# akofke/fountain

Measured on AMD Instinct MI355X. Metric: Mrays/s (primary+secondary) at fixed spp, higher is better.
Workload: dtype f32

## Files before the change

fountain_amd/csrc/ftn_gbuffer.hip:

```cpp
#include "ftn_wavefront.hip"
#include "ftn_gbuffer.h"

namespace ftn {

#define GB_MAX_PASS_THROUGH 4096u
struct GbParams {
    float w2c[16];
    float* out;
    float4 *spillA, *spillB, *spillC;
    float4* rec;
};

__device__ inline Rgb gb_albedo(const ftn_material& m) {
    const Rgb a(m.a[0], m.a[1], m.a[2]), b(m.b[0], m.b[1], m.b[2]);
    switch (m.type) {
        case FTN_MAT_MATTE: return clamp_positive(a);
        case FTN_MAT_MIRROR: return clamp_positive(a);
        case FTN_MAT_METAL: return fresnel_conductor(1.0f, Rgb(1.0f), a, b);
        case FTN_MAT_PLASTIC: return a + b;
        default: return clamp_positive(a) + clamp_positive(b);
    }
}

template <bool TEX>
__global__ void __launch_bounds__(256) k_gb_shade(RenderParams P, WfBuffers W, GbParams G, const uint32_t* __restrict__ q_in, const uint32_t* count_in,
                                                  uint32_t* q_out, uint32_t* count_out) {
    const DScene& S = P.S;
    const uint32_t qi = blockIdx.x * 256u + threadIdx.x;
    bool push = false;
    uint32_t p = 0;
    if (qi < *count_in) {
        p = q_in[qi];
        const float4 ro = W.ray[2 * (size_t)p], rdv = W.ray[2 * (size_t)p + 1];
        DRay ray0; ray0.o = V3(ro.x, ro.y, ro.z); ray0.d = V3(rdv.x, rdv.y, rdv.z); ray0.t_max = rdv.w; ray0.time = 0.0f;
        const DHit h = load_hit(W, p);
        float4 r0 = make_float4(0.0f, 0.0f, 0.0f, 0.0f), r1 = r0, r2 = r0;
        if (h.prim >= 0) {
            DSI si; make_interaction(S, h, ray0, &si);
            if (si.mat < 0) {
                const DRay nr = spawn_ray(si.hit, ray0.d);
                W.ray[2 * (size_t)p] = make_float4(nr.o.x, nr.o.y, nr.o.z, 0.0f); W.ray[2 * (size_t)p + 1] = make_float4(nr.d.x, nr.d.y, nr.d.z, nr.t_max);
                push = true;
            } else {
                ftn_material m = S.materials[si.mat];
                if (TEX && material_is_textured(S, si.mat)) {
                    const uint32_t slot = p / W.samples, sidx = p % W.samples;
                    const DTile tile = P.tiles[slot >> 8];
                    const int px = tile.x0 + (int)(slot & 15u), py = tile.y0 + (int)((slot >> 4) & 15u);
                    Rng crng; crng.seed(indexed_key(P.seed, px, py, W.first_sample + sidx));
                    const V2 j = crng.next2(); const V2 p_film((float)px + j.x, (float)py + j.y); const V2 p_lens = crng.next2(); const float time_u = crng.next();
                    const DRay cam = camera_ray(P.C, p_film, p_lens, time_u);
                    const DRayDiff rd = camera_ray_diff(P.C, p_film, p_lens, cam, 1.0f / sqrtf((float)P.spp));
                    DSIX ex; DSI s2; make_interaction(S, h, ray0, &s2, &ex);
                    const DTexDiffs td = compute_tex_diffs(si.hit.p, si.hit.n, ex.dpdu, ex.dpdv, rd);
                    m = material_resolve(S, si.mat, ex.uv, td);
                }
                const Rgb alb = gb_albedo(m);
                const V3 pc = m4_point(G.w2c, si.hit.p);
                r0 = make_float4(alb.r, alb.g, alb.b, 1.0f);
                r1 = make_float4(si.shading_n.x, si.shading_n.y, si.shading_n.z, pc.z);
                r2 = make_float4(si.hit.p.x, si.hit.p.y, si.hit.p.z, 0.0f);
            }
        }
        if (!push) { float4* R = G.rec + 3 * (size_t)p; R[0] = r0; R[1] = r1; R[2] = r2; }
    }
    const bool pred[1] = {push};
    const uint32_t val[1] = {p};
    uint32_t* const qs[1] = {q_out};
    uint32_t* const cs[1] = {count_out};
    block_push<1>(pred, val, qs, cs);
}

__global__ void k_gb_reset(WfBuffers W, uint32_t out_ctr) {
    if (threadIdx.x != 0 || blockIdx.x != 0) return;
    W.counters[CTR(11)] = 0;
    for (int i = 16; i < 56; i++) W.counters[CTR(i)] = 0;
    W.counters[CTR(out_ctr)] = 0;
}

__device__ inline void gb_film_add(const GbParams& G, const FilmCtxW& F, V2 p_film, float4 r0, float4 r1, float4 r2, int own_x, int own_y, float* acc, uint32_t* spill, uint32_t* bc_writes) {
    const float pdx = p_film.x - 0.5f, pdy = p_film.y - 0.5f;
    int p0x = f2i_sat(ceilf(pdx - F.radius[0])), p0y = f2i_sat(ceilf(pdy - F.radius[1]));
    int p1x = f2i_sat(floorf(pdx + F.radius[0])) + 1, p1y = f2i_sat(floorf(pdy + F.radius[1])) + 1;
    p0x = max(p0x, F.tpb[0]); p0y = max(p0y, F.tpb[1]); p1x = min(p1x, F.tpb[2]); p1y = min(p1y, F.tpb[3]);
    const bool hit = r0.w != 0.0f;
    const float v[10] = {r0.x, r0.y, r0.z, r1.x, r1.y, r1.z, r2.x, r2.y, r2.z, r1.w};
    int touched = 0;
    const size_t width = (size_t)(F.crop[2] - F.crop[0]);
    for (int y = p0y; y < p1y; y++)
        for (int x = p0x; x < p1x; x++) {
            touched++;
            if (x == own_x && y == own_y) {
                if (hit) {
#pragma unroll
                    for (int k = 0; k < 10; k++) acc[k] += v[k] * 1.0f;
                    acc[10] += 1.0f;
                }
                acc[11] += 1.0f;
                continue;
            }
            const size_t i = (size_t)(y - F.crop[1]) * width + (size_t)(x - F.crop[0]);
            float* a = reinterpret_cast<float*>(G.spillA + i);
            float* b = reinterpret_cast<float*>(G.spillB + i);
            float* c = reinterpret_cast<float*>(G.spillC + i);
            if (hit) {
#pragma unroll
                for (int k = 0; k < 3; k++) { atomicAdd(a + k, v[k] * 1.0f); atomicAdd(b + k, v[3 + k] * 1.0f); atomicAdd(c + k, v[6 + k] * 1.0f); }
                atomicAdd(c + 3, v[9] * 1.0f);
                atomicAdd(a + 3, 1.0f);
            }
            atomicAdd(b + 3, 1.0f);
            (*bc_writes)++;
        }
    if (touched != 1) (*spill)++;
}

#define GB_ACC_CHUNK 4u
__global__ void __launch_bounds__(256) k_gb_accumulate(RenderParams P, WfBuffers W, GbParams G) {
    __shared__ float4 s_rec[256 * GB_ACC_CHUNK * 3];
    const uint32_t slot = blockIdx.x * 256u + threadIdx.x;
    uint32_t spill = 0, bc = 0;
    bool valid = false, in_crop = false; int px = 0, py = 0; size_t ai = 0;
    FilmCtxW F; float acc[12];
#pragma unroll
    for (int k = 0; k < 12; k++) acc[k] = 0.0f;
    if (slot < W.n_slots) {
        const DTile tile = P.tiles[slot >> 8];
        px = tile.x0 + (int)(slot & 15u); py = tile.y0 + (int)((slot >> 4) & 15u);
        if (px < tile.x1 && py < tile.y1) {
            valid = true;
            for (int i = 0; i < 4; i++) F.crop[i] = P.crop[i];
            F.sb[0] = tile.x0; F.sb[1] = tile.y0; F.sb[2] = tile.x1; F.sb[3] = tile.y1; F.radius[0] = P.radius[0]; F.radius[1] = P.radius[1];
            const int p0x = f2i_sat(ceilf((float)tile.x0 - 0.5f - P.radius[0])), p0y = f2i_sat(ceilf((float)tile.y0 - 0.5f - P.radius[1]));
            const int p1x = f2i_sat(ceilf((float)tile.x1 - 0.5f + P.radius[0] + 1.0f)), p1y = f2i_sat(ceilf((float)tile.y1 - 0.5f - P.radius[1] + 1.0f));
            F.tpb[0] = max(p0x, P.crop[0]); F.tpb[1] = max(p0y, P.crop[1]); F.tpb[2] = min(p1x, P.crop[2]); F.tpb[3] = min(p1y, P.crop[3]);
            in_crop = px >= P.crop[0] && px < P.crop[2] && py >= P.crop[1] && py < P.crop[3];
            ai = in_crop ? ((size_t)(py - P.crop[1]) * (size_t)(P.crop[2] - P.crop[0]) + (size_t)(px - P.crop[0])) : 0;
            if (in_crop) {
#pragma unroll
                for (int k = 0; k < 12; k++) acc[k] = G.out[12 * ai + k];
            }
        }
    }
    const size_t block_first = (size_t)blockIdx.x * 256u * W.samples;
    for (uint32_t s0 = 0; s0 < W.samples; s0 += GB_ACC_CHUNK) {
        const uint32_t n = W.samples - s0 < GB_ACC_CHUNK ? W.samples - s0 : GB_ACC_CHUNK;
        for (uint32_t e = threadIdx.x; e < 256u * 3u * n; e += 256u) {
            const uint32_t sl = e / (3u * n), k3 = e - sl * 3u * n;
            const size_t p = block_first + (size_t)sl * W.samples + s0 + k3 / 3u;
            if (p < W.n_paths) s_rec[sl * GB_ACC_CHUNK * 3u + k3] = G.rec[3 * p + k3 % 3u];
        }
        __syncthreads();
        if (valid) {
            for (uint32_t k = 0; k < n; k++) {
                const float4* r = &s_rec[(threadIdx.x * GB_ACC_CHUNK + k) * 3u];
                Rng crng; crng.seed(indexed_key(P.seed, px, py, W.first_sample + s0 + k));
                const V2 j = crng.next2();
                gb_film_add(G, F, V2((float)px + j.x, (float)py + j.y), r[0], r[1], r[2], in_crop ? px : (-2147483647), py, acc, &spill, &bc);
            }
        }
        __syncthreads();
    }
    if (valid && in_crop) {
#pragma unroll
        for (int k = 0; k < 12; k++) G.out[12 * ai + k] = acc[k];
    }
    if (spill) atomicAdd(&P.stats->spill_samples, (unsigned long long)spill);
    if (bc) atomicAdd(&P.stats->bc_writes, (unsigned long long)bc);
}

__global__ void __launch_bounds__(256) k_gb_merge(GbParams G, size_t n, const DevStats* __restrict__ stats) {
    if (stats->bc_writes == 0) return;
    for (size_t i = (size_t)blockIdx.x * 256u + threadIdx.x; i < n; i += (size_t)gridDim.x * 256u) {
        const float4 a = G.spillA[i], b = G.spillB[i], c = G.spillC[i];
        if (b.w == 0.0f) continue;
        const float add[12] = {a.x, a.y, a.z, b.x, b.y, b.z, c.x, c.y, c.z, c.w, a.w, b.w};
#pragma unroll
        for (int k = 0; k < 12; k++) G.out[12 * i + k] += add[k];
    }
}

__global__ void __launch_bounds__(256) k_gb_resolve(const float* __restrict__ in, size_t n, float* __restrict__ out12) {
    for (size_t i = (size_t)blockIdx.x * 256u + threadIdx.x; i < n; i += (size_t)gridDim.x * 256u) gbuffer_resolve_pixel(in + 12 * i, out12 + 12 * i);
}
void launch_gbuffer_resolve(const float* in, size_t n, float* out12, hipStream_t stream) {
    if (n == 0) return;
    const unsigned grid = (unsigned)std::min<size_t>((n + 255) / 256, 4096);
    hipLaunchKernelGGL(k_gb_resolve, dim3(grid), dim3(256), 0, stream, in, n, out12);
}

int wavefront_gbuffer(WavefrontState** state, const RenderParams& P, const std::vector<DTile>& tiles, const float w2c[16], float* d_out,
                      float4* spill_a, float4* spill_b, float4* spill_c, hipStream_t stream, double* trace_ms_out) {
    knobs_begin();
    { int rc0 = wf_state_init(state); if (rc0) return rc0; }
    WavefrontState* st = *state;
    const uint32_t n_slots = (uint32_t)tiles.size() * 256u;
    const uint32_t total_samples = P.last_sample - P.first_sample;
    if (n_slots == 0 || total_samples == 0) return FTN_OK;
    if (tiles.size() > ((size_t)1 << 20)) { g_wf_err = "more than 2^20 tiles (2^28 pixel slots) in one call: render the film in several tile ranges"; return FTN_ERR_UNSUPPORTED; }
    uint32_t S = (uint32_t)std::max<size_t>(1, ((size_t)std::min<uint32_t>(knob("FTN_WF_PATHS_M", 256), 256u) << 20) / n_slots);
    S = std::min(S, total_samples);
    int rc = wf_reserve(st, (size_t)S * n_slots);
    while (rc == FTN_ERR_OUT_OF_MEMORY && S > 1) {
        wf_free(st); (void)hipGetLastError();
        S = (S + 1) / 2;
        rc = wf_reserve(st, (size_t)S * n_slots);
    }
    if (rc) { wf_free(st); return rc; }
    if ((rc = trace4_prepare(st, P.S))) return rc;
    WfBuffers W = st->W;
    W.br = nullptr; W.pd = nullptr; W.pd_md = 0; W.pd_occ = 0; W.drain_sig = nullptr; W.drain_seq = 0; W.serial = 0; W.rng_replay = 0; W.mis_any = 0;
    W.gen_blocks = knob("FTN_GEN_BLOCKS", 1);
    uint32_t valid = 0; for (const DTile& t : tiles) valid += (uint32_t)((t.x1 - t.x0) * (t.y1 - t.y0));
    W.valid_per_sample = valid;
    GbParams G;
    memcpy(G.w2c, w2c, sizeof(G.w2c)); G.out = d_out; G.spillA = spill_a; G.spillB = spill_b; G.spillC = spill_c; G.rec = st->pd;
    const bool spheres = P.S.n_spheres != 0, tex = P.S.n_textures != 0;
    const size_t lds = (size_t)P.stack_entries * 256 * sizeof(uint32_t);
    const unsigned blocks_per_cu = (unsigned)std::max<size_t>(1, std::min<size_t>(8, (size_t)(160 * 1024) / std::max<size_t>(lds, 1)));
    const unsigned trace_grid_max = (unsigned)st->n_cu * blocks_per_cu;
    double trace_ms = 0.0;
    for (uint32_t s0 = 0; s0 < total_samples; s0 += S) {
        const uint32_t Sp = std::min(S, total_samples - s0);
        W.n_slots = n_slots; W.samples = Sp; W.n_paths = Sp * n_slots; W.first_sample = P.first_sample + s0; W.seg_cap = (uint32_t)st->cap_paths;
        hipLaunchKernelGGL(k_wf_reset, dim3(1), dim3(64), 0, stream, W, 0, 0, P.stats);
        hipLaunchKernelGGL(k_wf_generate, dim3((W.n_paths + 255) / 256), dim3(256), 0, stream, P, W, 0);
        const unsigned tg = std::min<unsigned>(trace_grid_max, (2 * W.n_paths + 255) / 256);
        uint32_t n_q = Sp * valid;
        for (uint32_t r = 0;; r++) {
            const bool odd = (r & 1u) != 0;
            const uint32_t* q_in = odd ? W.q_shadow : W.q_closest;
            uint32_t* q_out = odd ? W.q_closest : W.q_shadow;
            const uint32_t c_in = odd ? 3u : 2u, c_out = odd ? 2u : 3u;
            if (r > 0) hipLaunchKernelGGL(k_gb_reset, dim3(1), dim3(64), 0, stream, W, c_out);
            WF_TRY(hipEventRecord(st->ev[0], stream));
            launch_trace(st, false, 0, spheres, tg, lds, stream, P, W, q_in, &W.counters[CTR(c_in)], &W.counters[CTR(16)], 2 * W.n_paths,
                         r == 0 && W.samples >= knob("FTN_T4_LOCKSTEP_MIN_SPP", 1) );
            WF_TRY(hipEventRecord(st->ev[1], stream));
            const dim3 sg(std::max<uint32_t>(1u, (n_q + 255) / 256));
            if (tex) hipLaunchKernelGGL(k_gb_shade<true>, sg, dim3(256), 0, stream, P, W, G, q_in, &W.counters[CTR(c_in)], q_out, &W.counters[CTR(c_out)]);
            else hipLaunchKernelGGL(k_gb_shade<false>, sg, dim3(256), 0, stream, P, W, G, q_in, &W.counters[CTR(c_in)], q_out, &W.counters[CTR(c_out)]);
            WF_TRY(hipMemcpyAsync(st->host_counters, W.counters, 16 * 32 * sizeof(uint32_t), hipMemcpyDeviceToHost, stream));
            WF_TRY(hipStreamSynchronize(stream));
            float ms = 0.0f; (void)hipEventElapsedTime(&ms, st->ev[0], st->ev[1]); trace_ms += ms;
            n_q = st->host_counters[CTR(c_out)];
            if (n_q == 0) break;
            if (r == GB_MAX_PASS_THROUGH) {
                g_wf_err = "a camera ray passed through more than 4096 null-material surfaces: the G-buffer would be incomplete";
                return FTN_ERR_INTERNAL;
            }
        }
        hipLaunchKernelGGL(k_gb_accumulate, dim3((n_slots + 255) / 256), dim3(256), 0, stream, P, W, G);
    }
    const size_t npix = (size_t)std::max(0, P.crop[2] - P.crop[0]) * (size_t)std::max(0, P.crop[3] - P.crop[1]);
    if (npix) hipLaunchKernelGGL(k_gb_merge, dim3((unsigned)std::min<size_t>((npix + 255) / 256, 4096)), dim3(256), 0, stream, G, npix, (const DevStats*)P.stats);
    WF_TRY(hipGetLastError());
    if (trace_ms_out) *trace_ms_out = trace_ms;
    return FTN_OK;
}

}
```

fountain_amd/csrc/ftn_trace4.hip:

```cpp
#include "ftn_wf_common.h"

namespace ftn {

enum : uint32_t { T4_IDLE = 0, T4_NODE = 1, T4_LEAF = 2 };
#define T4_NONE 0xffffffffu

typedef float t4_f2 __attribute__((ext_vector_type(2)));
__device__ inline bool slab4(float4 a, float4 b, V3 o, V3 inv, float t_max, float* t0o, float* t1o) {
    const float k = 1.0f + 2.0f * gamma_n(3);
    const t4_f2 px = {a.x, a.y}, py = {a.z, a.w}, pz = {b.x, b.y};
    const t4_f2 tx = (px - (t4_f2){o.x, o.x}) * (t4_f2){inv.x, inv.x};
    const t4_f2 ty = (py - (t4_f2){o.y, o.y}) * (t4_f2){inv.y, inv.y};
    const t4_f2 tz = (pz - (t4_f2){o.z, o.z}) * (t4_f2){inv.z, inv.z};
    const float far_k = fmin_(fmin_(fmax_(tx.x, tx.y), fmax_(ty.x, ty.y)), fmax_(tz.x, tz.y)) * k;
    const float t0 = fmax_(fmax_(fmax_(0.0f, fmin_(tx.x, tx.y)), fmin_(ty.x, ty.y)), fmin_(tz.x, tz.y));
    const float t1 = fmin_(t_max, far_k);
    *t0o = t0; *t1o = t1;
    return !(t0 > t1);
}

struct WaveQueue {
    uint32_t chunk_next, chunk_end, slice, slices_done, chunk; bool exhausted;
};
__device__ inline void wq_init(WaveQueue& q, uint32_t count, uint32_t chunk_max) {
    q.chunk_next = 0; q.chunk_end = 0; q.exhausted = count == 0; q.slice = blockIdx.x & 7u; q.slices_done = 0;
    uint32_t c = count / (gridDim.x * 4u * 16u); c &= ~63u; q.chunk = c < 64u ? 64u : (c > chunk_max ? chunk_max : c);
}
__device__ inline bool wq_refill(WaveQueue& q, uint32_t count, uint32_t* head, uint32_t lane) {
    bool just_dry = false;
    while (q.chunk_next == q.chunk_end && !q.exhausted) {
        const uint32_t s_lo = (uint32_t)(((unsigned long long)count * q.slice) >> 3) & ~63u, s_hi = q.slice == 7u ? count : ((uint32_t)(((unsigned long long)count * (q.slice + 1u)) >> 3) & ~63u);
        uint32_t base = 0;
        if (lane == 0) base = atomicAdd(head + CTR(q.slice), q.chunk);
        base = __shfl(base, 0, 64) + s_lo;
        if (base >= s_hi) { q.slice = (q.slice + 1u) & 7u; if (++q.slices_done == 8u) { q.exhausted = true; just_dry = true; } }
        else { q.chunk_next = base; q.chunk_end = base + q.chunk < s_hi ? base + q.chunk : s_hi; }
    }
    return just_dry;
}

struct RaySetup { V3 o, inv, dorig; float t_max, sx, sy, sz; uint32_t neg24 ; int kz; };
__device__ inline bool ray_is_exceptional(float ox, float oy, float oz, float ix, float iy, float iz) {
    return !(fabsf(ix) < FTN_INF && fabsf(iy) < FTN_INF && fabsf(iz) < FTN_INF && ix != 0.0f && iy != 0.0f && iz != 0.0f &&
             fabsf(ox) < FTN_INF && fabsf(oy) < FTN_INF && fabsf(oz) < FTN_INF &&
             fabsf(ox * ix) < FTN_INF && fabsf(oy * iy) < FTN_INF && fabsf(oz * iz) < FTN_INF);
}
template <bool SPHERES>
__device__ inline void ray_setup(RaySetup& R, float4 a, float4 b) {
    R.o = V3(a.x, a.y, a.z); const V3 d(b.x, b.y, b.z); R.t_max = b.w;
    if (SPHERES) R.dorig = d;
    R.inv = V3(1.0f / d.x, 1.0f / d.y, 1.0f / d.z);
    R.neg24 = ((d.x < 0.0f ? 1u : 0u) | (d.y < 0.0f ? 2u : 0u) | (d.z < 0.0f ? 4u : 0u)) * 0x010101u;
    R.kz = max_dimension(vabs(d));
    const bool k0 = R.kz == 0, k1 = R.kz == 1;
    const V3 dperm(k0 ? d.y : (k1 ? d.z : d.x), k0 ? d.z : (k1 ? d.x : d.y), k0 ? d.x : (k1 ? d.y : d.z));
    R.sx = -dperm.x / dperm.z; R.sy = -dperm.y / dperm.z; R.sz = 1.0f / dperm.z;
}

template <class E> struct T4Stack {
    E* base; E* lim; E* sp; E* spill; size_t n_lanes, gl; uint32_t spill_levels;
    __device__ inline size_t spill_at() const { const uint32_t lv = (uint32_t)((sp - lim) >> 8); return (size_t)(lv < spill_levels ? lv : spill_levels - 1u) * n_lanes + gl; }
    template <bool CHECK> __device__ inline void push(E v) {
        if (!CHECK || sp < lim) *sp = v; else if (spill_levels) spill[spill_at()] = v;
        sp += 256;
    }
    template <bool CHECK> __device__ inline E pop() {
        sp -= 256;
        if (!CHECK || sp < lim) return *sp;
        return spill_levels ? spill[spill_at()] : *base;
    }
    __device__ inline bool empty() const { return sp == base; }
};

enum : uint32_t { T8_IDLE = 0, T8_NODE = 1, T8_LEAF = 2, T8_LEAF_IN = 3  };
#define T8_XBOX 0x40000000u
__device__ inline bool ray_out_of_range8(float ox, float oy, float oz, float ix, float iy, float iz) {
    const float big_i = 1.152921504606846976e18f , big_o = 1.099511627776e12f ;
    return !(fabsf(ix) <= big_i && fabsf(iy) <= big_i && fabsf(iz) <= big_i && fabsf(ox) <= big_o && fabsf(oy) <= big_o && fabsf(oz) <= big_o);
}
struct T8Axis { float a, bn, bf; uint32_t n03, n47, f03, f47; };
__device__ inline T8Axis t8_axis(float org, uint32_t ebyte, float o, float inv, uint32_t lo03, uint32_t lo47, uint32_t hi03, uint32_t hi47) {
    T8Axis A;
    const float step = __uint_as_float(ebyte << 23);
    A.a = step * inv;
    const float b = (org - o) * inv;
    const float m = (fabsf(b) + 255.0f * fabsf(A.a)) * 9.5367431640625e-07f;
    A.bn = b - m; A.bf = b + m;
    const bool neg = inv < 0.0f;
    A.n03 = neg ? hi03 : lo03; A.n47 = neg ? hi47 : lo47; A.f03 = neg ? lo03 : hi03; A.f47 = neg ? lo47 : hi47;
    return A;
}
#define T8_BYTE(w, k) ((float)(((w) >> (8 * (k))) & 0xffu))
#define T8_CHILD(c, t0v, t1v) \
    { const uint32_t kx_ = (c) & 3; \
      const t4_f2 tx_ = __builtin_elementwise_fma((t4_f2){T8_BYTE((c) < 4 ? X.n03 : X.n47, kx_), T8_BYTE((c) < 4 ? X.f03 : X.f47, kx_)}, (t4_f2){X.a, X.a}, (t4_f2){X.bn, X.bf}); \
      const t4_f2 ty_ = __builtin_elementwise_fma((t4_f2){T8_BYTE((c) < 4 ? Y.n03 : Y.n47, kx_), T8_BYTE((c) < 4 ? Y.f03 : Y.f47, kx_)}, (t4_f2){Y.a, Y.a}, (t4_f2){Y.bn, Y.bf}); \
      const t4_f2 tz_ = __builtin_elementwise_fma((t4_f2){T8_BYTE((c) < 4 ? Z.n03 : Z.n47, kx_), T8_BYTE((c) < 4 ? Z.f03 : Z.f47, kx_)}, (t4_f2){Z.a, Z.a}, (t4_f2){Z.bn, Z.bf}); \
      t0v = fmax_(fmax_(fmax_(0.0f, tx_.x), ty_.x), tz_.x); t1v = fmin_(t_max, fmin_(fmin_(tx_.y, ty_.y), tz_.y) * k2); }

struct T4Lane { uint32_t mode, cur, lp; bool finish; };

template <bool CHECK>
__device__ inline void t4_pop_next(T4Stack<uint2>& St, T4Lane& L, float t_max) {
    for (;;) {
        if (St.empty()) { L.finish = true; return; }
        const uint2 v = St.template pop<CHECK>();
        if (!(__uint_as_float(v.y) > t_max)) {
            if (v.x >> 31) { L.lp = v.x & 0x7fffffffu; L.mode = T4_LEAF; } else { L.cur = v.x; L.mode = T4_NODE; }
            return;
        }
    }
}

template <bool CHECK>
__device__ __forceinline__ void t4_visit(T4Stack<uint2>& St, T4Lane& L, float t_max, uint32_t ea, uint32_t eb, uint32_t ec, uint32_t ed, float ta, float tb, float tc, float td, uint32_t ax) {
    const bool sA = (ax & 0xffu) != 0, sR = (ax & 0xff00u) != 0, sB = (ax & 0xff0000u) != 0;
    const uint32_t ex0 = sA ? eb : ea, ex1 = sA ? ea : eb, ey0 = sB ? ed : ec, ey1 = sB ? ec : ed;
    const float tx0 = sA ? tb : ta, tx1 = sA ? ta : tb, ty0 = sB ? td : tc, ty1 = sB ? tc : td;
    const uint32_t e0 = sR ? ey0 : ex0, e1 = sR ? ey1 : ex1, e2 = sR ? ex0 : ey0, e3 = sR ? ex1 : ey1;
    const float t1_ = sR ? ty1 : tx1, t2_ = sR ? tx0 : ty0, t3_ = sR ? tx1 : ty1;
    const bool h0 = e0 != T4_NONE, h1 = e1 != T4_NONE, h2 = e2 != T4_NONE, h3 = e3 != T4_NONE;
    const bool h01 = h0 || h1, h012 = h01 || h2;
    if (h3 && h012) St.template push<CHECK>(make_uint2(e3, __float_as_uint(t3_)));
    if (h2 && h01) St.template push<CHECK>(make_uint2(e2, __float_as_uint(t2_)));
    if (h1 && h0) St.template push<CHECK>(make_uint2(e1, __float_as_uint(t1_)));
    if (h012 || h3) {
        const uint32_t next = h0 ? e0 : (h1 ? e1 : (h2 ? e2 : e3));
        if (next >> 31) { L.lp = next & 0x7fffffffu; L.mode = T4_LEAF; } else L.cur = next;
    } else t4_pop_next<CHECK>(St, L, t_max);
}

template <bool CHECK>
__device__ inline void t4_record_step(const DScene& S, const RaySetup& R, T4Stack<uint2>& St, T4Lane& L) {
    const float4* rec = reinterpret_cast<const float4*>(reinterpret_cast<const char*>(S.quad) + L.cur);
    const float4 q0 = rec[0], q1 = rec[1], q2 = rec[2], q3 = rec[3], q4 = rec[4], q5 = rec[5], q6 = rec[6], q7 = rec[7];
    float ta, tb, tc, td, x1;
    const bool ha = slab4(q0, q1, R.o, R.inv, R.t_max, &ta, &x1), hb = slab4(q2, q3, R.o, R.inv, R.t_max, &tb, &x1);
    const bool hc = slab4(q4, q5, R.o, R.inv, R.t_max, &tc, &x1), hd = slab4(q6, q7, R.o, R.inv, R.t_max, &td, &x1);
    const uint32_t ea = ha ? __float_as_uint(q1.z) : T4_NONE, eb = hb ? __float_as_uint(q3.z) : T4_NONE, ec = hc ? __float_as_uint(q5.z) : T4_NONE, ed = hd ? __float_as_uint(q7.z) : T4_NONE;
    t4_visit<CHECK>(St, L, R.t_max, ea, eb, ec, ed, ta, tb, tc, td, __float_as_uint(q1.w) & R.neg24);
}

template <bool CHECK>
__device__ __forceinline__ void t4q_record_step(const DScene& S, T4Stack<uint2>& St, T4Lane& L, V3 o, V3 inv, float t_max, uint32_t neg24) {
    const uint4* rec = reinterpret_cast<const uint4*>(reinterpret_cast<const char*>(S.quad64) + L.cur);
    const uint4 r0 = rec[0], r1 = rec[1], r2 = rec[2], r3 = rec[3];
    const float k2 = 1.0f + 4.0f * gamma_n(3);
    const T8Axis X = t8_axis(__uint_as_float(r0.x), r0.w & 0xffu, o.x, inv.x, r1.x, r1.x, r1.y, r1.y);
    const T8Axis Y = t8_axis(__uint_as_float(r0.y), (r0.w >> 8) & 0xffu, o.y, inv.y, r1.z, r1.z, r1.w, r1.w);
    const T8Axis Z = t8_axis(__uint_as_float(r0.z), (r0.w >> 16) & 0xffu, o.z, inv.z, r2.x, r2.x, r2.y, r2.y);
    float ta, a1, tb, b1, tc, c1, td, d1;
    T8_CHILD(0, ta, a1) T8_CHILD(1, tb, b1) T8_CHILD(2, tc, c1) T8_CHILD(3, td, d1)
    const uint32_t ea = !(ta > a1) ? r2.z : T4_NONE, eb = !(tb > b1) ? r2.w : T4_NONE, ec = !(tc > c1) ? r3.x : T4_NONE, ed = !(td > d1) ? r3.y : T4_NONE;
    t4_visit<CHECK>(St, L, t_max, ea, eb, ec, ed, ta, tb, tc, td, r3.z & neg24);
}

enum : uint32_t { T4_LEAF_IN = 3 };
template <bool COUNT, bool SPHERES, int BURST, bool Q64 = false>
__global__ void __launch_bounds__(256, (SPHERES ? 1 : (Q64 ? T4Q_WAVES : 5))) k_wf_trace4(DScene S, WfBuffers W, const uint32_t* __restrict__ queue, const uint32_t* count_ptr, uint32_t* head, DevStats* stats,
                                                   uint32_t refill, uint32_t leaf_batch, uint32_t chunk_max, uint32_t lds_entries, uint2* __restrict__ spill, uint32_t spill_levels) {
    T4Stack<uint2> St;
    extern __shared__ uint2 lds_stack2[];
    St.base = lds_stack2 + threadIdx.x;
    St.lim = St.base + 256u * lds_entries; St.sp = St.base; St.spill = spill; St.spill_levels = spill_levels;
    St.n_lanes = (size_t)gridDim.x * 256u; St.gl = (size_t)blockIdx.x * 256u + threadIdx.x;
    const bool st_tiny = lds_entries < 3u;
    uint2* const st_soft = st_tiny ? St.base : St.lim - 3 * 256;
    const uint32_t count = *count_ptr;
    const uint32_t lane = lane_id();
    unsigned long long n_rec = 0, n_prim = 0;
    unsigned long long occ[7] = {0, 0, 0, 0, 0, 0, 0};
    T4Lane L; L.mode = T4_IDLE; L.cur = 0; L.lp = 0; L.finish = false;
    WaveQueue Q; wq_init(Q, count, chunk_max);
    uint32_t rid = 0;
    RaySetup R; R.o = V3(0.0f, 0.0f, 0.0f); R.inv = R.o; R.dorig = R.o; R.t_max = 0.0f; R.neg24 = 0; R.kz = 0; R.sx = R.sy = R.sz = 0.0f;
    int hprim = -1; float hb0 = 0.0f, hb1 = 0.0f, hb2 = 0.0f; bool found = false;
    const float4 rlo = make_float4(S.root_lo[0], S.root_lo[1], S.root_lo[2], 0.0f), rhi = make_float4(S.root_hi[0], S.root_hi[1], S.root_hi[2], 0.0f);
    for (;;) {
        const unsigned long long idle = __ballot(L.mode == T4_IDLE);
        if (!Q.exhausted && (uint32_t)__popcll(idle) >= refill) {
            const uint32_t need = (uint32_t)__popcll(idle);
            if (wq_refill(Q, count, head, lane)) {
                if (W.drain_sig && lane == 0 && atomicAdd(&W.counters[CTR(11)], 1u) + 1u == W.drain_at)
                    __hip_atomic_store(W.drain_sig, W.drain_seq, __ATOMIC_RELAXED, __HIP_MEMORY_SCOPE_SYSTEM);
            }
            const uint32_t avail = Q.chunk_end - Q.chunk_next;
            const uint32_t rank = (uint32_t)__popcll(idle & ((1ull << lane) - 1ull));
            bool hand_back = false; uint32_t q_entry = 0;
            if (COUNT) { occ[5]++; occ[6] += need < avail ? need : avail; }
            if (L.mode == T4_IDLE && rank < avail) {
                float4 a, b;
                q_entry = queue[Q.chunk_next + rank];
                load_queued_ray<false>(W, q_entry, &a, &b, &rid);
                ray_setup<SPHERES>(R, a, b);
                St.sp = St.base; L.cur = 0; found = false; hprim = -1; hb0 = 0.0f; hb1 = 0.0f; hb2 = 0.0f;
                if (ray_is_exceptional(R.o.x, R.o.y, R.o.z, R.inv.x, R.inv.y, R.inv.z) || (Q64 && ray_out_of_range8(R.o.x, R.o.y, R.o.z, R.inv.x, R.inv.y, R.inv.z)))
                    hand_back = true;
                else if (S.n_nodes == 0 || !slab_test(rlo, rhi, R.o, R.inv, R.t_max)) { W.hit[rid] = make_float4(FTN_INF, 0.0f, 0.0f, 0.0f); W.hit_prim[rid] = -1; }
                else if (S.root_is_leaf) { L.lp = 0; L.mode = T4_LEAF; }
                else L.mode = T4_NODE;
            }
            if (__ballot(hand_back) != 0) wave_push(hand_back, q_entry, W.q_exc_closest, &W.counters[CTR(32)]);
            Q.chunk_next += (need < avail ? need : avail);
        }
        const unsigned long long m_node = __ballot(L.mode == T4_NODE), m_leaf = __ballot(L.mode >= T4_LEAF);
        if ((m_node | m_leaf) == 0) { if (Q.exhausted) break; else continue; }
        L.finish = false;
        if (COUNT) occ[0]++;
        if (m_node != 0 && (uint32_t)__popcll(m_leaf) < leaf_batch) {
#pragma unroll
            for (int burst = 0; burst < BURST; burst++) {
                const bool on = L.mode == T4_NODE && !L.finish;
                if (COUNT && on) n_rec++;
                if (COUNT) { const unsigned long long m_on = __ballot(on); if (m_on) { occ[1]++; occ[2] += (unsigned long long)__popcll(m_on); } }
                if (__builtin_expect(__ballot(on && (st_tiny || St.sp > st_soft)) == 0, 1)) {
                    if (on) { if (Q64) t4q_record_step<false>(S, St, L, R.o, R.inv, R.t_max, R.neg24); else t4_record_step<false>(S, R, St, L); }
                } else if (on) { if (Q64) t4q_record_step<true>(S, St, L, R.o, R.inv, R.t_max, R.neg24); else t4_record_step<true>(S, R, St, L); }
            }
        } else {
            if (COUNT) { occ[3]++; occ[4] += (unsigned long long)__popcll(m_leaf); }
            if (L.mode >= T4_LEAF) {
                uint32_t prim = L.lp;
                const bool entering = Q64 && L.mode == T4_LEAF, explicit_box = entering && (L.lp & T8_XBOX);
                float4 x0 = make_float4(0.0f, 0.0f, 0.0f, 0.0f), x1 = x0;
                if (Q64) prim &= 0x3fffffffu;
                if (explicit_box) { x0 = S.quad64_xbox[2 * (size_t)prim]; x1 = S.quad64_xbox[2 * (size_t)prim + 1]; prim = __float_as_uint(x0.w); }
                float4 g0 = S.geom[S.geom_stride * prim], g1 = S.geom[S.geom_stride * prim + 1], g2 = S.geom[S.geom_stride * prim + 2];
                pin4(g0); pin4(g1); pin4(g2);
                bool pass = true;
                if (entering) {
                    if (!explicit_box) {
                        x0 = make_float4(fmin_(fmin_(g0.x, g1.x), g2.x), fmin_(fmin_(g0.y, g1.y), g2.y), fmin_(fmin_(g0.z, g1.z), g2.z), 0.0f);
                        x1 = make_float4(fmax_(fmax_(g0.x, g1.x), g2.x), fmax_(fmax_(g0.y, g1.y), g2.y), fmax_(fmax_(g0.z, g1.z), g2.z), 0.0f);
                    }
                    pass = slab_test(x0, x1, R.o, R.inv, R.t_max);
                }
                if (pass) {
                    if (COUNT) n_prim++;
                    float t = 0.0f, b0 = 0.0f, b1 = 0.0f, b2 = 0.0f;
                    const bool hh = prim_hit<SPHERES>(S, prim, g0, g1, g2, R.o, R.dorig, R.t_max, R.kz, R.sx, R.sy, R.sz, &t, &b0, &b1, &b2);
                    if (hh) { found = true; R.t_max = t; hprim = (int)prim; hb0 = b0; hb1 = b1; hb2 = b2; }
                }
                if (!pass || (__float_as_uint(g0.w) & GF_LEAF_END)) t4_pop_next<true>(St, L, R.t_max);
                else { L.lp = prim + 1u; if (Q64) L.mode = T4_LEAF_IN; }
            }
        }
        if (L.finish) {
            W.hit[rid] = make_float4(found ? R.t_max : FTN_INF, hb0, hb1, hb2); W.hit_prim[rid] = hprim;
            L.mode = T4_IDLE;
        }
    }
    if (COUNT) {
        for (int off = 32; off > 0; off >>= 1) { n_rec += __shfl_down(n_rec, off, 64); n_prim += __shfl_down(n_prim, off, 64); }
        if (lane == 0) { if (n_rec) atomicAdd(&stats->quad_records, n_rec); if (n_prim) atomicAdd(&stats->prims_tested, n_prim); for (int k = 0; k < 7; k++) if (occ[k]) atomicAdd(&stats->t4_occ[k], occ[k]); }
    }
    if (blockIdx.x == 0 && threadIdx.x == 0) atomicAdd(&stats->rays_closest, (unsigned long long)count);
}

extern __shared__ uint32_t lds_stack1[];
template <bool CHECK, int POLICY>
__device__ inline void t4_any_step(const DScene& S, const RaySetup& R, T4Stack<uint32_t>& St, T4Lane& L) {
    const float4* rec = reinterpret_cast<const float4*>(reinterpret_cast<const char*>(S.quad) + L.cur);
    const float4 q0 = rec[0], q1 = rec[1], q2 = rec[2], q3 = rec[3], q4 = rec[4], q5 = rec[5], q6 = rec[6], q7 = rec[7];
    float a0, a1, b0, b1, c0, c1, d0, d1;
    const bool ha = slab4(q0, q1, R.o, R.inv, R.t_max, &a0, &a1), hb = slab4(q2, q3, R.o, R.inv, R.t_max, &b0, &b1);
    const bool hc = slab4(q4, q5, R.o, R.inv, R.t_max, &c0, &c1), hd = slab4(q6, q7, R.o, R.inv, R.t_max, &d0, &d1);
    const uint32_t ea = __float_as_uint(q1.z), eb = __float_as_uint(q3.z), ec = __float_as_uint(q5.z), ed = __float_as_uint(q7.z);
    uint32_t next = 0; bool have = ha || hb || hc || hd;
    if (POLICY == 1) {
        const float sa = ha ? fmaxf(a1 - a0, 0.0f) : -1.0f, sb = hb ? fmaxf(b1 - b0, 0.0f) : -1.0f, sc = hc ? fmaxf(c1 - c0, 0.0f) : -1.0f, sd = hd ? fmaxf(d1 - d0, 0.0f) : -1.0f;
        const float best = fmaxf(fmaxf(sa, sb), fmaxf(sc, sd));
        const bool pa = sa == best, pb = !pa && sb == best, pc = !pa && !pb && sc == best, pd = !pa && !pb && !pc;
        next = pa ? ea : (pb ? eb : (pc ? ec : ed));
        if (ha && !pa) St.template push<CHECK>(ea);
        if (hb && !pb) St.template push<CHECK>(eb);
        if (hc && !pc) St.template push<CHECK>(ec);
        if (hd && !pd) St.template push<CHECK>(ed);
    } else {
        next = ha ? ea : (hb ? eb : (hc ? ec : ed));
        if (hd && (ha || hb || hc)) St.template push<CHECK>(ed);
        if (hc && (ha || hb)) St.template push<CHECK>(ec);
        if (hb && ha) St.template push<CHECK>(eb);
    }
    if (!have) {
        if (St.empty()) { L.finish = true; return; }
        next = St.template pop<CHECK>();
    }
    if (next >> 31) { L.lp = next & 0x7fffffffu; L.mode = T4_LEAF; } else L.cur = next;
}

template <bool COUNT, bool SPHERES, int BURST, int POLICY>
__global__ void __launch_bounds__(256) k_wf_trace4_any(DScene S, WfBuffers W, const uint32_t* __restrict__ queue, const uint32_t* count_ptr, uint32_t* head, DevStats* stats,
                                                       uint32_t refill, uint32_t leaf_batch, uint32_t chunk_max, uint32_t lds_entries, uint32_t* __restrict__ spill, uint32_t spill_levels) {
    T4Stack<uint32_t> St;
    St.base = lds_stack1 + threadIdx.x;
    St.lim = St.base + 256u * lds_entries; St.sp = St.base; St.spill = spill; St.spill_levels = spill_levels;
    St.n_lanes = (size_t)gridDim.x * 256u; St.gl = (size_t)blockIdx.x * 256u + threadIdx.x;
    const bool st_tiny = lds_entries < 3u;
    uint32_t* const st_soft = st_tiny ? St.base : St.lim - 3 * 256;
    const uint32_t count = *count_ptr;
    const uint32_t lane = lane_id();
    unsigned long long n_rec = 0, n_prim = 0;
    unsigned long long occ[7] = {0, 0, 0, 0, 0, 0, 0};
    T4Lane L; L.mode = T4_IDLE; L.cur = 0; L.lp = 0; L.finish = false;
    WaveQueue Q; wq_init(Q, count, chunk_max);
    uint32_t rid = 0;
    RaySetup R; R.o = V3(0.0f, 0.0f, 0.0f); R.inv = R.o; R.dorig = R.o; R.t_max = 0.0f; R.neg24 = 0; R.kz = 0; R.sx = R.sy = R.sz = 0.0f;
    bool found = false;
    const float4 rlo = make_float4(S.root_lo[0], S.root_lo[1], S.root_lo[2], 0.0f), rhi = make_float4(S.root_hi[0], S.root_hi[1], S.root_hi[2], 0.0f);
    for (;;) {
        const unsigned long long idle = __ballot(L.mode == T4_IDLE);
        if (!Q.exhausted && (uint32_t)__popcll(idle) >= refill) {
            const uint32_t need = (uint32_t)__popcll(idle);
            (void)wq_refill(Q, count, head, lane);
            const uint32_t avail = Q.chunk_end - Q.chunk_next;
            const uint32_t rank = (uint32_t)__popcll(idle & ((1ull << lane) - 1ull));
            bool hand_back = false; uint32_t q_entry = 0;
            if (COUNT) { occ[5]++; occ[6] += need < avail ? need : avail; }
            if (L.mode == T4_IDLE && rank < avail) {
                float4 a, b;
                q_entry = queue[Q.chunk_next + rank];
                load_queued_ray<true>(W, q_entry, &a, &b, &rid);
                ray_setup<SPHERES>(R, a, b);
                St.sp = St.base; L.cur = 0; found = false;
                if (ray_is_exceptional(R.o.x, R.o.y, R.o.z, R.inv.x, R.inv.y, R.inv.z)) hand_back = true;
                else if (S.n_nodes == 0 || !slab_test(rlo, rhi, R.o, R.inv, R.t_max)) store_occluded(W, rid, false);
                else if (S.root_is_leaf) { L.lp = 0; L.mode = T4_LEAF; }
                else L.mode = T4_NODE;
            }
            if (__ballot(hand_back) != 0) wave_push(hand_back, q_entry, W.q_exc_any, &W.counters[CTR(33)]);
            Q.chunk_next += (need < avail ? need : avail);
        }
        const unsigned long long m_node = __ballot(L.mode == T4_NODE), m_leaf = __ballot(L.mode == T4_LEAF);
        if ((m_node | m_leaf) == 0) { if (Q.exhausted) break; else continue; }
        L.finish = false;
        if (COUNT) occ[0]++;
        if (m_node != 0 && (uint32_t)__popcll(m_leaf) < leaf_batch) {
#pragma unroll
            for (int burst = 0; burst < BURST; burst++) {
                const bool on = L.mode == T4_NODE && !L.finish;
                if (COUNT && on) n_rec++;
                if (COUNT) { const unsigned long long m_on = __ballot(on); if (m_on) { occ[1]++; occ[2] += (unsigned long long)__popcll(m_on); } }
                if (__builtin_expect(__ballot(on && (st_tiny || St.sp > st_soft)) == 0, 1)) { if (on) t4_any_step<false, POLICY>(S, R, St, L); }
                else if (on) t4_any_step<true, POLICY>(S, R, St, L);
            }
        } else {
            if (COUNT) { occ[3]++; occ[4] += (unsigned long long)__popcll(m_leaf); }
            if (L.mode == T4_LEAF) {
                const uint32_t prim = L.lp;
                float4 g0 = S.geom[S.geom_stride * prim], g1 = S.geom[S.geom_stride * prim + 1], g2 = S.geom[S.geom_stride * prim + 2];
                pin4(g0); pin4(g1); pin4(g2);
                if (COUNT) n_prim++;
                float t = 0.0f, b0 = 0.0f, b1 = 0.0f, b2 = 0.0f;
                const bool hh = prim_hit<SPHERES>(S, prim, g0, g1, g2, R.o, R.dorig, R.t_max, R.kz, R.sx, R.sy, R.sz, &t, &b0, &b1, &b2);
                if (hh) { found = true; L.finish = true; }
                else if (__float_as_uint(g0.w) & GF_LEAF_END) {
                    if (St.empty()) L.finish = true;
                    else { const uint32_t next = St.template pop<true>(); if (next >> 31) L.lp = next & 0x7fffffffu; else { L.cur = next; L.mode = T4_NODE; } }
                } else L.lp++;
            }
        }
        if (L.finish) { store_occluded(W, rid, found); L.mode = T4_IDLE; }
    }
    if (COUNT) {
        for (int off = 32; off > 0; off >>= 1) { n_rec += __shfl_down(n_rec, off, 64); n_prim += __shfl_down(n_prim, off, 64); }
        if (lane == 0) {
            if (n_rec) { atomicAdd(&stats->quad_records, n_rec); atomicAdd(&stats->quad_records_any, n_rec); }
            if (n_prim) { atomicAdd(&stats->prims_tested, n_prim); atomicAdd(&stats->prims_any, n_prim); }
            for (int k = 0; k < 7; k++) if (occ[k]) atomicAdd(&stats->t4_occ[7 + k], occ[k]);
        }
    }
    if (blockIdx.x == 0 && threadIdx.x == 0) atomicAdd(&stats->rays_any, (unsigned long long)count);
}

template <bool CHECK, int POLICY>
__device__ __forceinline__ void t8_any_step(const DScene& S, T4Stack<uint32_t>& St, T4Lane& L, V3 o, V3 inv, float t_max) {
    const uint4* rec = reinterpret_cast<const uint4*>(reinterpret_cast<const char*>(S.oct) + L.cur);
    const uint4 r0 = rec[0], r1 = rec[1], r2 = rec[2], r3 = rec[3], r4 = rec[4], r5 = rec[5];
    const float k2 = 1.0f + 4.0f * gamma_n(3);
    const T8Axis X = t8_axis(__uint_as_float(r0.x), r0.w & 0xffu, o.x, inv.x, r3.x, r3.y, r3.z, r3.w);
    const T8Axis Y = t8_axis(__uint_as_float(r0.y), (r0.w >> 8) & 0xffu, o.y, inv.y, r4.x, r4.y, r4.z, r4.w);
    const T8Axis Z = t8_axis(__uint_as_float(r0.z), (r0.w >> 16) & 0xffu, o.z, inv.z, r5.x, r5.y, r5.z, r5.w);
    float a0, a1, b0, b1, c0, c1, d0, d1, e0, e1, f0, f1, g0, g1, h0, h1;
    T8_CHILD(0, a0, a1) T8_CHILD(1, b0, b1) T8_CHILD(2, c0, c1) T8_CHILD(3, d0, d1) T8_CHILD(4, e0, e1) T8_CHILD(5, f0, f1) T8_CHILD(6, g0, g1) T8_CHILD(7, h0, h1)
    const uint32_t la = r1.x, lb = r1.y, lc = r1.z, ld = r1.w, le = r2.x, lf = r2.y, lg = r2.z, lh = r2.w;
    const bool ha = !(a0 > a1) && la != T4_NONE, hb = !(b0 > b1) && lb != T4_NONE, hc = !(c0 > c1) && lc != T4_NONE, hd = !(d0 > d1) && ld != T4_NONE;
    const bool he = !(e0 > e1) && le != T4_NONE, hf = !(f0 > f1) && lf != T4_NONE, hg = !(g0 > g1) && lg != T4_NONE, hh = !(h0 > h1) && lh != T4_NONE;
    uint32_t next = T4_NONE;
    if (POLICY == 1) {
        const float sa = ha ? a1 - a0 : -1.0f, sb = hb ? b1 - b0 : -1.0f, sc = hc ? c1 - c0 : -1.0f, sd = hd ? d1 - d0 : -1.0f;
        const float se = he ? e1 - e0 : -1.0f, sf = hf ? f1 - f0 : -1.0f, sg = hg ? g1 - g0 : -1.0f, sh = hh ? h1 - h0 : -1.0f;
        const float best = fmaxf(fmaxf(fmaxf(sa, sb), fmaxf(sc, sd)), fmaxf(fmaxf(se, sf), fmaxf(sg, sh)));
        bool taken = !(best >= 0.0f);
#define T8_PICK(hx, sx, lx) { const bool me_ = hx && !taken && sx == best; if (me_) { next = lx; taken = true; } else if (hx) St.template push<CHECK>(lx); }
        T8_PICK(ha, sa, la) T8_PICK(hb, sb, lb) T8_PICK(hc, sc, lc) T8_PICK(hd, sd, ld) T8_PICK(he, se, le) T8_PICK(hf, sf, lf) T8_PICK(hg, sg, lg) T8_PICK(hh, sh, lh)
#undef T8_PICK
    } else {
        bool taken = false;
#define T8_PICK(hx, lx) { if (hx) { if (!taken) { next = lx; taken = true; } else St.template push<CHECK>(lx); } }
        T8_PICK(ha, la) T8_PICK(hb, lb) T8_PICK(hc, lc) T8_PICK(hd, ld) T8_PICK(he, le) T8_PICK(hf, lf) T8_PICK(hg, lg) T8_PICK(hh, lh)
#undef T8_PICK
    }
    if (next == T4_NONE) {
        if (St.empty()) { L.finish = true; return; }
        next = St.template pop<CHECK>();
    }
    if (next >> 31) { L.lp = next & 0x7fffffffu; L.mode = T8_LEAF; } else L.cur = next;
}

template <bool COUNT, int BURST, int POLICY>
__global__ void __launch_bounds__(256) k_wf_trace8_any(DScene S, WfBuffers W, const uint32_t* __restrict__ queue, const uint32_t* count_ptr, uint32_t* head, DevStats* stats,
                                                       uint32_t refill, uint32_t leaf_batch, uint32_t chunk_max, uint32_t lds_entries, uint32_t* __restrict__ spill, uint32_t spill_levels) {
    T4Stack<uint32_t> St;
    St.base = lds_stack1 + threadIdx.x;
    St.lim = St.base + 256u * lds_entries; St.sp = St.base; St.spill = spill; St.spill_levels = spill_levels;
    St.n_lanes = (size_t)gridDim.x * 256u; St.gl = (size_t)blockIdx.x * 256u + threadIdx.x;
    const bool st_tiny = lds_entries < 7u;
    uint32_t* const st_soft = st_tiny ? St.base : St.lim - 7 * 256;
    const uint32_t count = *count_ptr;
    const uint32_t lane = lane_id();
    unsigned long long n_rec = 0, n_prim = 0;
    unsigned long long occ[7] = {0, 0, 0, 0, 0, 0, 0};
    T4Lane L; L.mode = T8_IDLE; L.cur = 0; L.lp = 0; L.finish = false;
    WaveQueue Q; wq_init(Q, count, chunk_max);
    uint32_t rid = 0;
    RaySetup R; R.o = V3(0.0f, 0.0f, 0.0f); R.inv = R.o; R.dorig = R.o; R.t_max = 0.0f; R.neg24 = 0; R.kz = 0; R.sx = R.sy = R.sz = 0.0f;
    bool found = false;
    const float4 rlo = make_float4(S.root_lo[0], S.root_lo[1], S.root_lo[2], 0.0f), rhi = make_float4(S.root_hi[0], S.root_hi[1], S.root_hi[2], 0.0f);
    for (;;) {
        const unsigned long long idle = __ballot(L.mode == T8_IDLE);
        if (!Q.exhausted && (uint32_t)__popcll(idle) >= refill) {
            const uint32_t need = (uint32_t)__popcll(idle);
            (void)wq_refill(Q, count, head, lane);
            const uint32_t avail = Q.chunk_end - Q.chunk_next;
            const uint32_t rank = (uint32_t)__popcll(idle & ((1ull << lane) - 1ull));
            bool hand_back = false; uint32_t q_entry = 0;
            if (COUNT) { occ[5]++; occ[6] += need < avail ? need : avail; }
            if (L.mode == T8_IDLE && rank < avail) {
                float4 a, b;
                q_entry = queue[Q.chunk_next + rank];
                load_queued_ray<true>(W, q_entry, &a, &b, &rid);
                ray_setup<false>(R, a, b);
                St.sp = St.base; L.cur = 0; found = false;
                if (ray_is_exceptional(R.o.x, R.o.y, R.o.z, R.inv.x, R.inv.y, R.inv.z) || ray_out_of_range8(R.o.x, R.o.y, R.o.z, R.inv.x, R.inv.y, R.inv.z)) hand_back = true;
                else if (!slab_test(rlo, rhi, R.o, R.inv, R.t_max)) store_occluded(W, rid, false);
                else L.mode = T8_NODE;
            }
            if (__ballot(hand_back) != 0) wave_push(hand_back, q_entry, W.q_exc_any, &W.counters[CTR(33)]);
            Q.chunk_next += (need < avail ? need : avail);
        }
        const unsigned long long m_node = __ballot(L.mode == T8_NODE), m_leaf = __ballot(L.mode >= T8_LEAF);
        if ((m_node | m_leaf) == 0) { if (Q.exhausted) break; else continue; }
        L.finish = false;
        if (COUNT) occ[0]++;
        if (m_node != 0 && (uint32_t)__popcll(m_leaf) < leaf_batch) {
#pragma unroll
            for (int burst = 0; burst < BURST; burst++) {
                const bool on = L.mode == T8_NODE && !L.finish;
                if (COUNT && on) n_rec++;
                if (COUNT) { const unsigned long long m_on = __ballot(on); if (m_on) { occ[1]++; occ[2] += (unsigned long long)__popcll(m_on); } }
                if (__builtin_expect(__ballot(on && (st_tiny || St.sp > st_soft)) == 0, 1)) { if (on) t8_any_step<false, POLICY>(S, St, L, R.o, R.inv, R.t_max); }
                else if (on) t8_any_step<true, POLICY>(S, St, L, R.o, R.inv, R.t_max);
            }
        } else {
            if (COUNT) { occ[3]++; occ[4] += (unsigned long long)__popcll(m_leaf); }
            if (L.mode >= T8_LEAF) {
                const bool entering = L.mode == T8_LEAF;
                uint32_t prim = L.lp & 0x3fffffffu;
                float4 x0 = make_float4(0.0f, 0.0f, 0.0f, 0.0f), x1 = x0;
                const bool explicit_box = entering && (L.lp & T8_XBOX);
                if (explicit_box) { x0 = S.oct_xbox[2 * (size_t)prim]; x1 = S.oct_xbox[2 * (size_t)prim + 1]; prim = __float_as_uint(x0.w); }
                float4 g0 = S.geom[S.geom_stride * prim], g1 = S.geom[S.geom_stride * prim + 1], g2 = S.geom[S.geom_stride * prim + 2];
                pin4(g0); pin4(g1); pin4(g2);
                bool pass = true;
                if (entering) {
                    if (!explicit_box) {
                        x0 = make_float4(fmin_(fmin_(g0.x, g1.x), g2.x), fmin_(fmin_(g0.y, g1.y), g2.y), fmin_(fmin_(g0.z, g1.z), g2.z), 0.0f);
                        x1 = make_float4(fmax_(fmax_(g0.x, g1.x), g2.x), fmax_(fmax_(g0.y, g1.y), g2.y), fmax_(fmax_(g0.z, g1.z), g2.z), 0.0f);
                    }
                    pass = slab_test(x0, x1, R.o, R.inv, R.t_max);
                }
                bool hh = false;
                if (pass) {
                    if (COUNT) n_prim++;
                    float t = 0.0f, b0 = 0.0f, b1 = 0.0f, b2 = 0.0f;
                    hh = prim_hit<false>(S, prim, g0, g1, g2, R.o, R.dorig, R.t_max, R.kz, R.sx, R.sy, R.sz, &t, &b0, &b1, &b2);
                }
                if (hh) { found = true; L.finish = true; }
                else if (!pass || (__float_as_uint(g0.w) & GF_LEAF_END)) {
                    if (St.empty()) L.finish = true;
                    else { const uint32_t next = St.template pop<true>(); if (next >> 31) { L.lp = next & 0x7fffffffu; L.mode = T8_LEAF; } else { L.cur = next; L.mode = T8_NODE; } }
                } else { L.lp = prim + 1u; L.mode = T8_LEAF_IN; }
            }
        }
        if (L.finish) { store_occluded(W, rid, found); L.mode = T8_IDLE; }
    }
    if (COUNT) {
        for (int off = 32; off > 0; off >>= 1) { n_rec += __shfl_down(n_rec, off, 64); n_prim += __shfl_down(n_prim, off, 64); }
        if (lane == 0) {
            if (n_rec) { atomicAdd(&stats->quad_records, n_rec); atomicAdd(&stats->quad_records_any, n_rec); }
            if (n_prim) { atomicAdd(&stats->prims_tested, n_prim); atomicAdd(&stats->prims_any, n_prim); }
            for (int k = 0; k < 7; k++) if (occ[k]) atomicAdd(&stats->t4_occ[7 + k], occ[k]);
        }
    }
    if (blockIdx.x == 0 && threadIdx.x == 0) atomicAdd(&stats->rays_any, (unsigned long long)count);
}

Trace4Plan trace4_plan(const DScene& S, int n_cu, uint32_t knob_entries_closest, uint32_t knob_entries_any, uint32_t knob_wg_closest, uint32_t knob_wg_any, uint32_t knob_wg_oct, uint32_t knob_entries_oct) {
    Trace4Plan p; memset(&p, 0, sizeof(p));
    const uint32_t bound = S.quad_stack_bound ? S.quad_stack_bound : 1u;
    const uint32_t wg_c = knob_wg_closest ? knob_wg_closest : 5u, wg_a = knob_wg_any ? knob_wg_any : 4u;
    const uint32_t budget_c = ((158u * 1024u) / wg_c) & ~1023u, budget_a = ((158u * 1024u) / wg_a) & ~1023u;
    uint32_t ec = knob_entries_closest ? knob_entries_closest : budget_c / (256u * 8u);
    uint32_t ea = knob_entries_any ? knob_entries_any : budget_a / (256u * 4u);
    p.entries_closest = ec < bound ? ec : bound; p.entries_any = ea < bound ? ea : bound;
    if (p.entries_closest == 0) p.entries_closest = 1;
    if (p.entries_any == 0) p.entries_any = 1;
    p.spill_closest = bound - p.entries_closest; p.spill_any = bound - p.entries_any;
    p.lds_closest = (size_t)p.entries_closest * 256u * 8u; p.lds_any = (size_t)p.entries_any * 256u * 4u;
    auto per_cu = [](size_t lds, uint32_t wg) { return (unsigned)std::max<size_t>(1, std::min<size_t>(wg, (size_t)(158 * 1024) / std::max<size_t>(lds, 1))); };
    p.grid_closest = (unsigned)n_cu * per_cu(p.lds_closest, wg_c); p.grid_any = (unsigned)n_cu * per_cu(p.lds_any, wg_a);
    if (S.quad64 && S.n_quad64) {
        const uint32_t wg_q = knob_wg_closest ? knob_wg_closest : (uint32_t)T4Q_WAVES, budget_q = ((158u * 1024u) / wg_q) & ~1023u;
        const uint32_t bound_q = S.quad64_stack_bound ? S.quad64_stack_bound : 1u;
        uint32_t eq = knob_entries_closest ? knob_entries_closest : budget_q / (256u * 8u);
        p.entries_q64 = eq < bound_q ? eq : bound_q;
        if (p.entries_q64 == 0) p.entries_q64 = 1;
        p.spill_q64 = bound_q - p.entries_q64;
        p.lds_q64 = (size_t)p.entries_q64 * 256u * 8u;
        p.grid_q64 = (unsigned)n_cu * per_cu(p.lds_q64, wg_q);
        p.q64_ok = true;
    }
    if (S.oct && S.n_octs) {
        const uint32_t wg_8 = knob_wg_oct ? knob_wg_oct : 5u, budget_8 = ((158u * 1024u) / wg_8) & ~1023u, bound8 = S.oct_stack_bound ? S.oct_stack_bound : 1u;
        const uint32_t e8 = knob_entries_oct ? knob_entries_oct : budget_8 / (256u * 4u);
        p.entries_oct = e8 < bound8 ? e8 : bound8;
        p.spill_oct = bound8 - p.entries_oct;
        p.lds_oct = (size_t)p.entries_oct * 256u * 4u;
        p.grid_oct = (unsigned)n_cu * per_cu(p.lds_oct, wg_8);
        p.oct_ok = true;
    }
    return p;
}

void launch_trace4(int kind, bool count, bool spheres, unsigned grid, size_t lds, uint32_t lds_entries, void* spill, hipStream_t stream, const DScene& S, const WfBuffers& W,
                   const uint32_t* queue, const uint32_t* count_ptr, uint32_t* head, DevStats* stats, uint32_t refill, uint32_t leaf_batch, uint32_t chunk, uint32_t burst, uint32_t any_policy, uint32_t spill_levels) {
    const bool any = kind == T4K_ANY || kind == T4K_ANY_OCT;
#define FTN_T4(K, SPILL_T, ...) hipLaunchKernelGGL((K<__VA_ARGS__>), dim3(grid), dim3(256), lds, stream, S, W, queue, count_ptr, head, stats, refill, leaf_batch, chunk, lds_entries, (SPILL_T)spill, spill_levels)
    if (kind == T4K_CLOSEST_Q64) {
        if (count) FTN_T4(k_wf_trace4, uint2*, true, false, 2, true);
        else if (burst <= 1) FTN_T4(k_wf_trace4, uint2*, false, false, 1, true); else if (burst == 2) FTN_T4(k_wf_trace4, uint2*, false, false, 2, true);
        else if (burst == 3) FTN_T4(k_wf_trace4, uint2*, false, false, 3, true); else FTN_T4(k_wf_trace4, uint2*, false, false, 4, true);
    } else if (kind == T4K_ANY_OCT) {
#define FTN_T8(C, B) do { if (any_policy == 0) FTN_T4(k_wf_trace8_any, uint32_t*, C, B, 0); else FTN_T4(k_wf_trace8_any, uint32_t*, C, B, 1); } while (0)
        if (count) FTN_T8(true, 2);
        else if (burst <= 1) FTN_T8(false, 1); else if (burst == 2) FTN_T8(false, 2); else FTN_T8(false, 3);
#undef FTN_T8
    } else if (any) {
#define FTN_T4A(C, Sp, B) do { if (any_policy == 0) FTN_T4(k_wf_trace4_any, uint32_t*, C, Sp, B, 0); else FTN_T4(k_wf_trace4_any, uint32_t*, C, Sp, B, 1); } while (0)
        if (count) { if (spheres) FTN_T4A(true, true, 2); else FTN_T4A(true, false, 2); }
        else if (spheres) { if (burst <= 2) FTN_T4A(false, true, 2); else FTN_T4A(false, true, 4); }
        else { if (burst <= 1) FTN_T4A(false, false, 1); else if (burst == 2) FTN_T4A(false, false, 2); else if (burst == 3) FTN_T4A(false, false, 3); else FTN_T4A(false, false, 4); }
#undef FTN_T4A
    } else {
        if (count) { if (spheres) FTN_T4(k_wf_trace4, uint2*, true, true, 2); else FTN_T4(k_wf_trace4, uint2*, true, false, 2); }
        else if (spheres) { if (burst <= 2) FTN_T4(k_wf_trace4, uint2*, false, true, 2); else FTN_T4(k_wf_trace4, uint2*, false, true, 4); }
        else { if (burst <= 1) FTN_T4(k_wf_trace4, uint2*, false, false, 1); else if (burst == 2) FTN_T4(k_wf_trace4, uint2*, false, false, 2); else if (burst == 3) FTN_T4(k_wf_trace4, uint2*, false, false, 3); else FTN_T4(k_wf_trace4, uint2*, false, false, 4); }
    }
#undef FTN_T4
}

}
```

fountain_amd/csrc/ftn_wavefront.hip:

```cpp
#include "ftn_wf_common.h"
#include "ftn_texture.h"
#include <string>
#include <cstdlib>
#include <hipcub/hipcub.hpp>

namespace ftn {

__global__ void __launch_bounds__(256) k_wf_generate(RenderParams P, WfBuffers W, int write_state) {
    const uint32_t i = blockIdx.x * 256u + threadIdx.x;
    if (i >= W.n_paths) return;
    const uint32_t slot = i / W.samples, s = i % W.samples;
    const DTile tile = P.tiles[slot >> 8];
    const int px = tile.x0 + (int)(slot & 15u), py = tile.y0 + (int)((slot >> 4) & 15u);
    if (px < tile.x1 && py < tile.y1) {
        Rng rng; rng.seed(indexed_key(P.seed, px, py, W.first_sample + s));
        V2 j = rng.next2();
        V2 p_film((float)px + j.x, (float)py + j.y);
        V2 p_lens = rng.next2();
        float time_u = rng.next();
        DRay ray = camera_ray(P.C, p_film, p_lens, time_u);
        W.ray[2 * (size_t)(i)] = make_float4(ray.o.x, ray.o.y, ray.o.z, 0.0f);
        W.ray[2 * (size_t)(i) + 1] = make_float4(ray.d.x, ray.d.y, ray.d.z, ray.t_max);
        if (write_state) {
            W.beta[i] = make_float4(1.0f, 1.0f, 1.0f, __uint_as_float(PS_ALIVE));
            W.rad[i] = make_float4(0.0f, 0.0f, 0.0f, 0.0f);
            W.rng01[i] = make_ulonglong2(rng.s0, rng.s1); W.rng23[i] = make_ulonglong2(rng.s2, rng.s3);
        }
        uint32_t local = (uint32_t)(py - tile.y0) * (uint32_t)(tile.x1 - tile.x0) + (uint32_t)(px - tile.x0);
        if (W.gen_blocks && tile.x1 - tile.x0 == 16 && tile.y1 - tile.y0 == 16) {
            const uint32_t x = slot & 15u, y = (slot >> 4) & 15u;
            local = (x & 1u) | ((y & 1u) << 1) | ((x & 2u) << 1) | ((y & 2u) << 2) | ((x & 4u) << 2) | ((y & 4u) << 3) | ((x & 8u) << 3) | ((y & 8u) << 4);
        }
        const uint32_t pix = tile.valid_off + local;
        const uint32_t qi = pix * W.samples + s;
        W.q_active[0][qi] = i | (P.max_depth == 0 ? WF_Q_DEPTH : 0u);
        W.q_closest[qi] = i;
    }
}

enum : uint32_t { TM_IDLE = 0, TM_NODE = 1, TM_LEAF = 2 };

template <bool ANY, bool COUNT, bool SPHERES, int BURST >
__global__ void __launch_bounds__(256) k_wf_trace(DScene S, WfBuffers W, const uint32_t* __restrict__ queue, const uint32_t* count_ptr, uint32_t* head,
                                                  DevStats* stats, uint32_t refill, uint32_t leaf_batch, uint32_t chunk, uint32_t node_burst) {
    extern __shared__ uint32_t lds_stack[];
    uint32_t* const st_base = lds_stack + threadIdx.x;
    uint32_t* sptr = st_base;
    const uint32_t count = *count_ptr;
    const uint32_t lane = lane_id();
    const uint32_t np = W.n_paths;
    TravCount tc{0, 0};
    uint32_t w_idle_lanes = 0, w_leafwait_lanes = 0;
    uint32_t w_node_steps = 0, w_leaf_steps = 0;
    uint32_t mode = TM_IDLE;
    uint32_t chunk_next = 0, chunk_end = 0; bool exhausted = count == 0;
    uint32_t slice = blockIdx.x & 7u, slices_done = 0;
    { uint32_t c = count / (gridDim.x * 4u * 16u); c &= ~63u; chunk = c < 64u ? 64u : (c > chunk ? chunk : c); }
    uint32_t rid = 0, cur = 0 , neg16 = 0, lp = 0, lp_end = 0;
    V3 o, inv, dperm; float t_max = 0.0f, sx = 0.0f, sy = 0.0f, sz = 0.0f; int kz = 0;
    int hprim = -1; float hb0 = 0.0f, hb1 = 0.0f, hb2 = 0.0f; bool found = false;
    V3 dorig;
    for (;;) {
        const unsigned long long idle = __ballot(mode == TM_IDLE);
        if (!exhausted && (uint32_t)__popcll(idle) >= refill) {
            const uint32_t need = (uint32_t)__popcll(idle);
            while (chunk_next == chunk_end && !exhausted) {
                const uint32_t s_lo = (uint32_t)(((unsigned long long)count * slice) >> 3) & ~63u, s_hi = slice == 7u ? count : ((uint32_t)(((unsigned long long)count * (slice + 1u)) >> 3) & ~63u);
                uint32_t base = 0;
                if (lane == 0) base = atomicAdd(head + CTR(slice), chunk);
                base = __shfl(base, 0, 64) + s_lo;
                if (base >= s_hi) {
                    slice = (slice + 1u) & 7u;
                    if (++slices_done == 8u) {
                        exhausted = true;
                        if (!ANY && W.drain_sig && lane == 0 && atomicAdd(&W.counters[CTR(11)], 1u) + 1u == W.drain_at)
                            __hip_atomic_store(W.drain_sig, W.drain_seq, __ATOMIC_RELAXED, __HIP_MEMORY_SCOPE_SYSTEM);
                    }
                }
                else { chunk_next = base; chunk_end = base + chunk < s_hi ? base + chunk : s_hi; }
            }
            const uint32_t avail = chunk_end - chunk_next;
            const uint32_t rank = (uint32_t)__popcll(idle & ((1ull << lane) - 1ull));
            if (mode == TM_IDLE && rank < avail) {
                float4 a, b;
                load_queued_ray<ANY>(W, queue[chunk_next + rank], &a, &b, &rid);
                o = V3(a.x, a.y, a.z); const V3 d(b.x, b.y, b.z); t_max = b.w;
                if (SPHERES) dorig = d;
                inv = V3(1.0f / d.x, 1.0f / d.y, 1.0f / d.z);
                neg16 = (d.x < 0.0f ? 0x10000u : 0u) | (d.y < 0.0f ? 0x20000u : 0u) | (d.z < 0.0f ? 0x40000u : 0u);
                kz = max_dimension(vabs(d));
                { const int kx = kz == 2 ? 0 : kz + 1, ky = kx == 2 ? 0 : kx + 1; dperm = V3(d.get(kx), d.get(ky), d.get(kz)); }
                sx = -dperm.x / dperm.z; sy = -dperm.y / dperm.z; sz = 1.0f / dperm.z;
                sptr = st_base; cur = 0; found = false; hprim = -1; hb0 = 0.0f; hb1 = 0.0f; hb2 = 0.0f;
                mode = TM_NODE;
                if (S.n_nodes == 0) {
                    if (ANY) store_occluded(W, rid, false); else { W.hit[rid] = make_float4(FTN_INF, 0.0f, 0.0f, 0.0f); W.hit_prim[rid] = -1; }
                    mode = TM_IDLE;
                }
            }
            chunk_next += (need < avail ? need : avail);
        }
        const unsigned long long m_node = __ballot(mode == TM_NODE), m_leaf = __ballot(mode == TM_LEAF);
        if ((m_node | m_leaf) == 0) { if (exhausted) break; else continue; }
        bool finish = false;
        if (m_node != 0 && (uint32_t)__popcll(m_leaf) < leaf_batch) {
#pragma unroll
            for (uint32_t burst = 0; burst < (BURST ? (uint32_t)BURST : node_burst); burst++) {
                if (COUNT && __ballot(mode == TM_NODE && !finish) != 0) { w_node_steps++; w_idle_lanes += (uint32_t)__popcll(__ballot(mode == TM_IDLE || finish)); w_leafwait_lanes += (uint32_t)__popcll(__ballot(mode == TM_LEAF)); }
                if (mode == TM_NODE && !finish) {
                    const float4* rec = reinterpret_cast<const float4*>(reinterpret_cast<const char*>(S.nodes) + cur);
                    float4 na = rec[0], nb = rec[1];
                    pin4(na); pin4(nb);
                    if (COUNT) tc.nodes++;
                    bool pop = true;
                    if (slab_test_node(na, nb, o, inv, t_max)) {
                        const uint32_t idx = __float_as_uint(nb.z), meta = __float_as_uint(nb.w);
                        if (meta >> 24) { lp = idx; lp_end = idx + (meta & 0xffffu); mode = TM_LEAF; pop = false; }
                        else {
                            if (meta & neg16) { *sptr = cur + 32u; cur = idx; }
                            else { *sptr = idx; cur = cur + 32u; }
                            sptr += 256;
                            pop = false;
                        }
                    }
                    if (pop) { if (sptr == st_base) finish = true; else { sptr -= 256; cur = *sptr; } }
                }
            }
        } else {
            if (COUNT) w_leaf_steps++;
            if (mode == TM_LEAF) {
                const uint32_t prim = lp;
                float4 g0 = S.geom[S.geom_stride * prim], g1 = S.geom[S.geom_stride * prim + 1], g2 = S.geom[S.geom_stride * prim + 2];
                pin4(g0); pin4(g1); pin4(g2);
                if (COUNT) tc.prims++;
                float t = 0.0f, b0 = 0.0f, b1 = 0.0f, b2 = 0.0f;
                const bool hh = prim_hit<SPHERES>(S, prim, g0, g1, g2, o, dorig, t_max, kz, sx, sy, sz, &t, &b0, &b1, &b2);
                if (hh) { found = true; t_max = t; hprim = (int)prim; hb0 = b0; hb1 = b1; hb2 = b2; }
                lp++;
                if (ANY && hh) finish = true;
                else if (lp == lp_end) { if (sptr == st_base) finish = true; else { sptr -= 256; cur = *sptr; mode = TM_NODE; } }
            }
        }
        if (finish) {
            if (ANY) store_occluded(W, rid, found);
            else { W.hit[rid] = make_float4(found ? t_max : FTN_INF, hb0, hb1, hb2); W.hit_prim[rid] = hprim; }
            mode = TM_IDLE;
        }
    }
    if (COUNT) {
        unsigned long long n = tc.nodes, p = tc.prims;
        for (int off = 32; off > 0; off >>= 1) { n += __shfl_down(n, off, 64); p += __shfl_down(p, off, 64); }
        if (lane == 0) {
            if (n) atomicAdd(&stats->nodes_visited, n); if (p) atomicAdd(&stats->prims_tested, p);
            if (ANY) { if (n) atomicAdd(&stats->nodes_any, n); if (p) atomicAdd(&stats->prims_any, p); }
            atomicAdd(&W.counters[CTR(6)], w_node_steps); atomicAdd(&W.counters[CTR(7)], w_leaf_steps);
            atomicAdd(&W.counters[CTR(8)], w_idle_lanes >> 6); atomicAdd(&W.counters[CTR(9)], w_leafwait_lanes >> 6);
        }
    }
    if (stats && blockIdx.x == 0 && threadIdx.x == 0) { if (ANY) atomicAdd(&stats->rays_any, (unsigned long long)count); else atomicAdd(&stats->rays_closest, (unsigned long long)count); }
}

template <bool SPHERES>
__global__ void __launch_bounds__(256) k_wf_trace_any2(DScene S, WfBuffers W, const uint32_t* __restrict__ queue, const uint32_t* count_ptr, uint32_t* head,
                                                       DevStats* stats, uint32_t refill, uint32_t leaf_batch, uint32_t chunk, uint32_t policy) {
    extern __shared__ uint32_t lds_stack[];
    uint32_t* const st_base = lds_stack + threadIdx.x;
    uint32_t* sptr = st_base;
    const uint32_t count = *count_ptr;
    const uint32_t lane = lane_id();
    uint32_t mode = TM_IDLE;
    uint32_t chunk_next = 0, chunk_end = 0; bool exhausted = count == 0;
    uint32_t slice = blockIdx.x & 7u, slices_done = 0;
#ifdef FTN_DRAIN_PROBE
    const uint32_t t_start = (uint32_t)wall_clock64(); uint32_t t_dry = t_start; bool seen_dry = false;
#endif
    { uint32_t c = count / (gridDim.x * 4u * 16u); c &= ~63u; chunk = c < 64u ? 64u : (c > chunk ? chunk : c); }
    uint32_t rid = 0, cur = 0, neg16 = 0, lp = 0;
    V3 o, inv, dperm; float t_max = 0.0f, sx = 0.0f, sy = 0.0f, sz = 0.0f; int kz = 0;
    bool found = false;
    V3 dorig;
    const float4 rlo = make_float4(S.root_lo[0], S.root_lo[1], S.root_lo[2], 0.0f), rhi = make_float4(S.root_hi[0], S.root_hi[1], S.root_hi[2], 0.0f);
    for (;;) {
        const unsigned long long idle = __ballot(mode == TM_IDLE);
        if (!exhausted && (uint32_t)__popcll(idle) >= refill) {
            const uint32_t need = (uint32_t)__popcll(idle);
            while (chunk_next == chunk_end && !exhausted) {
                const uint32_t s_lo = (uint32_t)(((unsigned long long)count * slice) >> 3) & ~63u, s_hi = slice == 7u ? count : ((uint32_t)(((unsigned long long)count * (slice + 1u)) >> 3) & ~63u);
                uint32_t base = 0;
                if (lane == 0) base = atomicAdd(head + CTR(slice), chunk);
                base = __shfl(base, 0, 64) + s_lo;
                if (base >= s_hi) { slice = (slice + 1u) & 7u; if (++slices_done == 8u) exhausted = true; }
                else { chunk_next = base; chunk_end = base + chunk < s_hi ? base + chunk : s_hi; }
            }
            const uint32_t avail = chunk_end - chunk_next;
            const uint32_t rank = (uint32_t)__popcll(idle & ((1ull << lane) - 1ull));
            if (mode == TM_IDLE && rank < avail) {
                float4 a, b;
                load_queued_ray<true>(W, queue[chunk_next + rank], &a, &b, &rid);
                o = V3(a.x, a.y, a.z); const V3 d(b.x, b.y, b.z); t_max = b.w;
                if (SPHERES) dorig = d;
                inv = V3(1.0f / d.x, 1.0f / d.y, 1.0f / d.z);
                neg16 = (d.x < 0.0f ? 0x10000u : 0u) | (d.y < 0.0f ? 0x20000u : 0u) | (d.z < 0.0f ? 0x40000u : 0u);
                kz = max_dimension(vabs(d));
                { const int kx = kz == 2 ? 0 : kz + 1, ky = kx == 2 ? 0 : kx + 1; dperm = V3(d.get(kx), d.get(ky), d.get(kz)); }
                sx = -dperm.x / dperm.z; sy = -dperm.y / dperm.z; sz = 1.0f / dperm.z;
                sptr = st_base; cur = 0; found = false;
                if (S.n_nodes == 0 || !slab_test(rlo, rhi, o, inv, t_max)) { store_occluded(W, rid, false); mode = TM_IDLE; }
                else if (S.root_is_leaf) { lp = 0; mode = TM_LEAF; }
                else mode = TM_NODE;
            }
            chunk_next += (need < avail ? need : avail);
        }
        const unsigned long long m_node = __ballot(mode == TM_NODE), m_leaf = __ballot(mode == TM_LEAF);
#ifdef FTN_DRAIN_PROBE
        if (exhausted && !seen_dry) { seen_dry = true; t_dry = (uint32_t)wall_clock64(); }
#endif
        if ((m_node | m_leaf) == 0) { if (exhausted) break; else continue; }
        bool finish = false;
        if (m_node != 0 && (uint32_t)__popcll(m_leaf) < leaf_batch) {
#pragma unroll
            for (uint32_t burst = 0; burst < 8u; burst++) {
                if (mode == TM_NODE && !finish) {
                    const float4* rec = reinterpret_cast<const float4*>(reinterpret_cast<const char*>(S.fat) + cur);
                    float4 a0 = rec[0], b0 = rec[1], a1 = rec[2], b1 = rec[3];
                    pin4(a0); pin4(b0); pin4(a1); pin4(b1);
                    float i00, i01, i10, i11;
                    const bool h0 = slab_test_node_iv(a0, b0, o, inv, t_max, &i00, &i01), h1 = slab_test_node_iv(a1, b1, o, inv, t_max, &i10, &i11);
                    const uint32_t m0 = __float_as_uint(b0.w), m1 = __float_as_uint(b1.w);
                    const uint32_t e0 = __float_as_uint(b0.z) | ((m0 >> 24) ? 0x80000000u : 0u), e1 = __float_as_uint(b1.z) | ((m1 >> 24) ? 0x80000000u : 0u);
                    const bool second_first = (policy & 0xffu) == 2u ? (i11 - i10) > (i01 - i00) : (((m0 & neg16) != 0) != ((policy & 0xffu) == 1u));
                    const uint32_t en = second_first ? e1 : e0, ef = second_first ? e0 : e1;
                    const bool hn = second_first ? h1 : h0, hf = second_first ? h0 : h1;
                    uint32_t next = 0; bool have = true;
                    if (hn) { next = en; if (hf) { *sptr = ef; sptr += 256; } }
                    else if (hf) next = ef;
                    else if (sptr == st_base) { finish = true; have = false; }
                    else { sptr -= 256; next = *sptr; }
                    if (have) { if (next >> 31) { lp = next & 0x7fffffffu; mode = TM_LEAF; } else cur = next; }
                }
            }
        } else {
            if (mode == TM_LEAF) {
                const uint32_t prim = lp;
                float4 g0 = S.geom[S.geom_stride * prim], g1 = S.geom[S.geom_stride * prim + 1], g2 = S.geom[S.geom_stride * prim + 2];
                pin4(g0); pin4(g1); pin4(g2);
                float t = 0.0f, b0 = 0.0f, b1 = 0.0f, b2 = 0.0f;
                const bool hh = prim_hit<SPHERES>(S, prim, g0, g1, g2, o, dorig, t_max, kz, sx, sy, sz, &t, &b0, &b1, &b2);
                if (hh) { found = true; finish = true; }
                else if (__float_as_uint(g0.w) & GF_LEAF_END) {
                    if (sptr == st_base) finish = true;
                    else { sptr -= 256; const uint32_t next = *sptr; if (next >> 31) lp = next & 0x7fffffffu; else { cur = next; mode = TM_NODE; } }
                } else lp++;
            }
        }
        if (finish) { store_occluded(W, rid, found); mode = TM_IDLE; }
    }
#ifdef FTN_DRAIN_PROBE
    if (lane == 0) {
        uint32_t* T = &W.counters[CTR(13) + 4 * ((policy >> 8) & 7u)];
        atomicMax(&T[0], ~t_start); atomicMax(&T[1], ~t_dry); atomicMax(&T[2], t_dry); atomicMax(&T[3], (uint32_t)wall_clock64());
    }
#endif
    if (blockIdx.x == 0 && threadIdx.x == 0) atomicAdd(&stats->rays_any, (unsigned long long)count);
}

#define WF_NCLASS 8
__device__ inline uint32_t wf_class_of(const RenderParams& P, const WfBuffers& W, uint32_t entry) {
    if (entry & WF_Q_FIN) return 0u;
    const int prim = W.hit_prim[entry & WF_Q_ID_MASK];
    if (prim < 0 || (entry & WF_Q_DEPTH)) return 1u;
    return P.S.prim_class[prim];
}
#define WF_CLS_ROUNDS 32
__global__ void __launch_bounds__(256) k_wf_classify(RenderParams P, WfBuffers W, int in_q) {
    __shared__ unsigned char s_cls[WF_CLS_ROUNDS][256];
    __shared__ uint32_t s_cnt[WF_CLS_ROUNDS][WF_NCLASS][4];
    __shared__ uint32_t s_pre[WF_CLS_ROUNDS][WF_NCLASS];
    __shared__ uint32_t s_base[WF_NCLASS];
    const uint32_t count = W.counters[CTR(in_q == 0 ? 0 : 1)];
    const uint32_t stride = gridDim.x * 256u, rounds = (count + stride - 1) / stride;
    const uint32_t wave = threadIdx.x >> 6, lane = lane_id();
    for (uint32_t r0 = 0; r0 < rounds; r0 += WF_CLS_ROUNDS) {
        const uint32_t nr = rounds - r0 < WF_CLS_ROUNDS ? rounds - r0 : WF_CLS_ROUNDS;
        for (uint32_t r = 0; r < nr; r++) {
            const uint32_t qi = (r0 + r) * stride + blockIdx.x * 256u + threadIdx.x;
            uint32_t c = WF_NCLASS;
            if (qi < count) c = wf_class_of(P, W, W.q_active[in_q][qi]);
            s_cls[r][threadIdx.x] = (unsigned char)c;
#pragma unroll
            for (int k = 0; k < WF_NCLASS; k++) {
                const unsigned long long m = __ballot(c == (uint32_t)k);
                if (lane == 0) s_cnt[r][k][wave] = (uint32_t)__popcll(m);
            }
        }
        __syncthreads();
        if (threadIdx.x < WF_NCLASS) {
            const uint32_t k = threadIdx.x; uint32_t tot = 0;
            for (uint32_t r = 0; r < nr; r++) { s_pre[r][k] = tot; tot += s_cnt[r][k][0] + s_cnt[r][k][1] + s_cnt[r][k][2] + s_cnt[r][k][3]; }
            s_base[k] = tot ? atomicAdd(&W.cls[CTR(k)], tot) : 0u;
        }
        __syncthreads();
        for (uint32_t r = 0; r < nr; r++) {
            const uint32_t qi = (r0 + r) * stride + blockIdx.x * 256u + threadIdx.x;
            const uint32_t c = s_cls[r][threadIdx.x];
            unsigned long long mine = 0;
#pragma unroll
            for (int k = 0; k < WF_NCLASS; k++) { const unsigned long long m = __ballot(c == (uint32_t)k); if (c == (uint32_t)k) mine = m; }
            if (c < WF_NCLASS) {
                uint32_t off = s_base[c] + s_pre[r][c];
                for (uint32_t w2 = 0; w2 < wave; w2++) off += s_cnt[r][c][w2];
                W.q_sorted[(size_t)c * W.seg_cap + off + (uint32_t)__popcll(mine & ((1ull << lane) - 1ull))] = W.q_active[in_q][qi] & WF_Q_ID_MASK;
            }
        }
        __syncthreads();
    }
}

__device__ inline DHit load_hit(const WfBuffers& W, uint32_t r) {
    const float4 h = W.hit[r]; DHit o; o.t = h.x; o.b0 = h.y; o.b1 = h.z; o.b2 = h.w; o.prim = W.hit_prim[r]; return o;
}

#ifndef FTN_SHADE_MIN_WAVES
#define FTN_SHADE_MIN_WAVES 1
#endif
#ifndef FTN_SHADE_WAVES_NOBSDF
#define FTN_SHADE_WAVES_NOBSDF 4
#endif
#ifndef FTN_SHADE_WAVES_MATTE
#define FTN_SHADE_WAVES_MATTE 3
#endif
#ifndef FTN_SHADE_WAVES_OTHER
#define FTN_SHADE_WAVES_OTHER 3
#endif
template <bool TEX, int MT, bool ENV>
__global__ void __launch_bounds__(256, (MT == -1 ? FTN_SHADE_MIN_WAVES : (MT == -2 ? FTN_SHADE_WAVES_NOBSDF : (MT == 0 ? FTN_SHADE_WAVES_MATTE : FTN_SHADE_WAVES_OTHER)))) k_wf_shade(RenderParams P, WfBuffers W, int in_q, uint32_t class_mask, uint32_t first ) {
    const DScene& S = P.S;
    uint32_t cbase[WF_NCLASS + 1], ccnt[WF_NCLASS];
    cbase[0] = 0;
#pragma unroll
    for (int k = 0; k < WF_NCLASS; k++) { ccnt[k] = ((class_mask >> k) & 1u) ? W.cls[CTR(k)] : 0u; cbase[k + 1] = cbase[k] + ((ccnt[k] + 255u) & ~255u); }
    const uint32_t count = cbase[WF_NCLASS];
    uint32_t* out_q = W.q_active[in_q ^ 1];
    uint32_t* out_count = &W.counters[CTR(in_q == 0 ? 1 : 0)];
    int err = 0;
    const uint32_t stride = gridDim.x * 256u;
    const uint32_t rounds = (count + stride - 1) / stride;
    for (uint32_t round = 0; round < rounds; round++) {
        const uint32_t qi = round * stride + blockIdx.x * 256u + threadIdx.x;
        bool have = false;
        uint32_t sorted_idx = 0;
        if (qi < count) {
            uint32_t c = 0, cb = 0, cc = ccnt[0];
#pragma unroll
            for (int k = 1; k < WF_NCLASS; k++) if (qi >= cbase[k]) { c = (uint32_t)k; cb = cbase[k]; cc = ccnt[k]; }
            have = qi - cb < cc;
            sorted_idx = c * W.seg_cap + (qi - cb);
        }
        bool push_active = false, push_closest = false, push_mis = false, push_shadow = false, push_mis_any = false;
        uint32_t p = 0, active_entry = 0;
        if (have) {
            p = W.q_sorted[sorted_idx];
            float4 bq = make_float4(1.0f, 1.0f, 1.0f, __uint_as_float(PS_ALIVE)), lq = make_float4(0.0f, 0.0f, 0.0f, 0.0f);
            if (!first) { if (W.br) { bq = W.br[2 * (size_t)p]; lq = W.br[2 * (size_t)p + 1]; } else { bq = W.beta[p]; lq = W.rad[p]; } }
            Rgb beta(bq.x, bq.y, bq.z), L(lq.x, lq.y, lq.z);
            uint32_t ps = __float_as_uint(bq.w);
            if (ps & PS_DIRECT) {
                float4 q0, q1, q2, q3 = make_float4(0.0f, 0.0f, 0.0f, 0.0f);
                if (W.pd) { const float4* Q = W.pd + 4 * (size_t)p; q0 = Q[0]; q1 = Q[1]; q2 = Q[2]; if (W.pd_md) q3 = Q[3]; } else { q0 = W.pend0[p]; q1 = W.pend1[p]; q2 = W.pend2[p]; }
                const uint32_t occ_word = __float_as_uint(q3.w);
                Rgb radiance(0.0f);
                if ((ps & PS_SHADOW) && !(W.pd_occ ? (occ_word & 0xffu) != 0u : W.occluded[p] != 0)) radiance = radiance + Rgb(q0.x, q0.y, q0.z);
                if (ps & PS_MIS_ANY) {
                    const int light_index = (int)__float_as_uint(lq.w);
                    const DLight& Lt = ENV ? S.env0 : S.lights[light_index];
                    const float4 md = W.pd_md ? q3 : W.ray[2 * (size_t)(p + W.n_paths) + 1];
                    Rgb inc(0.0f);
                    if (!(W.pd_occ ? (occ_word & 0xff00u) != 0u : W.occluded[p + W.n_paths] != 0)) inc = light_Le_env(Lt, V3(md.x, md.y, md.z));
                    if (!inc.is_black()) radiance = radiance + Rgb(q1.x, q1.y, q1.z) * inc * q0.w / q1.w;
                } else if (ps & PS_MIS) {
                    const int light_index = (int)__float_as_uint(lq.w);
                    const DLight& Lt = ENV ? S.env0 : S.lights[light_index];
                    const DHit mh = load_hit(W, p + W.n_paths);
                    const float4 mo = W.ray[2 * (size_t)(p + W.n_paths)], md = W.ray[2 * (size_t)(p + W.n_paths) + 1];
                    Rgb inc(0.0f);
                    if (mh.prim >= 0) {
                      if (!ENV) {
                        int h_mat, h_light; prim_mat_light(S, mh.prim, &h_mat, &h_light);
                        if (h_light >= 0 && h_light == light_index) {
                            DRay r0; r0.o = V3(mo.x, mo.y, mo.z); r0.d = V3(md.x, md.y, md.z); r0.t_max = FTN_INF; r0.time = 0.0f;
                            DSI s2; make_interaction(S, mh, r0, &s2);
                            inc = area_Le(Lt, s2.hit.n, -r0.d);
                        }
                      }
                    } else if (ENV || Lt.kind == LK_INFINITE) inc = light_Le_env(Lt, V3(md.x, md.y, md.z));
                    if (!inc.is_black()) radiance = radiance + Rgb(q1.x, q1.y, q1.z) * inc * q0.w / q1.w;
                }
                Rgb direct = Rgb(q2.x, q2.y, q2.z) * ((float)S.n_lights * radiance);
                L = L + direct;
                ps &= ~(PS_DIRECT | PS_SHADOW | PS_MIS | PS_MIS_ANY);
            }
            if (!(ps & PS_ALIVE)) {
                W.rad[p] = make_float4(L.r, L.g, L.b, 0.0f);
            } else {
                DRay ray0; ray0.o = V3(0.0f, 0.0f, 0.0f); ray0.d = V3(0.0f, 0.0f, 1.0f); ray0.t_max = FTN_INF; ray0.time = 0.0f;
                DHit h; h.t = FTN_INF; h.b0 = 0.0f; h.b1 = 0.0f; h.b2 = 0.0f; h.prim = -1;
                bool need_ray = true;
                if (MT == -2 && !first) { h.prim = W.hit_prim[p]; need_ray = h.prim >= 0 || (ps & PS_BOUNCE_MASK) == 0u || (ps & PS_SPECULAR) != 0u; }
                if (need_ray) {
                    const float4 ro = W.ray[2 * (size_t)(p)], rdv = W.ray[2 * (size_t)(p) + 1];
                    ray0.o = V3(ro.x, ro.y, ro.z); ray0.d = V3(rdv.x, rdv.y, rdv.z); ray0.t_max = rdv.w;
                    h = load_hit(W, p);
                }
                const bool hit = h.prim >= 0;
                uint32_t bounces = ps & PS_BOUNCE_MASK;
                const bool specular_bounce = (ps & PS_SPECULAR) != 0;
                DSI si;
                if (hit) make_interaction(S, h, ray0, &si);
                if (bounces == 0 || specular_bounce) {
                    if (hit) {
                        Rgb e(0.0f);
                        if (!ENV && si.light >= 0) e = area_Le(S.lights[si.light], si.hit.n, -ray0.d);
                        L = L + beta * e;
                    } else L = L + beta * (ENV ? Rgb(0.0f) + light_Le_env(S.env0, ray0.d) : scene_env_Le(S, ray0.d));
                }
                bool alive = true;
                uint32_t light_word = 0;
                if (!hit || bounces >= P.max_depth) alive = false;
                else {
                    Rng rng;
                    if (first) {
                        const uint32_t slot = p / W.samples, sidx = p % W.samples;
                        const DTile tile = P.tiles[slot >> 8];
                        rng.seed(indexed_key(P.seed, tile.x0 + (int)(slot & 15u), tile.y0 + (int)((slot >> 4) & 15u), W.first_sample + sidx));
                        (void)rng.next2(); (void)rng.next2(); (void)rng.next();
                    } else if (W.rng_replay) {
                        const uint32_t slot = p / W.samples, sidx = p % W.samples;
                        const DTile tile = P.tiles[slot >> 8];
                        rng.seed(indexed_key(P.seed, tile.x0 + (int)(slot & 15u), tile.y0 + (int)((slot >> 4) & 15u), W.first_sample + sidx));
                        rng.skip(ps >> PS_DRAWS_SHIFT);
                    } else { ulonglong2 a = W.rng01[p], b = W.rng23[p]; rng.s0 = a.x; rng.s1 = a.y; rng.s2 = b.x; rng.s3 = b.y; }
                    uint32_t n_draws = first ? 5u : (ps >> PS_DRAWS_SHIFT);
                    const int mat = si.mat;
                    if (MT == -2 || mat < 0) {
                        DRay nr = spawn_ray(si.hit, ray0.d);
                        W.ray[2 * (size_t)(p)] = make_float4(nr.o.x, nr.o.y, nr.o.z, 0.0f); W.ray[2 * (size_t)(p) + 1] = make_float4(nr.d.x, nr.d.y, nr.d.z, nr.t_max);
                        push_closest = true;
                    } else {
                        DBsdf B;
                        ftn_material mloc; const ftn_material* mp = &S.materials[mat];
                        if (TEX && material_is_textured(S, mat)) {
                            DRayDiff rd;
                            if (W.serial) {
                                const float4 d0 = W.dfd[p], d1 = W.dfd[(size_t)W.n_paths + p], d2 = W.dfd[2 * (size_t)W.n_paths + p];
                                rd.has = true; rd.rxo = V3(d0.x, d0.y, d0.z); rd.ryo = V3(d1.x, d1.y, d1.z); rd.ryd = V3(d2.x, d2.y, d2.z); rd.rxd = V3(d0.w, d1.w, d2.w);
                            } else {
                                const uint32_t slot = p / W.samples, sidx = p % W.samples;
                                const DTile tile = P.tiles[slot >> 8];
                                const int px = tile.x0 + (int)(slot & 15u), py = tile.y0 + (int)((slot >> 4) & 15u);
                                Rng crng; crng.seed(indexed_key(P.seed, px, py, W.first_sample + sidx));
                                const V2 j = crng.next2(); const V2 p_film((float)px + j.x, (float)py + j.y); const V2 p_lens = crng.next2(); const float time_u = crng.next();
                                const DRay cam = camera_ray(P.C, p_film, p_lens, time_u);
                                rd = camera_ray_diff(P.C, p_film, p_lens, cam, 1.0f / sqrtf((float)P.spp));
                            }
                            DSIX ex; DSI s2; make_interaction(S, h, ray0, &s2, &ex);
                            const DTexDiffs td = compute_tex_diffs(si.hit.p, si.hit.n, ex.dpdu, ex.dpdv, rd);
                            mloc = material_resolve(S, mat, ex.uv, td); mp = &mloc;
                        }
                        if (!make_bsdf<(MT >= 0 ? MT : -1)>(*mp, si, true, &B)) { err = FTN_ERR_UNSUPPORTED; alive = false; }
                        else {
                            if (bsdf_num(B, T_ALL & ~T_SPECULAR) > 0 && S.n_lights > 0) {
                                const uint32_t nl = S.n_lights;
                                const uint32_t ln = (uint32_t)f2usize(fmin_(rng.next() * (float)nl, (float)(nl - 1)));
                                const V2 ul = rng.next2(), us = rng.next2();
                                n_draws += 5u;
                                const DLight& Lt = ENV ? S.env0 : S.lights[ln];
                                const uint32_t flags = T_ALL & ~T_SPECULAR;
                                const bool delta = !ENV && (Lt.kind == LK_POINT || Lt.kind == LK_DISTANT);
                                ps |= PS_DIRECT; light_word = ln;
                                Rgb ld(0.0f); float mis_w = 0.0f, mis_pdf = 1.0f; Rgb mis_f(0.0f); V3 mis_d(0.0f, 0.0f, 0.0f);
                                DLiSample ls = ENV ? light_sample_env(Lt, si.hit, ul) : light_sample(S, Lt, si.hit, ul);
                                if (ls.pdf > 0.0f && !ls.radiance.is_black()) {
                                    Rgb f = bsdf_f(B, si.wo, ls.wi, flags) * abs_dot(ls.wi, si.shading_n);
                                    float sp = bsdf_pdf(B, si.wo, ls.wi, flags);
                                    if (!f.is_black()) {
                                        DRay sr = spawn_ray_to_hit(si.hit, ls.p1);
                                        W.sh[2 * (size_t)(p)] = make_float4(sr.o.x, sr.o.y, sr.o.z, 0.0f); W.sh[2 * (size_t)(p) + 1] = make_float4(sr.d.x, sr.d.y, sr.d.z, sr.t_max);
                                        ld = delta ? (f * ls.radiance / ls.pdf) : (f * ls.radiance * power_heuristic(ls.pdf, sp) / ls.pdf);
                                        ps |= PS_SHADOW; push_shadow = true;
                                    }
                                }
                                if (!delta) {
                                    DScatter sc;
                                    if (bsdf_sample(B, si.wo, us, flags, &sc)) {
                                        Rgb f = sc.f * abs_dot(sc.wi, si.shading_n);
                                        if (!f.is_black()) {
                                            bool go = true;
                                            if (sc.type & T_SPECULAR) mis_w = 1.0f;
                                            else {
                                                float lp = ENV ? light_pdf_env(Lt, sc.wi) : light_pdf(S, Lt, si.hit, sc.wi);
                                                if (lp == 0.0f) go = false; else mis_w = power_heuristic(sc.pdf, lp);
                                            }
                                            if (go) {
                                                DRay mr = spawn_ray(si.hit, sc.wi);
                                                W.ray[2 * (size_t)(p + W.n_paths)] = make_float4(mr.o.x, mr.o.y, mr.o.z, 0.0f);
                                                W.ray[2 * (size_t)(p + W.n_paths) + 1] = make_float4(mr.d.x, mr.d.y, mr.d.z, mr.t_max);
                                                mis_f = f; mis_pdf = sc.pdf; mis_d = mr.d;
                                                if (W.mis_any && (ENV || Lt.kind == LK_INFINITE)) { ps |= PS_MIS_ANY; push_mis_any = true; } else { ps |= PS_MIS; push_mis = true; }
                                            }
                                        }
                                    }
                                }
                                if (W.pd) {
                                    float4* Q = W.pd + 4 * (size_t)p;
                                    Q[0] = make_float4(ld.r, ld.g, ld.b, mis_w); Q[1] = make_float4(mis_f.r, mis_f.g, mis_f.b, mis_pdf); Q[2] = make_float4(beta.r, beta.g, beta.b, 0.0f);
                                    if (W.pd_md) Q[3] = make_float4(mis_d.x, mis_d.y, mis_d.z, 0.0f);
                                } else {
                                    W.pend0[p] = make_float4(ld.r, ld.g, ld.b, mis_w);
                                    W.pend1[p] = make_float4(mis_f.r, mis_f.g, mis_f.b, mis_pdf);
                                    W.pend2[p] = make_float4(beta.r, beta.g, beta.b, 0.0f);
                                }
                            }
                            DScatter bs;
                            const V2 u = rng.next2();
                            n_draws += 2u;
                            const bool ok = bsdf_sample(B, -ray0.d, u, T_ALL, &bs);
                            if (ok && !bs.f.is_black()) {
                                beta = beta * (bs.f * abs_dot(bs.wi, si.shading_n) / bs.pdf);
                                ps = (bs.type & T_SPECULAR) ? (ps | PS_SPECULAR) : (ps & ~PS_SPECULAR);
                                DRay nr = spawn_ray(si.hit, bs.wi);
                                if (beta.max_component() < P.rr_threshold && bounces > 3) {
                                    float q = fmax_(0.05f, 1.0f - beta.max_component());
                                    n_draws += 1u;
                                    if (rng.next() < q) alive = false; else beta = beta / (1.0f - q);
                                }
                                if (alive) {
                                    W.ray[2 * (size_t)(p)] = make_float4(nr.o.x, nr.o.y, nr.o.z, 0.0f); W.ray[2 * (size_t)(p) + 1] = make_float4(nr.d.x, nr.d.y, nr.d.z, nr.t_max);
                                    bounces += 1; push_closest = true;
                                }
                            } else alive = false;
                        }
                    }
                    if (W.rng_replay) ps = (ps & ((1u << PS_DRAWS_SHIFT) - 1u)) | (n_draws << PS_DRAWS_SHIFT);
                    else if (alive || W.serial) { W.rng01[p] = make_ulonglong2(rng.s0, rng.s1); W.rng23[p] = make_ulonglong2(rng.s2, rng.s3); }
                }
                ps = (ps & ~(PS_BOUNCE_MASK | PS_ALIVE)) | (bounces & PS_BOUNCE_MASK) | (alive ? PS_ALIVE : 0u);
                push_active = alive || (ps & PS_DIRECT);
                if (W.br) {
                    if (push_active) { W.br[2 * (size_t)p] = make_float4(beta.r, beta.g, beta.b, __uint_as_float(ps)); W.br[2 * (size_t)p + 1] = make_float4(L.r, L.g, L.b, __uint_as_float(light_word)); }
                    else W.rad[p] = make_float4(L.r, L.g, L.b, 0.0f);
                } else {
                    if (push_active) W.beta[p] = make_float4(beta.r, beta.g, beta.b, __uint_as_float(ps));
                    W.rad[p] = make_float4(L.r, L.g, L.b, __uint_as_float(light_word));
                }
                active_entry = p | (alive ? (bounces >= P.max_depth ? WF_Q_DEPTH : 0u) : WF_Q_FIN);
            }
            if (W.serial && !push_active) W.ser_retired[p] = 1;
        }
        {
            const bool pred[6] = {push_active, push_closest, push_mis, push_shadow, push_mis_any, push_mis_any};
            const uint32_t val[6] = {active_entry, p, p | WF_MIS_BIT, p, p | WF_MIS_BIT, 0u};
            uint32_t* const qs[6] = {out_q, W.q_closest, W.q_closest, W.q_shadow, W.q_shadow, nullptr};
            uint32_t* const cs[6] = {out_count, &W.counters[CTR(2)], &W.counters[CTR(2)], &W.counters[CTR(3)], &W.counters[CTR(3)], &W.counters[CTR(10)]};
            block_push<6>(pred, val, qs, cs);
        }
    }
    if (err) atomicCAS(&P.stats->error, 0, err);
}

template <bool TEX, int MT, bool ENV> static unsigned shade_wgs_per_cu() {
    static const unsigned nb = [] { int v = 0; return (hipOccupancyMaxActiveBlocksPerMultiprocessor(&v, k_wf_shade<TEX, MT, ENV>, 256, 0) == hipSuccess && v >= 1) ? (unsigned)(v > 8 ? 8 : v) : 3u; }();
    return nb;
}

#define WF_DL_MAX 8u
#define WF_WH_MAX_LIGHTS 32u
__device__ inline void dl_unwind(const RenderParams& P, const WfBuffers& W, uint32_t p, uint32_t depth, bool have_tail, Rgb tail) {
    Rgb li = have_tail ? tail : Rgb(0.0f);
    bool child = have_tail;
    for (int d = (int)depth - 1; d >= 0; d--) {
        const float4 a = W.dlA[(size_t)d * W.n_paths + p];
        Rgb r(a.x, a.y, a.z);
        if (child) { const float4 b = W.dlB[(size_t)d * W.n_paths + p]; r = r + Rgb(b.x, b.y, b.z) * li * b.w / a.w; }
        else if ((uint32_t)d + 1 < P.max_depth) r = r + Rgb(0.0f);
        if ((uint32_t)d + 1 < P.max_depth) r = r + Rgb(0.0f);
        li = r; child = true;
    }
    W.rad[p] = make_float4(li.r, li.g, li.b, 0.0f);
}

template <bool WHITTED, bool TEX>
__global__ void __launch_bounds__(256) k_wf_shade_dl(RenderParams P, WfBuffers W, int in_q) {
    const DScene& S = P.S;
    uint32_t cbase[WF_NCLASS + 1], ccnt[WF_NCLASS];
    cbase[0] = 0;
#pragma unroll
    for (int k = 0; k < WF_NCLASS; k++) { ccnt[k] = W.cls[CTR(k)]; cbase[k + 1] = cbase[k] + ((ccnt[k] + 255u) & ~255u); }
    const uint32_t count = cbase[WF_NCLASS];
    uint32_t* out_q = W.q_active[in_q ^ 1];
    uint32_t* out_count = &W.counters[CTR(in_q == 0 ? 1 : 0)];
    int err = 0;
    const uint32_t stride = gridDim.x * 256u;
    const uint32_t rounds = (count + stride - 1) / stride;
    const uint32_t nl = S.n_lights;
    for (uint32_t round = 0; round < rounds; round++) {
        const uint32_t qi = round * stride + blockIdx.x * 256u + threadIdx.x;
        bool have = false; uint32_t sorted_idx = 0;
        if (qi < count) {
            uint32_t c = 0, cb = 0, cc = ccnt[0];
#pragma unroll
            for (int k = 1; k < WF_NCLASS; k++) if (qi >= cbase[k]) { c = (uint32_t)k; cb = cbase[k]; cc = ccnt[k]; }
            have = qi - cb < cc;
            sorted_idx = c * W.seg_cap + (qi - cb);
        }
        bool push_active = false, push_closest = false, push_mis = false, push_mis_any = false;
        uint32_t sh_mask = 0;
        uint32_t p = 0, active_entry = 0;
        if (have) {
            p = W.q_sorted[sorted_idx];
            const float4 bq = W.beta[p], lq = W.rad[p];
            uint32_t ps = __float_as_uint(bq.w);
            uint32_t depth = ps & PS_BOUNCE_MASK;
            if (ps & PS_DIRECT) {
                const uint32_t lv = depth - 1u;
                float4 a = W.dlA[(size_t)lv * W.n_paths + p];
                Rgb rad(a.x, a.y, a.z);
                if (WHITTED) {
                    const uint32_t mask = __float_as_uint(lq.w);
                    for (uint32_t l = 0; l < nl; l++) if ((mask >> l) & 1u) {
                        const float4 t = W.whT[(size_t)l * W.n_paths + p];
                        if (!W.occluded[p + (size_t)l * W.n_paths]) rad = rad + Rgb(t.x, t.y, t.z);
                    }
                } else {
                    const float4 q0 = W.pend0[p], q1 = W.pend1[p];
                    Rgb radiance(0.0f);
                    if ((ps & PS_SHADOW) && !W.occluded[p]) radiance = radiance + Rgb(q0.x, q0.y, q0.z);
                    const int light_index = (int)__float_as_uint(lq.w);
                    const DLight& Lt = S.lights[light_index];
                    if (ps & PS_MIS_ANY) {
                        const float4 md = W.ray[2 * (size_t)(p + W.n_paths) + 1];
                        Rgb inc(0.0f);
                        if (!W.occluded[p + W.n_paths]) inc = light_Le_env(Lt, V3(md.x, md.y, md.z));
                        if (!inc.is_black()) radiance = radiance + Rgb(q1.x, q1.y, q1.z) * inc * q0.w / q1.w;
                    } else if (ps & PS_MIS) {
                        const DHit mh = load_hit(W, p + W.n_paths);
                        const float4 mo = W.ray[2 * (size_t)(p + W.n_paths)], md = W.ray[2 * (size_t)(p + W.n_paths) + 1];
                        Rgb inc(0.0f);
                        if (mh.prim >= 0) {
                            int h_mat, h_light; prim_mat_light(S, mh.prim, &h_mat, &h_light);
                            if (h_light >= 0 && h_light == light_index) {
                                DRay r0; r0.o = V3(mo.x, mo.y, mo.z); r0.d = V3(md.x, md.y, md.z); r0.t_max = FTN_INF; r0.time = 0.0f;
                                DSI s2; make_interaction(S, mh, r0, &s2);
                                inc = area_Le(Lt, s2.hit.n, -r0.d);
                            }
                        } else if (Lt.kind == LK_INFINITE) inc = light_Le_env(Lt, V3(md.x, md.y, md.z));
                        if (!inc.is_black()) radiance = radiance + Rgb(q1.x, q1.y, q1.z) * inc * q0.w / q1.w;
                    }
                    rad = rad + (float)nl * radiance;
                }
                a.x = rad.r; a.y = rad.g; a.z = rad.b;
                W.dlA[(size_t)lv * W.n_paths + p] = a;
                ps &= ~(PS_DIRECT | PS_SHADOW | PS_MIS | PS_MIS_ANY);
            }
            if (!(ps & PS_ALIVE)) {
                dl_unwind(P, W, p, depth, false, Rgb(0.0f));
                W.beta[p] = make_float4(0.0f, 0.0f, 0.0f, __uint_as_float(ps));
            } else {
                const float4 ro = W.ray[2 * (size_t)(p)], rdv = W.ray[2 * (size_t)(p) + 1];
                DRay ray0; ray0.o = V3(ro.x, ro.y, ro.z); ray0.d = V3(rdv.x, rdv.y, rdv.z); ray0.t_max = rdv.w; ray0.time = 0.0f;
                const DHit h = load_hit(W, p);
                bool alive = false; uint32_t light_word = 0; bool ended = false;
                if (h.prim < 0) { dl_unwind(P, W, p, depth, true, scene_env_Le(S, ray0.d)); ended = true; }
                else if (depth >= WF_DL_MAX) { err = FTN_ERR_UNSUPPORTED; ended = true; }
                else {
                    DSI si; make_interaction(S, h, ray0, &si);
                    DBsdf B;
                    ftn_material mloc; const ftn_material* mp = si.mat >= 0 ? &S.materials[si.mat] : nullptr;
                    DSIX ex; DTexDiffs td; float bsdf_eta = 1.0f; DRayDiff rd; rd.has = false;
                    if (TEX && mp) {
                        if (depth == 0u) {
                            const uint32_t slot = p / W.samples, sidx = p % W.samples;
                            const DTile tile = P.tiles[slot >> 8];
                            const int px = tile.x0 + (int)(slot & 15u), py = tile.y0 + (int)((slot >> 4) & 15u);
                            Rng crng; crng.seed(indexed_key(P.seed, px, py, W.first_sample + sidx));
                            const V2 j = crng.next2(); const V2 p_film((float)px + j.x, (float)py + j.y); const V2 p_lens = crng.next2(); const float time_u = crng.next();
                            const DRay cam = camera_ray(P.C, p_film, p_lens, time_u);
                            rd = camera_ray_diff(P.C, p_film, p_lens, cam, 1.0f / sqrtf((float)P.spp));
                        } else {
                            const float4 d0 = W.dfd[p], d1 = W.dfd[(size_t)W.n_paths + p], d2 = W.dfd[2 * (size_t)W.n_paths + p];
                            rd.has = true; rd.rxo = V3(d0.x, d0.y, d0.z); rd.ryo = V3(d1.x, d1.y, d1.z); rd.ryd = V3(d2.x, d2.y, d2.z); rd.rxd = V3(d0.w, d1.w, d2.w);
                        }
                        DSI s2; make_interaction(S, h, ray0, &s2, &ex);
                        td = compute_tex_diffs(si.hit.p, si.hit.n, ex.dpdu, ex.dpdv, rd);
                        if (material_is_textured(S, si.mat)) { mloc = material_resolve(S, si.mat, ex.uv, td); mp = &mloc; }
                        if (mp->type == FTN_MAT_GLASS) bsdf_eta = mp->s0;
                    }
                    if (!mp || !make_bsdf<-1>(*mp, si, false, &B)) { err = FTN_ERR_UNSUPPORTED; ended = true; }
                    else {
                        Rng rng; { ulonglong2 a = W.rng01[p], b = W.rng23[p]; rng.s0 = a.x; rng.s1 = a.y; rng.s2 = b.x; rng.s3 = b.y; }
                        Rgb rad(0.0f);
                        if (WHITTED) {
                            uint32_t mask = 0;
                            if (nl > WF_WH_MAX_LIGHTS) err = FTN_ERR_UNSUPPORTED;
                            else for (uint32_t l = 0; l < nl; l++) {
                                const DLight& Lt = S.lights[l];
                                DLiSample ls = light_sample(S, Lt, si.hit, rng.next2());
                                if (ls.radiance.is_black() || ls.pdf == 0.0f) continue;
                                Rgb f = bsdf_f(B, si.wo, ls.wi, T_ALL);
                                if (!f.is_black()) {
                                    DRay sr = spawn_ray_to_hit(si.hit, ls.p1);
                                    const size_t slot = p + (size_t)l * W.n_paths;
                                    W.sh[2 * slot] = make_float4(sr.o.x, sr.o.y, sr.o.z, 0.0f); W.sh[2 * slot + 1] = make_float4(sr.d.x, sr.d.y, sr.d.z, sr.t_max);
                                    const Rgb term = f * ls.radiance * abs_dot(ls.wi, si.shading_n) / ls.pdf;
                                    W.whT[slot] = make_float4(term.r, term.g, term.b, 0.0f);
                                    mask |= 1u << l;
                                }
                            }
                            if (mask) { ps |= PS_DIRECT; light_word = mask; sh_mask = mask; }
                        } else {
                            if (si.light >= 0) rad = rad + area_Le(S.lights[si.light], si.hit.n, si.wo);
                            else rad = rad + Rgb(0.0f);
                            if (nl > 0) {
                                const uint32_t ln = (uint32_t)f2usize(fmin_(rng.next() * (float)nl, (float)(nl - 1)));
                                const V2 ul = rng.next2(), us = rng.next2();
                                const DLight& Lt = S.lights[ln];
                                const uint32_t flags = T_ALL & ~T_SPECULAR;
                                const bool delta = Lt.kind == LK_POINT || Lt.kind == LK_DISTANT;
                                ps |= PS_DIRECT; light_word = ln;
                                Rgb ld(0.0f); float mis_w = 0.0f, mis_pdf = 1.0f; Rgb mis_f(0.0f);
                                DLiSample ls = light_sample(S, Lt, si.hit, ul);
                                if (ls.pdf > 0.0f && !ls.radiance.is_black()) {
                                    Rgb f = bsdf_f(B, si.wo, ls.wi, flags) * abs_dot(ls.wi, si.shading_n);
                                    float sp = bsdf_pdf(B, si.wo, ls.wi, flags);
                                    if (!f.is_black()) {
                                        DRay sr = spawn_ray_to_hit(si.hit, ls.p1);
                                        W.sh[2 * (size_t)(p)] = make_float4(sr.o.x, sr.o.y, sr.o.z, 0.0f); W.sh[2 * (size_t)(p) + 1] = make_float4(sr.d.x, sr.d.y, sr.d.z, sr.t_max);
                                        ld = delta ? (f * ls.radiance / ls.pdf) : (f * ls.radiance * power_heuristic(ls.pdf, sp) / ls.pdf);
                                        ps |= PS_SHADOW; sh_mask = 1u;
                                    }
                                }
                                if (!delta) {
                                    DScatter sc;
                                    if (bsdf_sample(B, si.wo, us, flags, &sc)) {
                                        Rgb f = sc.f * abs_dot(sc.wi, si.shading_n);
                                        if (!f.is_black()) {
                                            bool go = true;
                                            if (sc.type & T_SPECULAR) mis_w = 1.0f;
                                            else { float lp = light_pdf(S, Lt, si.hit, sc.wi); if (lp == 0.0f) go = false; else mis_w = power_heuristic(sc.pdf, lp); }
                                            if (go) {
                                                DRay mr = spawn_ray(si.hit, sc.wi);
                                                W.ray[2 * (size_t)(p + W.n_paths)] = make_float4(mr.o.x, mr.o.y, mr.o.z, 0.0f);
                                                W.ray[2 * (size_t)(p + W.n_paths) + 1] = make_float4(mr.d.x, mr.d.y, mr.d.z, mr.t_max);
                                                mis_f = f; mis_pdf = sc.pdf;
                                                if (W.mis_any && Lt.kind == LK_INFINITE) { ps |= PS_MIS_ANY; push_mis_any = true; } else { ps |= PS_MIS; push_mis = true; }
                                            }
                                        }
                                    }
                                }
                                W.pend0[p] = make_float4(ld.r, ld.g, ld.b, mis_w);
                                W.pend1[p] = make_float4(mis_f.r, mis_f.g, mis_f.b, mis_pdf);
                            }
                        }
                        float4 lvA = make_float4(rad.r, rad.g, rad.b, 1.0f), lvB = make_float4(0.0f, 0.0f, 0.0f, 0.0f);
                        if (depth + 1u < P.max_depth) {
                            const V2 ur = rng.next2();
                            DScatter sr;
                            const bool has_r = bsdf_sample(B, si.wo, ur, T_REFL | T_SPECULAR, &sr) && !(abs_dot(sr.wi, si.shading_n) == 0.0f);
                            const bool has_t = bsdf_num(B, T_TRANS | T_SPECULAR) > 0;
                            if (has_t) err = FTN_ERR_UNSUPPORTED;
                            else if (has_r) {
                                lvA.w = sr.pdf; lvB = make_float4(sr.f.r, sr.f.g, sr.f.b, fabsf(dot(sr.wi, si.shading_n)));
                                if (TEX) {
                                    rd = specular_diff(true, rd, si.hit.p, si.wo, sr.wi, si.shading_n, ex.dndu, ex.dndv, td, bsdf_eta);
                                    W.dfd[p] = make_float4(rd.rxo.x, rd.rxo.y, rd.rxo.z, rd.rxd.x); W.dfd[(size_t)W.n_paths + p] = make_float4(rd.ryo.x, rd.ryo.y, rd.ryo.z, rd.rxd.y);
                                    W.dfd[2 * (size_t)W.n_paths + p] = make_float4(rd.ryd.x, rd.ryd.y, rd.ryd.z, rd.rxd.z);
                                }
                                DRay nr = spawn_ray(si.hit, sr.wi);
                                W.ray[2 * (size_t)(p)] = make_float4(nr.o.x, nr.o.y, nr.o.z, 0.0f); W.ray[2 * (size_t)(p) + 1] = make_float4(nr.d.x, nr.d.y, nr.d.z, nr.t_max);
                                alive = true; push_closest = true;
                            }
                        }
                        W.dlA[(size_t)depth * W.n_paths + p] = lvA; W.dlB[(size_t)depth * W.n_paths + p] = lvB;
                        depth += 1u;
                        W.rng01[p] = make_ulonglong2(rng.s0, rng.s1); W.rng23[p] = make_ulonglong2(rng.s2, rng.s3);
                        if (!alive && !(ps & PS_DIRECT)) { dl_unwind(P, W, p, depth, false, Rgb(0.0f)); ended = true; }
                    }
                }
                if (err && !ended) ended = true;
                if (ended) { alive = false; ps &= ~(PS_DIRECT | PS_SHADOW | PS_MIS | PS_MIS_ANY); sh_mask = 0; push_closest = push_mis = push_mis_any = false; if (err) W.rad[p] = make_float4(0.0f, 0.0f, 0.0f, 0.0f); }
                ps = (ps & ~(PS_BOUNCE_MASK | PS_ALIVE)) | (depth & PS_BOUNCE_MASK) | (alive ? PS_ALIVE : 0u);
                W.beta[p] = make_float4(0.0f, 0.0f, 0.0f, __uint_as_float(ps));
                if (!ended) W.rad[p] = make_float4(0.0f, 0.0f, 0.0f, __uint_as_float(light_word));
                push_active = alive || (ps & PS_DIRECT);
                active_entry = p | (alive ? 0u : WF_Q_FIN);
            }
        }
        {
            const bool pred[5] = {push_active, push_closest, push_mis, push_mis_any, push_mis_any};
            const uint32_t val[5] = {active_entry, p, p | WF_MIS_BIT, p | WF_MIS_BIT, 0u};
            uint32_t* const qs[5] = {out_q, W.q_closest, W.q_closest, W.q_shadow, nullptr};
            uint32_t* const cs[5] = {out_count, &W.counters[CTR(2)], &W.counters[CTR(2)], &W.counters[CTR(3)], &W.counters[CTR(10)]};
            block_push<5>(pred, val, qs, cs);
        }
        for (uint32_t l = 0; l < (WHITTED ? nl : 1u); l++) {
            const bool on = ((sh_mask >> l) & 1u) != 0;
            const bool pred[1] = {on};
            const uint32_t val[1] = {p + l * W.n_paths};
            uint32_t* const qs[1] = {W.q_shadow};
            uint32_t* const cs[1] = {&W.counters[CTR(3)]};
            if (__syncthreads_or(on ? 1 : 0)) block_push<1>(pred, val, qs, cs);
        }
    }
    if (err) atomicCAS(&P.stats->error, 0, err);
}

__global__ void k_wf_reset(WfBuffers W, int mode, int in_q, DevStats* stats) {
    if (threadIdx.x != 0 || blockIdx.x != 0) return;
    if (mode == 0) {
        for (int i = 0; i < 64; i++) W.counters[CTR(i)] = 0;
#ifdef FTN_DRAIN_PROBE
        for (int k = 0; k < 32; k++) W.counters[CTR(13) + k] = 0;
#endif
        W.counters[CTR(0)] = W.samples * W.valid_per_sample; W.counters[CTR(2)] = W.samples * W.valid_per_sample;
        stats->camera_samples += (unsigned long long)W.samples * W.valid_per_sample;
    } else if (mode == 1) {
        W.counters[CTR(2)] = 0; W.counters[CTR(3)] = 0; W.counters[CTR(in_q == 0 ? 1 : 0)] = 0; W.counters[CTR(11)] = 0;
        for (int i = 16; i < 32; i++) W.counters[CTR(i)] = 0;
        for (int i = 32; i < 56; i++) W.counters[CTR(i)] = 0;
    } else if (mode == 2) {
        for (int i = 0; i < WF_NCLASS; i++) W.cls[CTR(i)] = 0;
    } else if (mode == 3) {
        for (int i = 0; i < 64; i++) W.counters[CTR(i)] = 0;
    }
}

struct FilmCtxW { int crop[4]; int tpb[4]; int sb[4]; float radius[2]; };
#define WF_OWN_SERIAL (-2147483647 - 1)
__device__ inline void wf_film_add(const RenderParams& P, const FilmCtxW& F, V2 p_film, Rgb L, int own_x, int own_y, float4* acc, uint32_t* spill, uint32_t* bc_writes) {
    float pdx = p_film.x - 0.5f, pdy = p_film.y - 0.5f;
    int p0x = f2i_sat(ceilf(pdx - F.radius[0])), p0y = f2i_sat(ceilf(pdy - F.radius[1]));
    int p1x = f2i_sat(floorf(pdx + F.radius[0])) + 1, p1y = f2i_sat(floorf(pdy + F.radius[1])) + 1;
    p0x = max(p0x, F.tpb[0]); p0y = max(p0y, F.tpb[1]); p1x = min(p1x, F.tpb[2]); p1y = min(p1y, F.tpb[3]);
    const Rgb contrib = L * 1.0f * 1.0f;
    int touched = 0;
    const size_t width = (size_t)(F.crop[2] - F.crop[0]);
    for (int y = p0y; y < p1y; y++)
        for (int x = p0x; x < p1x; x++) {
            touched++;
            if (x == own_x && y == own_y) { acc->x += contrib.r; acc->y += contrib.g; acc->z += contrib.b; acc->w += 1.0f; continue; }
            const bool in_tile = x >= F.sb[0] && x < F.sb[2] && y >= F.sb[1] && y < F.sb[3];
            if (in_tile && own_x == WF_OWN_SERIAL) {
                float4* a = P.accA + ((size_t)(y - F.crop[1]) * width + (size_t)(x - F.crop[0]));
                float4 v = *a; v.x += contrib.r; v.y += contrib.g; v.z += contrib.b; v.w += 1.0f; *a = v;
                continue;
            }
            float* f = reinterpret_cast<float*>((in_tile ? P.accB : P.accC) + ((size_t)(y - F.crop[1]) * width + (size_t)(x - F.crop[0])));
            atomicAdd(f + 0, contrib.r); atomicAdd(f + 1, contrib.g); atomicAdd(f + 2, contrib.b); atomicAdd(f + 3, 1.0f);
            (*bc_writes)++;
        }
    if (touched != 1) (*spill)++;
}
#define WF_ACC_CHUNK 8u
__global__ void __launch_bounds__(256) k_wf_accumulate(RenderParams P, WfBuffers W) {
    __shared__ float4 s_rad[256 * WF_ACC_CHUNK];
    const uint32_t slot = blockIdx.x * 256u + threadIdx.x;
    uint32_t spill = 0, bc = 0, cam = 0; int err = 0;
    bool valid = false, in_crop = false; int px = 0, py = 0; size_t ai = 0;
    FilmCtxW F; float4 acc = make_float4(0.0f, 0.0f, 0.0f, 0.0f);
    if (slot < W.n_slots) {
        const DTile tile = P.tiles[slot >> 8];
        px = tile.x0 + (int)(slot & 15u); py = tile.y0 + (int)((slot >> 4) & 15u);
        if (px < tile.x1 && py < tile.y1) {
            valid = true;
            for (int i = 0; i < 4; i++) F.crop[i] = P.crop[i];
            F.sb[0] = tile.x0; F.sb[1] = tile.y0; F.sb[2] = tile.x1; F.sb[3] = tile.y1; F.radius[0] = P.radius[0]; F.radius[1] = P.radius[1];
            int p0x = f2i_sat(ceilf((float)tile.x0 - 0.5f - P.radius[0])), p0y = f2i_sat(ceilf((float)tile.y0 - 0.5f - P.radius[1]));
            int p1x = f2i_sat(ceilf((float)tile.x1 - 0.5f + P.radius[0] + 1.0f)), p1y = f2i_sat(ceilf((float)tile.y1 - 0.5f - P.radius[1] + 1.0f));
            F.tpb[0] = max(p0x, P.crop[0]); F.tpb[1] = max(p0y, P.crop[1]); F.tpb[2] = min(p1x, P.crop[2]); F.tpb[3] = min(p1y, P.crop[3]);
            in_crop = px >= P.crop[0] && px < P.crop[2] && py >= P.crop[1] && py < P.crop[3];
            ai = in_crop ? ((size_t)(py - P.crop[1]) * (size_t)(P.crop[2] - P.crop[0]) + (size_t)(px - P.crop[0])) : 0;
            if (in_crop) acc = P.accA[ai];
        }
    }
    const size_t block_first = (size_t)blockIdx.x * 256u * W.samples;
    for (uint32_t s0 = 0; s0 < W.samples; s0 += WF_ACC_CHUNK) {
        const uint32_t n = W.samples - s0 < WF_ACC_CHUNK ? W.samples - s0 : WF_ACC_CHUNK;
        for (uint32_t e = threadIdx.x; e < 256u * n; e += 256u) {
            const uint32_t sl = e / n, k = e - sl * n;
            const size_t p = block_first + (size_t)sl * W.samples + s0 + k;
            if (p < W.n_paths) s_rad[sl * WF_ACC_CHUNK + k] = W.rad[p];
        }
        __syncthreads();
        if (valid) {
            for (uint32_t k = 0; k < n; k++) {
                const float4 l = s_rad[threadIdx.x * WF_ACC_CHUNK + k];
                Rgb L(l.x, l.y, l.z);
                if (L.has_nans()) err = FTN_ERR_NAN_RADIANCE;
                Rng crng; crng.seed(indexed_key(P.seed, px, py, W.first_sample + s0 + k));
                const V2 j = crng.next2();
                wf_film_add(P, F, V2((float)px + j.x, (float)py + j.y), L, in_crop ? px : (-2147483647), py, &acc, &spill, &bc);
                cam++;
            }
        }
        __syncthreads();
    }
    if (valid && in_crop) P.accA[ai] = acc;
    (void)cam;
    if (spill) atomicAdd(&P.stats->spill_samples, (unsigned long long)spill);
    if (bc) atomicAdd(&P.stats->bc_writes, (unsigned long long)bc);
    if (err) atomicCAS(&P.stats->error, 0, err);
}

template <bool TEX>
__global__ void __launch_bounds__(256) k_wf_serial_advance(RenderParams P, WfBuffers W, int out_q, int init) {
    const uint32_t t = blockIdx.x * 256u + threadIdx.x;
    bool push = false;
    uint32_t spill = 0, bc = 0, cam = 0; int err = 0;
    if (t < W.n_paths) {
        const DTile tile = P.tiles[t];
        const uint32_t tw = (uint32_t)(tile.x1 - tile.x0), npix = tw * (uint32_t)(tile.y1 - tile.y0);
        Rng rng; uint2 cur = make_uint2(0u, 0u); bool start = false;
        if (init) { rng.seed(tile.tile_id); start = npix > 0u && P.spp > 0u; W.ser_retired[t] = 0; }
        else if (W.ser_retired[t]) {
            W.ser_retired[t] = 0;
            { const ulonglong2 a = W.rng01[t], b = W.rng23[t]; rng.s0 = a.x; rng.s1 = a.y; rng.s2 = b.x; rng.s3 = b.y; }
            cur = W.ser_cursor[t];
            const float4 l = W.rad[t]; const float2 pf = W.ser_pfilm[t];
            Rgb L(l.x, l.y, l.z);
            if (L.has_nans()) err = FTN_ERR_NAN_RADIANCE;
            FilmCtxW F;
            for (int i = 0; i < 4; i++) F.crop[i] = P.crop[i];
            F.sb[0] = tile.x0; F.sb[1] = tile.y0; F.sb[2] = tile.x1; F.sb[3] = tile.y1; F.radius[0] = P.radius[0]; F.radius[1] = P.radius[1];
            const int p0x = f2i_sat(ceilf((float)tile.x0 - 0.5f - P.radius[0])), p0y = f2i_sat(ceilf((float)tile.y0 - 0.5f - P.radius[1]));
            const int p1x = f2i_sat(ceilf((float)tile.x1 - 0.5f + P.radius[0] + 1.0f)), p1y = f2i_sat(ceilf((float)tile.y1 - 0.5f - P.radius[1] + 1.0f));
            F.tpb[0] = max(p0x, P.crop[0]); F.tpb[1] = max(p0y, P.crop[1]); F.tpb[2] = min(p1x, P.crop[2]); F.tpb[3] = min(p1y, P.crop[3]);
            float4 none = make_float4(0.0f, 0.0f, 0.0f, 0.0f);
            wf_film_add(P, F, V2(pf.x, pf.y), L, WF_OWN_SERIAL, 0, &none, &spill, &bc);
            cam = 1;
            if (++cur.y == P.spp) { cur.y = 0; cur.x++; }
            start = cur.x < npix;
        }
        if (start) {
            const int px = tile.x0 + (int)(cur.x % tw), py = tile.y0 + (int)(cur.x / tw);
            const V2 j = rng.next2();
            const V2 p_film((float)px + j.x, (float)py + j.y);
            const V2 p_lens = rng.next2();
            const float time_u = rng.next();
            const DRay ray = camera_ray(P.C, p_film, p_lens, time_u);
            W.ray[2 * (size_t)t] = make_float4(ray.o.x, ray.o.y, ray.o.z, 0.0f);
            W.ray[2 * (size_t)t + 1] = make_float4(ray.d.x, ray.d.y, ray.d.z, ray.t_max);
            W.beta[t] = make_float4(1.0f, 1.0f, 1.0f, __uint_as_float(PS_ALIVE));
            W.rad[t] = make_float4(0.0f, 0.0f, 0.0f, 0.0f);
            W.rng01[t] = make_ulonglong2(rng.s0, rng.s1); W.rng23[t] = make_ulonglong2(rng.s2, rng.s3);
            W.ser_cursor[t] = cur; W.ser_pfilm[t] = make_float2(p_film.x, p_film.y);
            if (TEX) {
                const DRayDiff rd = camera_ray_diff(P.C, p_film, p_lens, ray, 1.0f / sqrtf((float)P.spp));
                W.dfd[t] = make_float4(rd.rxo.x, rd.rxo.y, rd.rxo.z, rd.rxd.x); W.dfd[(size_t)W.n_paths + t] = make_float4(rd.ryo.x, rd.ryo.y, rd.ryo.z, rd.rxd.y);
                W.dfd[2 * (size_t)W.n_paths + t] = make_float4(rd.ryd.x, rd.ryd.y, rd.ryd.z, rd.rxd.z);
            }
            push = true;
        }
    }
    {
        const bool pred[2] = {push, push};
        const uint32_t val[2] = {t | (P.max_depth == 0 ? WF_Q_DEPTH : 0u), t};
        uint32_t* const qs[2] = {W.q_active[out_q], W.q_closest};
        uint32_t* const cs[2] = {&W.counters[CTR(out_q == 0 ? 0 : 1)], &W.counters[CTR(2)]};
        block_push<2>(pred, val, qs, cs);
    }
    if (cam) atomicAdd(&P.stats->camera_samples, (unsigned long long)cam);
    if (spill) atomicAdd(&P.stats->spill_samples, (unsigned long long)spill);
    if (bc) atomicAdd(&P.stats->bc_writes, (unsigned long long)bc);
    if (err) atomicCAS(&P.stats->error, 0, err);
}

static thread_local std::string g_wf_err;
const char* wavefront_error() { return g_wf_err.c_str(); }

__device__ inline uint32_t spread3(uint32_t v) {
    v &= 0x3ffu; v = (v | (v << 16)) & 0x030000ffu; v = (v | (v << 8)) & 0x0300f00fu; v = (v | (v << 4)) & 0x030c30c3u; v = (v | (v << 2)) & 0x09249249u; return v;
}
template <bool ANY>
__global__ void __launch_bounds__(256) k_wf_ray_keys(DScene S, WfBuffers W, const uint32_t* __restrict__ queue, uint32_t count, uint32_t* __restrict__ keys, uint32_t bits) {
    const uint32_t i = blockIdx.x * 256u + threadIdx.x;
    if (i >= count) return;
    float4 a, b; uint32_t slot;
    load_queued_ray<ANY>(W, queue[i], &a, &b, &slot);
    const float ex = S.root_hi[0] - S.root_lo[0], ey = S.root_hi[1] - S.root_lo[1], ez = S.root_hi[2] - S.root_lo[2];
    const float sc = (float)(1u << bits);
    const float fx = fminf(fmaxf((a.x - S.root_lo[0]) / ex, 0.0f), 0.999f) * sc, fy = fminf(fmaxf((a.y - S.root_lo[1]) / ey, 0.0f), 0.999f) * sc, fz = fminf(fmaxf((a.z - S.root_lo[2]) / ez, 0.0f), 0.999f) * sc;
    const uint32_t m = spread3((uint32_t)fx) | (spread3((uint32_t)fy) << 1) | (spread3((uint32_t)fz) << 2);
    const uint32_t oct = (b.x < 0.0f ? 1u : 0u) | (b.y < 0.0f ? 2u : 0u) | (b.z < 0.0f ? 4u : 0u);
    keys[i] = (m << 3) | oct;
}

struct WavefrontState {
    void* sort_tmp = nullptr; size_t sort_tmp_bytes = 0;
    size_t cap_paths = 0;
    void* mem[40]; int n_mem = 0;
    WfBuffers W;
    float4* br = nullptr; float4* pd = nullptr;
    hipEvent_t ev[64]; int n_ev = 0;
    hipStream_t side = nullptr; hipEvent_t ev_ready = nullptr, ev_side = nullptr;
    uint32_t* drain_sig = nullptr; uint32_t drain_seq = 0;
    uint32_t* host_counters = nullptr;
    int n_cu = 256;
    void* dl_mem[8] = {nullptr, nullptr, nullptr, nullptr, nullptr, nullptr, nullptr, nullptr}; size_t dl_paths = 0; uint32_t dl_levels = 0, dl_slots = 0; bool dl_tex = false;
    Trace4Plan t4; bool t4_on = false, t8_on = false, q64_on = false;
    void* ser_mem[4] = {nullptr, nullptr, nullptr, nullptr}; size_t ser_paths = 0; bool ser_tex = false; uint32_t* ser_host = nullptr;
    void* t4_spill_c = nullptr; void* t4_spill_a = nullptr; size_t t4_spill_c_bytes = 0, t4_spill_a_bytes = 0;
};
#define WF_TRY(expr) do { hipError_t e_ = (expr); if (e_ != hipSuccess) { g_wf_err = std::string(#expr ": ") + hipGetErrorString(e_); return e_ == hipErrorOutOfMemory ? FTN_ERR_OUT_OF_MEMORY : FTN_ERR_NO_DEVICE; } } while (0)

static void wf_free(WavefrontState* st) { for (int i = 0; i < st->n_mem; i++) (void)hipFree(st->mem[i]); st->n_mem = 0; st->cap_paths = 0; }
void wavefront_destroy(WavefrontState* st) {
    if (!st) return;
    wf_free(st);
    if (st->sort_tmp) (void)hipFree(st->sort_tmp);
    for (int i = 0; i < st->n_ev; i++) (void)hipEventDestroy(st->ev[i]);
    if (st->ev_ready) (void)hipEventDestroy(st->ev_ready);
    if (st->ev_side) (void)hipEventDestroy(st->ev_side);
    if (st->side) (void)hipStreamDestroy(st->side);
    if (st->drain_sig) (void)hipFree(st->drain_sig);
    for (void* m : st->dl_mem) if (m) (void)hipFree(m);
    for (void* m : st->ser_mem) if (m) (void)hipFree(m);
    if (st->t4_spill_c) (void)hipFree(st->t4_spill_c);
    if (st->t4_spill_a) (void)hipFree(st->t4_spill_a);
    if (st->host_counters) (void)hipHostFree(st->host_counters);
    if (st->ser_host) (void)hipHostFree(st->ser_host);
    delete st;
}
template <class T> static int wf_alloc(WavefrontState* st, T** p, size_t n) {
    WF_TRY(hipMalloc((void**)p, n * sizeof(T)));
    st->mem[st->n_mem++] = (void*)*p;
    return FTN_OK;
}
static int wf_reserve(WavefrontState* st, size_t n) {
    if (n <= st->cap_paths) return FTN_OK;
    wf_free(st);
    WfBuffers& W = st->W; int rc;
    if ((rc = wf_alloc(st, &W.ray, 4 * n)) || (rc = wf_alloc(st, &W.hit, 2 * n)) || (rc = wf_alloc(st, &W.hit_prim, 2 * n)) ||
        (rc = wf_alloc(st, &W.sh, 2 * n)) || (rc = wf_alloc(st, &W.occluded, 2 * n)) || (rc = wf_alloc(st, &W.beta, n)) || (rc = wf_alloc(st, &W.rad, n)) ||
        (rc = wf_alloc(st, &W.rng01, n)) || (rc = wf_alloc(st, &W.rng23, n)) || (rc = wf_alloc(st, &W.pend0, n)) || (rc = wf_alloc(st, &W.pend1, n)) || (rc = wf_alloc(st, &W.pend2, n)) ||
        (rc = wf_alloc(st, &W.q_active[0], n)) || (rc = wf_alloc(st, &W.q_active[1], n)) || (rc = wf_alloc(st, &W.q_closest, 2 * n)) || (rc = wf_alloc(st, &W.q_shadow, 2 * n)) || (rc = wf_alloc(st, &W.q_sorted, 8 * n)) || (rc = wf_alloc(st, &W.cls, 8 * 32)) ||
        (rc = wf_alloc(st, &W.q_exc_closest, 2 * n)) || (rc = wf_alloc(st, &W.q_exc_any, 2 * n)) || (rc = wf_alloc(st, &W.counters, 64 * 32)) || (rc = wf_alloc(st, &st->br, 2 * n)) || (rc = wf_alloc(st, &st->pd, 4 * n))) return rc;
    st->cap_paths = n;
    return FTN_OK;
}

#include <unordered_map>
static thread_local std::unordered_map<std::string, std::pair<bool, uint32_t>> g_knobs;
static void knobs_begin() { g_knobs.clear(); }
static uint32_t knob(const char* name, uint32_t def) {
    auto it = g_knobs.find(name);
    if (it == g_knobs.end()) { const char* v = getenv(name); it = g_knobs.emplace(name, std::make_pair(v != nullptr, v ? (uint32_t)atoi(v) : 0u)).first; }
    return it->second.first ? it->second.second : def;
}

static int sort_ray_queue(WavefrontState* st, const RenderParams& P, const WfBuffers& W, bool any, uint32_t* queue, uint32_t cnt, uint32_t* out,
                          uint32_t* k_in, uint32_t* k_out, uint32_t bits, hipStream_t stream, const uint32_t** sorted_q) {
    *sorted_q = queue;
    if (cnt < knob("FTN_WF_SORT_MIN", 16384u)) return FTN_OK;
    if (any) hipLaunchKernelGGL(k_wf_ray_keys<true>, dim3((cnt + 255) / 256), dim3(256), 0, stream, P.S, W, queue, cnt, k_in, bits);
    else hipLaunchKernelGGL(k_wf_ray_keys<false>, dim3((cnt + 255) / 256), dim3(256), 0, stream, P.S, W, queue, cnt, k_in, bits);
    const int end_bit = (int)(3 * bits + 3);
    size_t need = 0;
    hipcub::DoubleBuffer<uint32_t> keys(k_in, k_out), vals(queue, out);
    WF_TRY(hipcub::DeviceRadixSort::SortPairs(nullptr, need, keys, vals, (int)cnt, 0, end_bit, stream));
    if (need > st->sort_tmp_bytes) { if (st->sort_tmp) (void)hipFree(st->sort_tmp); st->sort_tmp = nullptr; st->sort_tmp_bytes = 0; WF_TRY(hipMalloc(&st->sort_tmp, need)); st->sort_tmp_bytes = need; }
    WF_TRY(hipcub::DeviceRadixSort::SortPairs(st->sort_tmp, need, keys, vals, (int)cnt, 0, end_bit, stream));
    *sorted_q = vals.Current();
    return FTN_OK;
}


#ifdef FTN_DRAIN_PROBE
static uint32_t g_probe_bounce = 0;
#endif
static int trace4_prepare(WavefrontState* st, const DScene& S) {
    st->t4_on = S.quad != nullptr && knob("FTN_TRACE4", 1) != 0;
    if (!st->t4_on) return FTN_OK;
    st->t4 = trace4_plan(S, st->n_cu, knob("FTN_T4_ENTRIES", 0), knob("FTN_T4_ENTRIES_ANY", 0), knob("FTN_T4_WG", 0), knob("FTN_T4_WG_ANY", 0), knob("FTN_T8_WG", 0), knob("FTN_T8_ENTRIES", 0));
    st->q64_on = st->t4.q64_ok && S.n_spheres == 0 && knob("FTN_QUAD64", 1) != 0;
    const size_t need_c = std::max<size_t>((size_t)st->t4.grid_closest * 256u * st->t4.spill_closest * sizeof(uint2),
                                           st->q64_on ? (size_t)st->t4.grid_q64 * 256u * st->t4.spill_q64 * sizeof(uint2) : 0);
    st->t8_on = st->t4.oct_ok && S.n_spheres == 0 && knob("FTN_T8", 1) != 0;
    const size_t need_a8 = st->t8_on ? (size_t)st->t4.grid_oct * 256u * st->t4.spill_oct * sizeof(uint32_t) : 0;
    const size_t need_a = std::max<size_t>(need_a8, (size_t)st->t4.grid_any * 256u * st->t4.spill_any * sizeof(uint32_t));
    if (need_c > st->t4_spill_c_bytes) { if (st->t4_spill_c) (void)hipFree(st->t4_spill_c); st->t4_spill_c = nullptr; st->t4_spill_c_bytes = 0; WF_TRY(hipMalloc(&st->t4_spill_c, need_c)); st->t4_spill_c_bytes = need_c; }
    if (need_a > st->t4_spill_a_bytes) { if (st->t4_spill_a) (void)hipFree(st->t4_spill_a); st->t4_spill_a = nullptr; st->t4_spill_a_bytes = 0; WF_TRY(hipMalloc(&st->t4_spill_a, need_a)); st->t4_spill_a_bytes = need_a; }
    return FTN_OK;
}

static void launch_trace(WavefrontState* st, bool any, int count, bool spheres, unsigned grid, size_t lds, hipStream_t stream, const RenderParams& P, const WfBuffers& W,
                         const uint32_t* queue, const uint32_t* count_ptr, uint32_t* head, uint32_t max_rays, bool camera_rays = false) {
    if (st->t4_on && count != 1) {
        const Trace4Plan& T = st->t4;
        const bool oct = any && st->t8_on, q64 = !any && st->q64_on;
        const unsigned g = std::min<unsigned>(oct ? T.grid_oct : (any ? T.grid_any : (q64 ? T.grid_q64 : T.grid_closest)), std::max<unsigned>(1u, (max_rays + 255u) / 256u));
        uint32_t chunk4 = knob("FTN_TRACE_CHUNK", 128);
        while (chunk4 > 64u && (uint64_t)chunk4 * g * 4u * 4u > (uint64_t)max_rays) chunk4 >>= 1;
        if (oct) launch_trace4(T4K_ANY_OCT, count == 2, false, g, T.lds_oct, T.entries_oct, st->t4_spill_a, stream, P.S, W, queue, count_ptr, head, P.stats,
                               camera_rays ? knob("FTN_T8_REFILL1", 16) : knob("FTN_T8_REFILL", 24), camera_rays ? knob("FTN_T8_LEAF_BATCH1", 16) : knob("FTN_T8_LEAF_BATCH", 16), chunk4, knob("FTN_T8_BURST", 2), knob("FTN_T8_POLICY", 1), T.spill_oct);
        else launch_trace4(any ? T4K_ANY : (q64 ? T4K_CLOSEST_Q64 : T4K_CLOSEST), count == 2, spheres, g, any ? T.lds_any : (q64 ? T.lds_q64 : T.lds_closest),
                      any ? T.entries_any : (q64 ? T.entries_q64 : T.entries_closest), any ? st->t4_spill_a : st->t4_spill_c, stream, P.S, W,
                      queue, count_ptr, head, P.stats,
                      any ? knob("FTN_T4_ANY_REFILL", 32) : (camera_rays ? knob("FTN_T4_REFILL0", 64) : knob("FTN_T4_REFILL", 32)),
                      any ? knob("FTN_T4_ANY_LEAF_BATCH", 16) : (camera_rays ? knob("FTN_T4_LEAF_BATCH0", 2) : knob("FTN_T4_LEAF_BATCH", 16)), chunk4,
                      any ? knob("FTN_T4_ANY_BURST", 4) : (camera_rays ? knob("FTN_T4_BURST0", 3) : knob("FTN_T4_BURST", 2)), knob("FTN_T4_ANY_POLICY", 1), any ? T.spill_any : (q64 ? T.spill_q64 : T.spill_closest));
        const unsigned ge = std::min<unsigned>(grid, (unsigned)st->n_cu);
        uint32_t* ecount = &W.counters[CTR(any ? 33 : 32)]; uint32_t* ehead = &W.counters[CTR(any ? 48 : 40)];
        DevStats* none = nullptr;
#define FTN_TRE(A, Sp) hipLaunchKernelGGL((k_wf_trace<A, false, Sp, 8>), dim3(ge), dim3(256), lds, stream, P.S, W, any ? W.q_exc_any : W.q_exc_closest, ecount, ehead, none, 24u, 2u, 64u, 8u)
        if (any) { if (spheres) FTN_TRE(true, true); else FTN_TRE(true, false); } else { if (spheres) FTN_TRE(false, true); else FTN_TRE(false, false); }
#undef FTN_TRE
        return;
    }
    const bool count_b = count != 0;
    const uint32_t refill = knob("FTN_TRACE_REFILL", 24), leaf_batch = knob("FTN_TRACE_LEAF_BATCH", 2), chunk_knob = knob("FTN_TRACE_CHUNK", 128), node_burst = knob("FTN_TRACE_BURST", 8);
    uint32_t chunk = chunk_knob;
    const uint32_t waves = grid * 4u;
    while (chunk > 64u && (uint64_t)chunk * waves * 4u > (uint64_t)max_rays) chunk >>= 1;
    if (any && !count_b && knob("FTN_TRACE_ANY2", 1) && P.S.fat) {
        const uint32_t refill2 = knob("FTN_ANY2_REFILL", 16), leaf_batch2 = knob("FTN_ANY2_LEAF_BATCH", leaf_batch);
        uint32_t policy2 = knob("FTN_ANY2_POLICY", 2);
#ifdef FTN_DRAIN_PROBE
        policy2 |= g_probe_bounce << 8;
#endif
        if (spheres) hipLaunchKernelGGL((k_wf_trace_any2<true>), dim3(grid), dim3(256), lds, stream, P.S, W, queue, count_ptr, head, P.stats, refill2, leaf_batch2, chunk, policy2);
        else hipLaunchKernelGGL((k_wf_trace_any2<false>), dim3(grid), dim3(256), lds, stream, P.S, W, queue, count_ptr, head, P.stats, refill2, leaf_batch2, chunk, policy2);
        return;
    }
    lds += knob("FTN_TRACE_LDS_PAD", 0);
#define FTN_TR(A, C, Sp, B) hipLaunchKernelGGL((k_wf_trace<A, C, Sp, B>), dim3(grid), dim3(256), lds, stream, P.S, W, queue, count_ptr, head, P.stats, refill, leaf_batch, chunk, node_burst)
    const bool fixed = node_burst == 8 && !count_b && !knob("FTN_TRACE_NO_UNROLL", 0);
    if (fixed) { if (any) { if (spheres) FTN_TR(true, false, true, 8); else FTN_TR(true, false, false, 8); } else { if (spheres) FTN_TR(false, false, true, 8); else FTN_TR(false, false, false, 8); } }
    else if (any) { if (count_b) { if (spheres) FTN_TR(true, true, true, 0); else FTN_TR(true, true, false, 0); } else { if (spheres) FTN_TR(true, false, true, 0); else FTN_TR(true, false, false, 0); } }
    else { if (count_b) { if (spheres) FTN_TR(false, true, true, 0); else FTN_TR(false, true, false, 0); } else { if (spheres) FTN_TR(false, false, true, 0); else FTN_TR(false, false, false, 0); } }
#undef FTN_TR
}

static void wf_free_dl(WavefrontState* st) { for (void*& m : st->dl_mem) { if (m) (void)hipFree(m); m = nullptr; } st->dl_paths = 0; st->dl_levels = 0; st->dl_slots = 0; st->dl_tex = false; }
static int wf_reserve_dl(WavefrontState* st, size_t n, uint32_t levels, uint32_t slots, bool tex) {
    if (n <= st->dl_paths && levels <= st->dl_levels && slots <= st->dl_slots && (!tex || st->dl_tex)) return FTN_OK;
    wf_free_dl(st);
    const size_t sl = std::max<uint32_t>(slots, 2u);
    WF_TRY(hipMalloc(&st->dl_mem[0], (size_t)levels * n * sizeof(float4)));
    WF_TRY(hipMalloc(&st->dl_mem[1], (size_t)levels * n * sizeof(float4)));
    WF_TRY(hipMalloc(&st->dl_mem[2], (size_t)slots * n * sizeof(float4)));
    WF_TRY(hipMalloc(&st->dl_mem[3], 2 * (size_t)slots * n * sizeof(float4)));
    WF_TRY(hipMalloc(&st->dl_mem[4], sl * n));
    WF_TRY(hipMalloc(&st->dl_mem[5], sl * n * sizeof(uint32_t)));
    WF_TRY(hipMalloc(&st->dl_mem[6], sl * n * sizeof(uint32_t)));
    if (tex) WF_TRY(hipMalloc(&st->dl_mem[7], 3 * n * sizeof(float4)));
    st->dl_paths = n; st->dl_levels = levels; st->dl_slots = slots; st->dl_tex = tex;
    return FTN_OK;
}

static int wf_state_init(WavefrontState** state) {
    if (*state) return FTN_OK;
    *state = new WavefrontState();
    for (int i = 0; i < 64; i++) { WF_TRY(hipEventCreate(&(*state)->ev[i])); (*state)->n_ev = i + 1; }
    {
        int least = 0, greatest = 0;
        WF_TRY(hipDeviceGetStreamPriorityRange(&least, &greatest));
        WF_TRY(hipStreamCreateWithPriority(&(*state)->side, hipStreamNonBlocking, knob("FTN_WF_SIDE_PRIO", 1) ? least : 0));
    }
    WF_TRY(hipEventCreateWithFlags(&(*state)->ev_ready, hipEventDisableTiming));
    WF_TRY(hipEventCreateWithFlags(&(*state)->ev_side, hipEventDisableTiming));
    {
        int dev = 0, can = 0;
        WF_TRY(hipGetDevice(&dev));
        if (hipDeviceGetAttribute(&can, hipDeviceAttributeCanUseStreamWaitValue, dev) == hipSuccess && can) {
            if (hipExtMallocWithFlags((void**)&(*state)->drain_sig, 8, hipMallocSignalMemory) != hipSuccess) { (void)hipGetLastError(); (*state)->drain_sig = nullptr; }
            else WF_TRY(hipMemset((*state)->drain_sig, 0, 8));
        }
    }
    WF_TRY(hipHostMalloc((void**)&(*state)->host_counters, 16 * 32 * sizeof(uint32_t)));
    hipDeviceProp_t prop; int dev = 0; WF_TRY(hipGetDevice(&dev)); WF_TRY(hipGetDeviceProperties(&prop, dev));
    (*state)->n_cu = prop.multiProcessorCount > 0 ? prop.multiProcessorCount : 256;
    return FTN_OK;
}

__global__ void __launch_bounds__(256) k_batch_setup(const float* __restrict__ rays8, uint32_t n, float4* __restrict__ ray, uint32_t* __restrict__ queue) {
    const uint32_t i = blockIdx.x * 256u + threadIdx.x;
    if (i >= n) return;
    const float* r = rays8 + 8 * (size_t)i;
    ray[2 * (size_t)i] = make_float4(r[0], r[1], r[2], r[7]);
    ray[2 * (size_t)i + 1] = make_float4(r[3], r[4], r[5], r[6]);
    queue[i] = i;
}
__global__ void __launch_bounds__(256) k_batch_finish(DScene S, const float* __restrict__ rays8, uint32_t n, const float4* __restrict__ hit, const int* __restrict__ hit_prim,
                                                      float* t_hit, int* prim, float* bary, float* out24) {
    const uint32_t i = blockIdx.x * 256u + threadIdx.x;
    if (i >= n) return;
    const float4 h4 = hit[i]; const int hp = hit_prim[i];
    if (t_hit) t_hit[i] = hp >= 0 ? h4.x : FTN_INF;
    if (prim) prim[i] = hp;
    if (bary) { bary[3 * (size_t)i] = hp >= 0 ? h4.y : 0.0f; bary[3 * (size_t)i + 1] = hp >= 0 ? h4.z : 0.0f; bary[3 * (size_t)i + 2] = hp >= 0 ? h4.w : 0.0f; }
    if (out24) {
        float* o = out24 + 24 * (size_t)i;
        if (hp < 0) { for (int k = 0; k < 24; k++) o[k] = 0.0f; o[23] = -1.0f; }
        else {
            const float* r = rays8 + 8 * (size_t)i;
            DRay ray0; ray0.o = V3(r[0], r[1], r[2]); ray0.d = V3(r[3], r[4], r[5]); ray0.t_max = r[6]; ray0.time = r[7];
            DHit h; h.t = h4.x; h.b0 = h4.y; h.b1 = h4.z; h.b2 = h4.w; h.prim = hp;
            DSI si; make_interaction(S, h, ray0, &si);
            o[0] = si.hit.p.x; o[1] = si.hit.p.y; o[2] = si.hit.p.z; o[3] = si.hit.p_err.x; o[4] = si.hit.p_err.y; o[5] = si.hit.p_err.z;
            o[6] = si.hit.n.x; o[7] = si.hit.n.y; o[8] = si.hit.n.z; o[9] = 0.0f; o[10] = 0.0f;
            o[11] = si.wo.x; o[12] = si.wo.y; o[13] = si.wo.z; o[14] = si.s_dpdu.x; o[15] = si.s_dpdu.y; o[16] = si.s_dpdu.z;
            o[17] = 0.0f; o[18] = 0.0f; o[19] = 0.0f; o[20] = si.shading_n.x; o[21] = si.shading_n.y; o[22] = si.shading_n.z; o[23] = h.t;
        }
    }
}
int wavefront_trace_batch(WavefrontState** state, const DScene& S, uint32_t stack_entries, const float* d_rays8, size_t n_rays, int mode, bool count,
                          float* t_hit, int* prim, float* bary, unsigned char* occluded, float* out24, DevStats* stats, hipStream_t stream) {
    if (n_rays == 0) return FTN_OK;
    if (n_rays >= (1ull << 31)) { g_wf_err = "too many rays in one batch"; return FTN_ERR_INVALID_ARGUMENT; }
    knobs_begin();
    int rc = wf_state_init(state); if (rc) return rc;
    WavefrontState* st = *state;
    if ((rc = trace4_prepare(st, S))) return rc;
    const uint32_t n = (uint32_t)n_rays;
    const bool any = mode == 1;
    float4 *ray = nullptr, *hit = nullptr; int* hit_prim = nullptr; uint32_t *queue = nullptr, *scratch = nullptr, *counters = nullptr, *q_exc = nullptr;
    auto cleanup = [&]() { (void)hipFree(ray); (void)hipFree(hit); (void)hipFree(hit_prim); (void)hipFree(queue); (void)hipFree(scratch); (void)hipFree(counters); (void)hipFree(q_exc); };
#define WFB_TRY(expr) do { hipError_t e_ = (expr); if (e_ != hipSuccess) { g_wf_err = std::string(#expr ": ") + hipGetErrorString(e_); cleanup(); return e_ == hipErrorOutOfMemory ? FTN_ERR_OUT_OF_MEMORY : FTN_ERR_NO_DEVICE; } } while (0)
    WFB_TRY(hipMalloc((void**)&ray, (size_t)n * 32)); WFB_TRY(hipMalloc((void**)&queue, (size_t)n * 4)); WFB_TRY(hipMalloc((void**)&scratch, (size_t)n * 12));
    WFB_TRY(hipMalloc((void**)&counters, 64 * 32 * 4)); WFB_TRY(hipMemsetAsync(counters, 0, 64 * 32 * 4, stream));
    WFB_TRY(hipMalloc((void**)&q_exc, (size_t)n * 4));
    if (!any) { WFB_TRY(hipMalloc((void**)&hit, (size_t)n * 16)); WFB_TRY(hipMalloc((void**)&hit_prim, (size_t)n * 4)); }
    hipLaunchKernelGGL(k_batch_setup, dim3((n + 255) / 256), dim3(256), 0, stream, d_rays8, n, ray, queue);
    WFB_TRY(hipMemcpyAsync(&counters[CTR(any ? 3 : 2)], &n, 4, hipMemcpyHostToDevice, stream));
    WfBuffers W; memset(&W, 0, sizeof(W));
    W.n_paths = n; W.ray = ray; W.sh = ray; W.hit = hit; W.hit_prim = hit_prim; W.occluded = occluded; W.counters = counters; W.q_exc_closest = q_exc; W.q_exc_any = q_exc;
    RenderParams P; memset(&P, 0, sizeof(P)); P.S = S; P.stats = stats;
    const uint32_t* q = queue;
    if (knob("FTN_WF_SORT", 0)) { rc = sort_ray_queue(st, P, W, any, queue, n, scratch, scratch + n, scratch + 2 * (size_t)n, 7, stream, &q); if (rc) { cleanup(); return rc; } }
    const size_t lds = (size_t)stack_entries * 256 * sizeof(uint32_t);
    const unsigned per_cu = (unsigned)std::max<size_t>(1, std::min<size_t>(8, (size_t)(160 * 1024) / std::max<size_t>(lds, 1)));
    const unsigned grid = std::min<unsigned>((unsigned)st->n_cu * per_cu, (n + 255) / 256);
    launch_trace(st, any, count ? 1 : 0, S.n_spheres != 0, grid, lds, stream, P, W, q, &counters[CTR(any ? 3 : 2)], &counters[CTR(any ? 24 : 16)], n);
    if (!any) hipLaunchKernelGGL(k_batch_finish, dim3((n + 255) / 256), dim3(256), 0, stream, S, d_rays8, n, hit, hit_prim, t_hit, prim, bary, out24);
    WFB_TRY(hipStreamSynchronize(stream));
    WFB_TRY(hipGetLastError());
#undef WFB_TRY
    cleanup();
    return FTN_OK;
}

static int wavefront_render_serial(WavefrontState* st, const RenderParams& P, uint32_t n_tiles, bool count, bool count_production, hipStream_t stream, WavefrontTimes* times) {
    int rc = wf_reserve(st, (size_t)std::max<uint32_t>(n_tiles, 256u));
    if (rc) { wf_free(st); return rc; }
    const bool tex = P.S.n_textures != 0;
    if (n_tiles > st->ser_paths || (tex && !st->ser_tex)) {
        for (void*& m : st->ser_mem) { if (m) (void)hipFree(m); m = nullptr; }
        st->ser_paths = 0;
        WF_TRY(hipMalloc(&st->ser_mem[0], (size_t)n_tiles * sizeof(uint2)));
        WF_TRY(hipMalloc(&st->ser_mem[1], (size_t)n_tiles * sizeof(float2)));
        WF_TRY(hipMalloc(&st->ser_mem[2], (size_t)n_tiles));
        if (tex) WF_TRY(hipMalloc(&st->ser_mem[3], 3 * (size_t)n_tiles * sizeof(float4)));
        st->ser_paths = n_tiles; st->ser_tex = tex;
    }
    if ((rc = trace4_prepare(st, P.S))) return rc;
    WfBuffers W = st->W;
    W.serial = 1; W.ser_cursor = (uint2*)st->ser_mem[0]; W.ser_pfilm = (float2*)st->ser_mem[1]; W.ser_retired = (unsigned char*)st->ser_mem[2]; W.dfd = (float4*)st->ser_mem[3];
    W.n_slots = 0; W.samples = 1; W.n_paths = n_tiles; W.first_sample = 0; W.seg_cap = (uint32_t)st->cap_paths; W.valid_per_sample = 0;
    W.gen_blocks = 0; W.rng_replay = 0; W.br = nullptr; W.pd = nullptr; W.pd_md = 0; W.pd_occ = 0;
    const int count_mode = count ? (count_production ? 2 : 1) : 0;
    W.mis_any = ((!count || count_production) && knob("FTN_MIS_ANY", 1)) ? 1u : 0u;
    const bool spheres = P.S.n_spheres != 0;
    const size_t lds = (size_t)P.stack_entries * 256 * sizeof(uint32_t);
    const unsigned blocks_per_cu = (unsigned)std::max<size_t>(1, std::min<size_t>(8, (size_t)(160 * 1024) / std::max<size_t>(lds, 1)));
    const unsigned tg = std::min<unsigned>((unsigned)st->n_cu * blocks_per_cu, (2 * n_tiles + 255) / 256);
    const dim3 pgrid((n_tiles + 255) / 256), sgrid(std::min<unsigned>((unsigned)st->n_cu * 8u, (n_tiles + 255) / 256));
    const bool env = P.S.env_only && knob("FTN_SHADE_ENV", 1);
    hipEvent_t e0 = st->ev[0], e1 = st->ev[1];
    (void)hipEventRecord(e0, stream);
    hipLaunchKernelGGL(k_wf_reset, dim3(1), dim3(64), 0, stream, W, 3, 0, P.stats);
    if (tex) hipLaunchKernelGGL((k_wf_serial_advance<true>), pgrid, dim3(256), 0, stream, P, W, 0, 1); else hipLaunchKernelGGL((k_wf_serial_advance<false>), pgrid, dim3(256), 0, stream, P, W, 0, 1);
    int in_q = 0; unsigned long long rounds = 0, trace_launches = 0;
    if (!st->ser_host) WF_TRY(hipHostMalloc((void**)&st->ser_host, 2 * 16 * 32 * sizeof(uint32_t)));
    int polled_q[2] = {0, 0}; uint32_t* last = st->ser_host;
    const bool side_ok = st->side != nullptr && knob("FTN_WF_OVERLAP", 2) != 0 && getenv("ROCPROF_COUNTER_COLLECTION") == nullptr;
    const uint64_t max_rounds = 256u * (uint64_t)std::max<uint32_t>(P.spp, 1u) * ((uint64_t)P.max_depth + 4u + (1u << 12));
    for (uint64_t it = 0; it < max_rounds; it++) {
        const bool beside = it > 0 && side_ok;
        if (beside) { WF_TRY(hipEventRecord(st->ev_ready, stream)); WF_TRY(hipStreamWaitEvent(st->side, st->ev_ready, 0));
                      launch_trace(st, true, count_mode, spheres, tg, lds, st->side, P, W, W.q_shadow, &W.counters[CTR(3)], &W.counters[CTR(24)], 2 * n_tiles);
                      WF_TRY(hipEventRecord(st->ev_side, st->side)); }
        launch_trace(st, false, count_mode, spheres, tg, lds, stream, P, W, W.q_closest, &W.counters[CTR(2)], &W.counters[CTR(16)], 2 * n_tiles);
        trace_launches++;
        if (it > 0 && !beside) launch_trace(st, true, count_mode, spheres, tg, lds, stream, P, W, W.q_shadow, &W.counters[CTR(3)], &W.counters[CTR(24)], 2 * n_tiles);
        if (beside) WF_TRY(hipStreamWaitEvent(stream, st->ev_side, 0));
        hipLaunchKernelGGL(k_wf_reset, dim3(1), dim3(64), 0, stream, W, 2, in_q, P.stats);
        hipLaunchKernelGGL(k_wf_classify, sgrid, dim3(256), 0, stream, P, W, in_q);
        hipLaunchKernelGGL(k_wf_reset, dim3(1), dim3(64), 0, stream, W, 1, in_q, P.stats);
#define FTN_SH2(T, M, E, mask) hipLaunchKernelGGL((k_wf_shade<T, M, E>), sgrid, dim3(256), 0, stream, P, W, in_q, mask, 0u)
#define FTN_SH(M, mask) do { if (tex) { if (env) FTN_SH2(true, M, true, mask); else FTN_SH2(true, M, false, mask); } \
                             else { if (env) FTN_SH2(false, M, true, mask); else FTN_SH2(false, M, false, mask); } } while (0)
        if (!knob("FTN_SHADE_SPECIALISE", 1)) FTN_SH(-1, 0xffu);
        else {
            FTN_SH(-2, 0x83u);
            if (P.S.material_types & 1u) FTN_SH(0, 1u << 2);
            if (P.S.material_types & 2u) FTN_SH(1, 1u << 3);
            if (P.S.material_types & 4u) FTN_SH(2, 1u << 4);
            if (P.S.material_types & 8u) FTN_SH(3, 1u << 5);
            if (P.S.material_types & 16u) FTN_SH(4, 1u << 6);
        }
#undef FTN_SH2
#undef FTN_SH
        if (tex) hipLaunchKernelGGL((k_wf_serial_advance<true>), pgrid, dim3(256), 0, stream, P, W, in_q ^ 1, 0); else hipLaunchKernelGGL((k_wf_serial_advance<false>), pgrid, dim3(256), 0, stream, P, W, in_q ^ 1, 0);
        in_q ^= 1; rounds++;
        uint32_t* hb = st->ser_host + (it & 1u) * 16u * 32u;
        WF_TRY(hipMemcpyAsync(hb, W.counters, 16 * 32 * sizeof(uint32_t), hipMemcpyDeviceToHost, stream));
        WF_TRY(hipEventRecord(st->ev[2 + (it & 1u)], stream));
        polled_q[it & 1u] = in_q;
        if (it >= 1) {
            const uint32_t k = (uint32_t)((it - 1) & 1u);
            WF_TRY(hipEventSynchronize(st->ev[2 + k]));
            if (st->ser_host[k * 16u * 32u + CTR(polled_q[k] == 0 ? 0 : 1)] == 0) { last = hb; break; }
        }
        last = hb;
    }
    WF_TRY(hipStreamSynchronize(stream));
    memcpy(st->host_counters, last, 16 * 32 * sizeof(uint32_t));
    (void)hipEventRecord(e1, stream);
    WF_TRY(hipEventSynchronize(e1));
    WF_TRY(hipGetLastError());
    if (times) {
        float ms = 0.0f; (void)hipEventElapsedTime(&ms, e0, e1);
        memset(times, 0, sizeof(*times));
        times->trace_launches = trace_launches; times->mis_any_rays = W.mis_any ? st->host_counters[CTR(10)] : 0;
        times->shade_launches = rounds;
        (void)ms;
    }
    return FTN_OK;
}

int wavefront_render(WavefrontState** state, const RenderParams& P0, const std::vector<DTile>& tiles, bool count, hipStream_t stream, WavefrontTimes* times,
                     bool count_production) {
    knobs_begin();
    { int rc0 = wf_state_init(state); if (rc0) return rc0; }
    WavefrontState* st = *state;
    RenderParams P = P0;
    const uint32_t n_slots = (uint32_t)tiles.size() * 256u;
    if (n_slots == 0) return FTN_OK;
    const uint32_t total_samples = P.last_sample - P.first_sample;
    if (total_samples == 0) return FTN_OK;
    if (tiles.size() > ((size_t)1 << 20)) { g_wf_err = "more than 2^20 tiles (2^28 pixel slots) in one call: render the film in several tile ranges"; return FTN_ERR_UNSUPPORTED; }
    if (P.sampler_kind != FTN_SAMPLER_INDEXED) {
        if (P.integrator_kind != FTN_INTEGRATOR_PATH) { g_wf_err = "the tile-serial sampler runs on the queues for PathIntegrator"; return FTN_ERR_UNSUPPORTED; }
        return wavefront_render_serial(st, P, (uint32_t)tiles.size(), count, count_production, stream, times);
    }
    uint32_t S = (uint32_t)std::max<size_t>(1, ((size_t)std::min<uint32_t>(knob("FTN_WF_PATHS_M", 256), 256u) << 20) / n_slots);
    S = std::min(S, total_samples);
    const int count_mode = count ? (count_production ? 2 : 1) : 0;
    const bool dl_mode = P.integrator_kind != FTN_INTEGRATOR_PATH;
    const bool whitted = P.integrator_kind == FTN_INTEGRATOR_WHITTED;
    const bool dl_tex = dl_mode && P.S.n_textures != 0;
    uint32_t dl_levels = 0, dl_slots = 0;
    if (dl_mode) {
        if (whitted && P.S.n_lights > WF_WH_MAX_LIGHTS) { g_wf_err = "the wavefront pipeline runs WhittedIntegrator for up to 32 lights (one bit per light in a path's pending-light word)"; return FTN_ERR_UNSUPPORTED; }
        dl_levels = std::max<uint32_t>(1u, std::min<uint32_t>(P.max_depth, WF_DL_MAX)); dl_slots = whitted ? std::max<uint32_t>(P.S.n_lights, 1u) : 1u;
        const size_t cap = ((size_t)1 << 31) / std::max<uint32_t>(dl_slots, 2u) - 1u;
        S = (uint32_t)std::max<size_t>(1, std::min<size_t>(S, cap / n_slots));
        if ((size_t)n_slots > cap) { g_wf_err = "too many pixel slots for this many lights in one call: render the film in several tile ranges"; return FTN_ERR_UNSUPPORTED; }
    }
    auto reserve = [&](uint32_t samples) -> int {
        int r = wf_reserve(st, (size_t)samples * n_slots);
        if (!r && dl_mode) r = wf_reserve_dl(st, st->cap_paths, dl_levels, dl_slots, dl_tex);
        return r;
    };
    int rc = reserve(S);
    while (rc == FTN_ERR_OUT_OF_MEMORY && S > 1) {
        wf_free(st); wf_free_dl(st); (void)hipGetLastError();
        S = (S + 1) / 2;
        rc = reserve(S);
    }
    if (rc) { wf_free(st); wf_free_dl(st); return rc; }
    if ((rc = trace4_prepare(st, P.S))) return rc;
    if (dl_mode) { st->W.dlA = (float4*)st->dl_mem[0]; st->W.dlB = (float4*)st->dl_mem[1]; st->W.whT = (float4*)st->dl_mem[2]; st->W.dfd = (float4*)st->dl_mem[7]; }
    WfBuffers W = st->W;
    if (dl_mode) { W.sh = (float4*)st->dl_mem[3]; W.occluded = (unsigned char*)st->dl_mem[4]; W.q_shadow = (uint32_t*)st->dl_mem[5]; W.q_exc_any = (uint32_t*)st->dl_mem[6]; }
    if (!knob("FTN_ENV_CELLS_USE", 1)) P.S.env0.cells = nullptr;
    const bool spheres = P.S.n_spheres != 0;
    uint32_t valid = 0; for (const DTile& t : tiles) valid += (uint32_t)((t.x1 - t.x0) * (t.y1 - t.y0));
    W.valid_per_sample = valid;
    W.mis_any = ((!count || count_production) && knob("FTN_MIS_ANY", 1)) ? 1u : 0u;
    W.rng_replay = (!dl_mode && 5u + 8u * ((uint32_t)P.max_depth + 1u) <= 511u && knob("FTN_RNG_REPLAY", 1)) ? 1u : 0u;
    W.br = (!dl_mode && knob("FTN_WF_BR", 1)) ? st->br : nullptr;
    W.pd = (!dl_mode && knob("FTN_WF_PD", 3)) ? st->pd : nullptr;
    W.pd_md = (W.pd && knob("FTN_WF_PD", 3) >= 2) ? 1u : 0u;
    W.pd_occ = (W.pd && knob("FTN_WF_PD", 3) >= 3) ? 1u : 0u;
    W.gen_blocks = knob("FTN_GEN_BLOCKS", 1);
    const size_t lds = (size_t)P.stack_entries * 256 * sizeof(uint32_t);
    const unsigned blocks_per_cu = (unsigned)std::max<size_t>(1, std::min<size_t>(8, (size_t)(160 * 1024) / std::max<size_t>(lds, 1)));
    const unsigned trace_grid_max = (unsigned)st->n_cu * blocks_per_cu;
    const unsigned shade_grid_max = (unsigned)st->n_cu * 8u;
    double trace_ms = 0.0; unsigned long long trace_launches = 0, mis_any_rays = 0;
    double group_ms[4] = {0.0, 0.0, 0.0, 0.0}; unsigned long long group_n[4] = {0, 0, 0, 0};
    const uint32_t overlap_mode = knob("FTN_WF_OVERLAP", 2);
    const bool drain_gate = knob("FTN_WF_DRAIN_GATE", 1) != 0 && getenv("ROCPROF_COUNTER_COLLECTION") == nullptr;
    const uint32_t sort_bits = knob("FTN_WF_SORT", 0) ? std::min<uint32_t>(std::max<uint32_t>(knob("FTN_WF_SORT_BITS", 7), 1u), 9u) : 0u;
    uint32_t n_active = 0;
    int ev_used = 0;
    struct Span { int a, b, kind; };
    std::vector<Span> spans;
    static const char* const kGroup[4] = {"closest-hit trace", "any-hit trace", "classify + shade", "queue sort"};
    auto flush_events = [&]() -> int {
        if (spans.empty()) return FTN_OK;
        for (const Span& s : spans) WF_TRY(hipEventSynchronize(st->ev[s.b]));
        for (const Span& s : spans) {
            float ms = 0.0f; (void)hipEventElapsedTime(&ms, st->ev[s.a], st->ev[s.b]);
            group_ms[s.kind] += ms; group_n[s.kind]++;
            if (s.kind == 0) trace_ms += ms;
            if (knob("FTN_WF_DEBUG", 0)) fprintf(stderr, "[wf] %s: %.3f ms\n", kGroup[s.kind], ms);
        }
        spans.clear(); ev_used = 0;
        return FTN_OK;
    };
    auto span_begin = [&](hipStream_t sm) -> int { const int a = ev_used++; (void)hipEventRecord(st->ev[a], sm); return a; };
    auto span_end = [&](int a, int kind, hipStream_t sm) { const int b = ev_used++; (void)hipEventRecord(st->ev[b], sm); spans.push_back(Span{a, b, kind}); };
    auto render_passes = [&]() -> int {
    for (uint32_t s0 = 0; s0 < total_samples; s0 += S) {
        const uint32_t Sp = std::min(S, total_samples - s0);
        W.n_slots = n_slots; W.samples = Sp; W.n_paths = Sp * n_slots; W.first_sample = P.first_sample + s0; W.seg_cap = (uint32_t)st->cap_paths;
        hipLaunchKernelGGL(k_wf_reset, dim3(1), dim3(64), 0, stream, W, 0, 0, P.stats);
        hipLaunchKernelGGL(k_wf_generate, dim3((W.n_paths + 255) / 256), dim3(256), 0, stream, P, W, dl_mode ? 1 : 0);
        int in_q = 0;
        const uint32_t* q_cl = W.q_closest; const uint32_t* q_sh = W.q_shadow;
        const uint32_t max_iter = P.max_depth + 2 + (1u << 20);
        for (uint32_t it = 0; it < max_iter; it++) {
            bool polled = false;
            const unsigned tg = std::min<unsigned>(trace_grid_max, (2 * W.n_paths + 255) / 256);
            if (ev_used + 10 > 64) { rc = flush_events(); if (rc) return rc; }
#ifdef FTN_DRAIN_PROBE
            g_probe_bounce = it;
#endif
            const bool overlap = overlap_mode == 1u || (overlap_mode == 2u && W.n_paths <= (32u << 20));
            const bool beside = overlap && it > 0 && q_sh == W.q_shadow;
            W.drain_sig = nullptr; W.drain_seq = 0;
            const bool gated = beside && st->drain_sig && drain_gate;
            if (beside) WF_TRY(hipEventRecord(st->ev_ready, stream));
            if (gated) {
                if (st->drain_seq >= 0xfffffff0u) { WF_TRY(hipStreamSynchronize(stream)); WF_TRY(hipStreamSynchronize(st->side)); WF_TRY(hipMemset(st->drain_sig, 0, 8)); st->drain_seq = 0; }
                W.drain_sig = st->drain_sig; W.drain_seq = ++st->drain_seq;
                W.drain_at = 1;
            }
            { const int e = span_begin(stream);
              launch_trace(st, false, count_mode, spheres, tg, lds, stream, P, W, q_cl, &W.counters[CTR(2)], &W.counters[CTR(16)], 2 * W.n_paths,
                           it == 0 && W.samples >= knob("FTN_T4_LOCKSTEP_MIN_SPP", 1) );
              span_end(e, 0, stream); }
            if (gated) WF_TRY(hipStreamWriteValue32(stream, st->drain_sig, W.drain_seq, 0));
            trace_launches++;
            if (beside) WF_TRY(hipStreamWaitEvent(st->side, st->ev_ready, 0));
            if (gated) WF_TRY(hipStreamWaitValue32(st->side, st->drain_sig, W.drain_seq, hipStreamWaitValueGte, 0xffffffffu));
            if (it > 0) {
                const unsigned sg = std::min<unsigned>(trace_grid_max, (2 * W.n_paths + 255) / 256);
                hipStream_t as = beside ? st->side : stream;
                const int e = span_begin(as);
                launch_trace(st, true, count_mode, spheres, sg, lds, as, P, W, q_sh, &W.counters[CTR(3)], &W.counters[CTR(24)], 2 * W.n_paths, it == 1 && W.samples >= 4u);
                span_end(e, 1, as);
                if (beside) WF_TRY(hipEventRecord(st->ev_side, st->side));
            }
            {
                const int e_cls = span_begin(stream);
                const unsigned cg = std::min<unsigned>(shade_grid_max, (W.n_paths + 255) / 256);
                hipLaunchKernelGGL(k_wf_reset, dim3(1), dim3(64), 0, stream, W, 2, in_q, P.stats);
                hipLaunchKernelGGL(k_wf_classify, dim3(cg), dim3(256), 0, stream, P, W, in_q);
                span_end(e_cls, 2, stream);
            }
            if (beside) WF_TRY(hipStreamWaitEvent(stream, st->ev_side, 0));
            const int e_shade = span_begin(stream);
            hipLaunchKernelGGL(k_wf_reset, dim3(1), dim3(64), 0, stream, W, 1, in_q, P.stats);
            {
                const dim3 sgrid(std::min<unsigned>(shade_grid_max, (W.n_paths + 255) / 256));
                const bool tex = P.S.n_textures != 0;
                const uint32_t first = it == 0 ? 1u : 0u;
                if (dl_mode) {
                    if (whitted) { if (tex) hipLaunchKernelGGL((k_wf_shade_dl<true, true>), sgrid, dim3(256), 0, stream, P, W, in_q); else hipLaunchKernelGGL((k_wf_shade_dl<true, false>), sgrid, dim3(256), 0, stream, P, W, in_q); }
                    else { if (tex) hipLaunchKernelGGL((k_wf_shade_dl<false, true>), sgrid, dim3(256), 0, stream, P, W, in_q); else hipLaunchKernelGGL((k_wf_shade_dl<false, false>), sgrid, dim3(256), 0, stream, P, W, in_q); }
                } else if (!knob("FTN_SHADE_SPECIALISE", 1)) {
                    if (tex) hipLaunchKernelGGL((k_wf_shade<true, -1, false>), sgrid, dim3(256), 0, stream, P, W, in_q, 0xffu, first);
                    else hipLaunchKernelGGL((k_wf_shade<false, -1, false>), sgrid, dim3(256), 0, stream, P, W, in_q, 0xffu, first);
                } else {
                    const bool env = P.S.env_only && knob("FTN_SHADE_ENV", 1);
                    const unsigned grid_k = knob("FTN_SHADE_GRID", 0), grid_k_nb = knob("FTN_SHADE_GRID_NOBSDF", 0);
#define FTN_SH2(T, M, E, mask) do { const unsigned per_cu = (M) == -2 ? (grid_k_nb ? grid_k_nb : 2u * shade_wgs_per_cu<T, M, E>()) : (grid_k ? grid_k : shade_wgs_per_cu<T, M, E>()); \
                                    hipLaunchKernelGGL((k_wf_shade<T, M, E>), dim3(std::min<unsigned>((unsigned)st->n_cu * per_cu, (W.n_paths + 255) / 256)), dim3(256), 0, stream, P, W, in_q, mask, first); } while (0)
#define FTN_SH(M, mask) do { if (tex) { if (env) FTN_SH2(true, M, true, mask); else FTN_SH2(true, M, false, mask); } \
                             else { if (env) FTN_SH2(false, M, true, mask); else FTN_SH2(false, M, false, mask); } } while (0)
                    FTN_SH(-2, 0x83u);
                    if (P.S.material_types & 1u) FTN_SH(0, 1u << 2);
                    if (P.S.material_types & 2u) FTN_SH(1, 1u << 3);
                    if (P.S.material_types & 4u) FTN_SH(2, 1u << 4);
                    if (P.S.material_types & 8u) FTN_SH(3, 1u << 5);
                    if (P.S.material_types & 16u) FTN_SH(4, 1u << 6);
#undef FTN_SH2
#undef FTN_SH
                }
            }
            span_end(e_shade, 2, stream);
            in_q ^= 1;
            if (sort_bits) {
                WF_TRY(hipMemcpyAsync(st->host_counters, W.counters, 16 * 32 * sizeof(uint32_t), hipMemcpyDeviceToHost, stream));
                WF_TRY(hipStreamSynchronize(stream));
                polled = true;
#ifdef FTN_DRAIN_PROBE
                { const uint32_t* T = &st->host_counters[CTR(13) + 4 * (it & 7u)];
                  if (T[3]) fprintf(stderr, "[wf] any-hit launch of bounce %u: first wave dry at %.1f us, last wave dry at %.1f us, end %.1f us\n", it, (~T[1] - ~T[0]) * 0.01, (T[2] - ~T[0]) * 0.01, (T[3] - ~T[0]) * 0.01); }
#endif
                const size_t n = st->cap_paths;
                uint32_t* const k_in = W.q_sorted + 4 * n, *const k_out = W.q_sorted + 6 * n;
                q_cl = W.q_closest; q_sh = W.q_shadow;
                const int e_sort = span_begin(stream);
                if ((rc = sort_ray_queue(st, P, W, false, W.q_closest, st->host_counters[CTR(2)], W.q_sorted, k_in, k_out, sort_bits, stream, &q_cl))) return rc;
                if (knob("FTN_WF_SORT_ANY", 0) && (rc = sort_ray_queue(st, P, W, true, W.q_shadow, st->host_counters[CTR(3)], W.q_sorted + 2 * n, k_in, k_out, sort_bits, stream, &q_sh))) return rc;
                span_end(e_sort, 3, stream);
            }
            if (it >= P.max_depth || polled) {
                if (!polled) {
                    WF_TRY(hipMemcpyAsync(st->host_counters, W.counters, 16 * 32 * sizeof(uint32_t), hipMemcpyDeviceToHost, stream));
                    WF_TRY(hipStreamSynchronize(stream));
                }
                if (it >= P.max_depth && count && knob("FTN_WF_DEBUG", 0)) fprintf(stderr, "[wf] wave steps so far: node %u leaf %u; lanes during node steps (x64): idle %u waiting-with-leaf %u\n", st->host_counters[CTR(6)], st->host_counters[CTR(7)], st->host_counters[CTR(8)], st->host_counters[CTR(9)]);
                n_active = st->host_counters[CTR(in_q == 0 ? 0 : 1)];
                if (n_active == 0) break;
            }
        }
        if (W.mis_any) mis_any_rays += st->host_counters[CTR(10)];
        hipLaunchKernelGGL(k_wf_accumulate, dim3((n_slots + 255) / 256), dim3(256), 0, stream, P, W);
    }
    return FTN_OK;
    };
    rc = render_passes();
    { const int rc_flush = flush_events(); if (!rc) rc = rc_flush; }
    if (rc) return rc;
    WF_TRY(hipGetLastError());
    if (times) {
        times->trace_ms = trace_ms; times->trace_launches = trace_launches; times->mis_any_rays = mis_any_rays;
        times->any_ms = group_ms[1]; times->any_launches = group_n[1]; times->shade_ms = group_ms[2]; times->shade_launches = group_n[2]; times->sort_ms = group_ms[3];
    }
    return FTN_OK;
}

}
```

fountain_amd/csrc/ftn_wf_common.h:

```cpp
#ifndef FTN_WF_COMMON_H
#define FTN_WF_COMMON_H
#include "ftn_wavefront.h"

namespace ftn {

enum : uint32_t { PS_BOUNCE_MASK = 0xffffu, PS_SPECULAR = 1u << 16, PS_ALIVE = 1u << 17, PS_DIRECT = 1u << 18, PS_SHADOW = 1u << 19, PS_MIS = 1u << 20, PS_DELTA = 1u << 21, PS_MIS_ANY = 1u << 22  };
#define PS_DRAWS_SHIFT 23
#define WF_MIS_BIT 0x80000000u

struct WfBuffers {
    uint32_t n_paths;
    uint32_t n_slots;
    uint32_t samples;
    uint32_t first_sample;
    float4 *ray;
    float4* hit;
    int* hit_prim;
    float4 *sh;
    unsigned char* occluded;
    float4 *beta;
    float4 *rad;
    float4* br;
    ulonglong2 *rng01, *rng23;
    float4 *pend0, *pend1, *pend2;
    float4* pd;
    uint32_t pd_md, pd_occ;
    uint32_t *q_active[2], *q_closest, *q_shadow;
    uint32_t* q_sorted;
    uint32_t* cls;
    uint32_t seg_cap;
    uint32_t* counters;
    uint32_t valid_per_sample;
    uint32_t* drain_sig; uint32_t drain_seq, drain_at;
    uint32_t *q_exc_closest, *q_exc_any;
    float4 *dlA, *dlB, *whT;
    float4* dfd;
    uint32_t serial;
    uint2* ser_cursor;
    float2* ser_pfilm;
    unsigned char* ser_retired;
    uint32_t rng_replay;
    uint32_t gen_blocks;
    uint32_t mis_any;
};

#define WF_Q_FIN 0x80000000u
#define WF_Q_DEPTH 0x40000000u
#define WF_Q_ID_MASK 0x0fffffffu

#define CTR(i) ((i) * 32)
__device__ inline uint32_t lane_id() { return threadIdx.x & 63u; }
__device__ inline void wave_push(bool pred, uint32_t value, uint32_t* queue, uint32_t* counter) {
    const unsigned long long m = __ballot(pred);
    if (m == 0) return;
    const int leader = __ffsll((long long)m) - 1;
    uint32_t base = 0;
    if ((int)lane_id() == leader) base = atomicAdd(counter, (uint32_t)__popcll(m));
    base = __shfl(base, leader, 64);
    if (pred) queue[base + (uint32_t)__popcll(m & ((1ull << lane_id()) - 1ull))] = value;
}

template <int NQ>
__device__ inline void block_push(const bool (&pred)[NQ], const uint32_t (&value)[NQ], uint32_t* const (&queue)[NQ], uint32_t* const (&counter)[NQ]) {
    __shared__ uint32_t s_cnt[NQ][4];
    __shared__ uint32_t s_base[NQ];
    const uint32_t wave = threadIdx.x >> 6, lane = lane_id();
    unsigned long long m[NQ];
#pragma unroll
    for (int q = 0; q < NQ; q++) { m[q] = __ballot(pred[q]); if (lane == 0) s_cnt[q][wave] = (uint32_t)__popcll(m[q]); }
    __syncthreads();
    if (threadIdx.x < NQ) {
        const uint32_t q = threadIdx.x;
        const uint32_t tot = s_cnt[q][0] + s_cnt[q][1] + s_cnt[q][2] + s_cnt[q][3];
        s_base[q] = tot ? atomicAdd(counter[q], tot) : 0u;
    }
    __syncthreads();
#pragma unroll
    for (int q = 0; q < NQ; q++) {
        if (pred[q]) {
            uint32_t off = s_base[q];
            for (uint32_t w = 0; w < wave; w++) off += s_cnt[q][w];
            if (queue[q]) queue[q][off + (uint32_t)__popcll(m[q] & ((1ull << lane) - 1ull))] = value[q];
        }
    }
    __syncthreads();
}

__device__ inline void store_occluded(const WfBuffers& W, uint32_t slot, bool occ) {
    if (W.pd_occ) {
        if (!occ) return;
        const bool mis = slot >= W.n_paths;
        const uint32_t p = mis ? slot - W.n_paths : slot;
        ((unsigned char*)(W.pd + 4 * (size_t)p + 3))[12 + (mis ? 1 : 0)] = occ ? 1 : 0;
    } else W.occluded[slot] = occ ? 1 : 0;
}

template <bool ANY>
__device__ inline void load_queued_ray(const WfBuffers& W, uint32_t rid, float4* a, float4* b, uint32_t* slot) {
    const uint32_t pid = rid & ~WF_MIS_BIT;
    if (ANY && !(rid & WF_MIS_BIT)) { *a = W.sh[2 * (size_t)pid]; *b = W.sh[2 * (size_t)pid + 1]; *slot = pid; }
    else { const uint32_t r = (rid & WF_MIS_BIT) ? pid + W.n_paths : pid; *a = W.ray[2 * (size_t)r]; *b = W.ray[2 * (size_t)r + 1]; *slot = r; }
}

template <bool SPHERES>
__device__ inline bool prim_hit(const DScene& S, uint32_t prim, float4 g0, float4 g1, float4 g2, V3 o, V3 dorig, float t_max, int kz, float sx, float sy, float sz,
                                float* t_out, float* b0o, float* b1o, float* b2o) {
    const uint32_t fl = __float_as_uint(g0.w);
    float t = 0.0f, b0 = 0.0f, b1 = 0.0f, b2 = 0.0f; bool hh = false;
    if (SPHERES && (fl & GF_KIND_SPHERE)) {
        DRay r; r.o = o; r.d = dorig; r.t_max = t_max; r.time = 0.0f;
        hh = sphere_intersect<false>(S.spheres[__float_as_uint(g1.w)], r, &t, nullptr);
    } else {
        const bool k0 = kz == 0, k1 = kz == 1;
#define FTN_PERM(v) V3(k0 ? (v).y : (k1 ? (v).z : (v).x), k0 ? (v).z : (k1 ? (v).x : (v).y), k0 ? (v).x : (k1 ? (v).y : (v).z))
        const V3 op = FTN_PERM(o);
        V3 p0t = FTN_PERM(g0), p1t = FTN_PERM(g1), p2t = FTN_PERM(g2);
#undef FTN_PERM
        p0t = V3(p0t.x - op.x, p0t.y - op.y, p0t.z - op.z);
        p1t = V3(p1t.x - op.x, p1t.y - op.y, p1t.z - op.z);
        p2t = V3(p2t.x - op.x, p2t.y - op.y, p2t.z - op.z);
        p0t.x += sx * p0t.z; p0t.y += sy * p0t.z;
        p1t.x += sx * p1t.z; p1t.y += sy * p1t.z;
        p2t.x += sx * p2t.z; p2t.y += sy * p2t.z;
        float e0 = p1t.x * p2t.y - p1t.y * p2t.x;
        float e1 = p2t.x * p0t.y - p2t.y * p0t.x;
        float e2 = p0t.x * p1t.y - p0t.y * p1t.x;
        if (e0 == 0.0f || e1 == 0.0f || e2 == 0.0f) {
            e0 = (float)((double)p1t.x * (double)p2t.y - (double)p1t.y * (double)p2t.x);
            e1 = (float)((double)p2t.x * (double)p0t.y - (double)p2t.y * (double)p0t.x);
            e2 = (float)((double)p0t.x * (double)p1t.y - (double)p0t.y * (double)p1t.x);
        }
        const float det = e0 + e1 + e2;
        if (!(sign_pos(e0) != sign_pos(e1) || sign_pos(e1) != sign_pos(e2)) && det != 0.0f) {
            p0t.z *= sz; p1t.z *= sz; p2t.z *= sz;
            const float t_scaled = e0 * p0t.z + e1 * p1t.z + e2 * p2t.z;
            if (!((det < 0.0f && (t_scaled >= 0.0f || t_scaled < t_max * det)) || (det > 0.0f && (t_scaled <= 0.0f || t_scaled > t_max * det)))) {
                const float inv_det = 1.0f / det;
                b0 = e0 * inv_det; b1 = e1 * inv_det; b2 = e2 * inv_det; t = t_scaled * inv_det;
                const float max_zt = fmax_(fmax_(fabsf(p0t.z), fabsf(p1t.z)), fabsf(p2t.z));
                const float delta_z = gamma_n(3) * max_zt;
                const float max_xt = fmax_(fmax_(fabsf(p0t.x), fabsf(p1t.x)), fabsf(p2t.x));
                const float max_yt = fmax_(fmax_(fabsf(p0t.y), fabsf(p1t.y)), fabsf(p2t.y));
                const float delta_x = gamma_n(5) * (max_xt + max_zt), delta_y = gamma_n(5) * (max_yt + max_zt);
                const float delta_e = 2.0f * (gamma_n(2) * max_xt * max_yt + delta_y * max_xt + delta_x * max_yt);
                const float max_e = fmax_(fmax_(fabsf(e0), fabsf(e1)), fabsf(e2));
                const float delta_t = 3.0f * (gamma_n(3) * max_e * max_zt + delta_e * max_zt + delta_z * max_e) * fabsf(inv_det);
                hh = !(t <= delta_t);
                if (hh && (fl & GF_HAS_UVS) && tri_uv_degenerate_reject(S, (int)prim, V3(g0.x, g0.y, g0.z), V3(g1.x, g1.y, g1.z), V3(g2.x, g2.y, g2.z))) hh = false;
            }
        }
    }
    *t_out = t; *b0o = b0; *b1o = b1; *b2o = b2;
    return hh;
}


struct Trace4Plan {
    uint32_t entries_closest, entries_any;
    uint32_t spill_closest, spill_any;
    size_t lds_closest, lds_any;
    unsigned grid_closest, grid_any;
    bool oct_ok; uint32_t entries_oct, spill_oct; size_t lds_oct; unsigned grid_oct;
    bool q64_ok; uint32_t entries_q64, spill_q64; size_t lds_q64; unsigned grid_q64;
};
enum : int { T4K_CLOSEST = 0, T4K_ANY = 1, T4K_ANY_OCT = 2, T4K_CLOSEST_Q64 = 3 };
#ifndef T4Q_WAVES
#define T4Q_WAVES 6
#endif
Trace4Plan trace4_plan(const DScene& S, int n_cu, uint32_t knob_entries_closest, uint32_t knob_entries_any, uint32_t knob_wg_closest, uint32_t knob_wg_any, uint32_t knob_wg_oct, uint32_t knob_entries_oct);
void launch_trace4(int kind, bool count, bool spheres, unsigned grid, size_t lds, uint32_t lds_entries, void* spill, hipStream_t stream, const DScene& S, const WfBuffers& W,
                   const uint32_t* queue, const uint32_t* count_ptr, uint32_t* head, DevStats* stats, uint32_t refill, uint32_t leaf_batch, uint32_t chunk, uint32_t burst, uint32_t any_policy, uint32_t spill_levels);

}
#endif
```

Before: 3229.

## Regenerate camera rays in trace and shade instead of storing them

Adds a cam_rebuild mode in which the generate kernel skips writing primary rays and path state. The first-bounce trace kernel and first shade kernel instead recompute each camera ray from the pixel, sample index and seed. The aim is to cut global-memory writes and reads of ray buffers for primary rays, paying with extra RNG and camera arithmetic in the trace and shade kernels. New template variants of the trace and shade kernels are added, and exceptional rays are written back when handed off.

```diff
diff --git a/fountain_amd/csrc/ftn_gbuffer.hip b/fountain_amd/csrc/ftn_gbuffer.hip
--- a/fountain_amd/csrc/ftn_gbuffer.hip
+++ b/fountain_amd/csrc/ftn_gbuffer.hip
@@ -44,12 +44,8 @@
             } else {
                 ftn_material m = S.materials[si.mat];
                 if (TEX && material_is_textured(S, si.mat)) {
-                    const uint32_t slot = p / W.samples, sidx = p % W.samples;
-                    const DTile tile = P.tiles[slot >> 8];
-                    const int px = tile.x0 + (int)(slot & 15u), py = tile.y0 + (int)((slot >> 4) & 15u);
-                    Rng crng; crng.seed(indexed_key(P.seed, px, py, W.first_sample + sidx));
-                    const V2 j = crng.next2(); const V2 p_film((float)px + j.x, (float)py + j.y); const V2 p_lens = crng.next2(); const float time_u = crng.next();
-                    const DRay cam = camera_ray(P.C, p_film, p_lens, time_u);
+                    Rng crng; V2 p_film, p_lens;
+                    const DRay cam = wf_camera_ray(P.C, P.seed, P.tiles, W, p, &crng, &p_film, &p_lens);
                     const DRayDiff rd = camera_ray_diff(P.C, p_film, p_lens, cam, 1.0f / sqrtf((float)P.spp));
                     DSIX ex; DSI s2; make_interaction(S, h, ray0, &s2, &ex);
                     const DTexDiffs td = compute_tex_diffs(si.hit.p, si.hit.n, ex.dpdu, ex.dpdv, rd);
@@ -210,6 +206,7 @@
     if ((rc = trace4_prepare(st, P.S))) return rc;
     WfBuffers W = st->W;
     W.br = nullptr; W.pd = nullptr; W.pd_md = 0; W.pd_occ = 0; W.drain_sig = nullptr; W.drain_seq = 0; W.serial = 0; W.rng_replay = 0; W.mis_any = 0;
+    W.cam_rebuild = 0;
     W.gen_blocks = knob("FTN_GEN_BLOCKS", 1);
     uint32_t valid = 0; for (const DTile& t : tiles) valid += (uint32_t)((t.x1 - t.x0) * (t.y1 - t.y0));
     W.valid_per_sample = valid;
diff --git a/fountain_amd/csrc/ftn_trace4.hip b/fountain_amd/csrc/ftn_trace4.hip
--- a/fountain_amd/csrc/ftn_trace4.hip
+++ b/fountain_amd/csrc/ftn_trace4.hip
@@ -156,9 +156,12 @@
 }
 
 enum : uint32_t { T4_LEAF_IN = 3 };
-template <bool COUNT, bool SPHERES, int BURST, bool Q64 = false>
+__device__ inline const CamKey& cam_key_of(const CamKey& k) { return k; }
+template <bool COUNT, bool SPHERES, int BURST, bool Q64 = false, class... CAMKEY>
 __global__ void __launch_bounds__(256, (SPHERES ? 1 : (Q64 ? T4Q_WAVES : 5))) k_wf_trace4(DScene S, WfBuffers W, const uint32_t* __restrict__ queue, const uint32_t* count_ptr, uint32_t* head, DevStats* stats,
-                                                   uint32_t refill, uint32_t leaf_batch, uint32_t chunk_max, uint32_t lds_entries, uint2* __restrict__ spill, uint32_t spill_levels) {
+                                                   uint32_t refill, uint32_t leaf_batch, uint32_t chunk_max, uint32_t lds_entries, uint2* __restrict__ spill, uint32_t spill_levels,
+                                                   CAMKEY... cam_key) {
+    constexpr bool CAM = sizeof...(CAMKEY) != 0;
     T4Stack<uint2> St;
     extern __shared__ uint2 lds_stack2[];
     St.base = lds_stack2 + threadIdx.x;
@@ -191,11 +194,19 @@
             if (L.mode == T4_IDLE && rank < avail) {
                 float4 a, b;
                 q_entry = queue[Q.chunk_next + rank];
-                load_queued_ray<false>(W, q_entry, &a, &b, &rid);
+                if constexpr (CAM) {
+                    Rng rng; V2 p_film, p_lens;
+                    rid = q_entry;
+                    const CamKey& K = cam_key_of(cam_key...);
+                    const DRay cr = wf_camera_ray(K.C, K.seed, K.tiles, W, rid, &rng, &p_film, &p_lens);
+                    a = make_float4(cr.o.x, cr.o.y, cr.o.z, 0.0f); b = make_float4(cr.d.x, cr.d.y, cr.d.z, cr.t_max);
+                } else load_queued_ray<false>(W, q_entry, &a, &b, &rid);
                 ray_setup<SPHERES>(R, a, b);
                 St.sp = St.base; L.cur = 0; found = false; hprim = -1; hb0 = 0.0f; hb1 = 0.0f; hb2 = 0.0f;
-                if (ray_is_exceptional(R.o.x, R.o.y, R.o.z, R.inv.x, R.inv.y, R.inv.z) || (Q64 && ray_out_of_range8(R.o.x, R.o.y, R.o.z, R.inv.x, R.inv.y, R.inv.z)))
+                if (ray_is_exceptional(R.o.x, R.o.y, R.o.z, R.inv.x, R.inv.y, R.inv.z) || (Q64 && ray_out_of_range8(R.o.x, R.o.y, R.o.z, R.inv.x, R.inv.y, R.inv.z))) {
                     hand_back = true;
+                    if (CAM) { W.ray[2 * (size_t)rid] = a; W.ray[2 * (size_t)rid + 1] = b; }
+                }
                 else if (S.n_nodes == 0 || !slab_test(rlo, rhi, R.o, R.inv, R.t_max)) { W.hit[rid] = make_float4(FTN_INF, 0.0f, 0.0f, 0.0f); W.hit_prim[rid] = -1; }
                 else if (S.root_is_leaf) { L.lp = 0; L.mode = T4_LEAF; }
                 else L.mode = T4_NODE;
@@ -543,9 +554,21 @@
     return p;
 }
 
+bool trace4_has_camera_variant(int kind, bool count, bool spheres, uint32_t burst) {
+    return (kind == T4K_CLOSEST_Q64 || kind == T4K_CLOSEST) && !spheres && (count || burst == 3u);
+}
+
 void launch_trace4(int kind, bool count, bool spheres, unsigned grid, size_t lds, uint32_t lds_entries, void* spill, hipStream_t stream, const DScene& S, const WfBuffers& W,
-                   const uint32_t* queue, const uint32_t* count_ptr, uint32_t* head, DevStats* stats, uint32_t refill, uint32_t leaf_batch, uint32_t chunk, uint32_t burst, uint32_t any_policy, uint32_t spill_levels) {
+                   const uint32_t* queue, const uint32_t* count_ptr, uint32_t* head, DevStats* stats, uint32_t refill, uint32_t leaf_batch, uint32_t chunk, uint32_t burst, uint32_t any_policy, uint32_t spill_levels,
+                   const CamKey* cam) {
     const bool any = kind == T4K_ANY || kind == T4K_ANY_OCT;
+    if (cam) {
+#define FTN_T4C(...) hipLaunchKernelGGL((k_wf_trace4<__VA_ARGS__, CamKey>), dim3(grid), dim3(256), lds, stream, S, W, queue, count_ptr, head, stats, refill, leaf_batch, chunk, lds_entries, (uint2*)spill, spill_levels, *cam)
+        if (kind == T4K_CLOSEST_Q64) { if (count) FTN_T4C(true, false, 2, true); else FTN_T4C(false, false, 3, true); }
+        else { if (count) FTN_T4C(true, false, 2, false); else FTN_T4C(false, false, 3, false); }
+#undef FTN_T4C
+        return;
+    }
 #define FTN_T4(K, SPILL_T, ...) hipLaunchKernelGGL((K<__VA_ARGS__>), dim3(grid), dim3(256), lds, stream, S, W, queue, count_ptr, head, stats, refill, leaf_batch, chunk, lds_entries, (SPILL_T)spill, spill_levels)
     if (kind == T4K_CLOSEST_Q64) {
         if (count) FTN_T4(k_wf_trace4, uint2*, true, false, 2, true);
diff --git a/fountain_amd/csrc/ftn_wavefront.hip b/fountain_amd/csrc/ftn_wavefront.hip
--- a/fountain_amd/csrc/ftn_wavefront.hip
+++ b/fountain_amd/csrc/ftn_wavefront.hip
@@ -13,18 +13,16 @@
     const DTile tile = P.tiles[slot >> 8];
     const int px = tile.x0 + (int)(slot & 15u), py = tile.y0 + (int)((slot >> 4) & 15u);
     if (px < tile.x1 && py < tile.y1) {
-        Rng rng; rng.seed(indexed_key(P.seed, px, py, W.first_sample + s));
-        V2 j = rng.next2();
-        V2 p_film((float)px + j.x, (float)py + j.y);
-        V2 p_lens = rng.next2();
-        float time_u = rng.next();
-        DRay ray = camera_ray(P.C, p_film, p_lens, time_u);
-        W.ray[2 * (size_t)(i)] = make_float4(ray.o.x, ray.o.y, ray.o.z, 0.0f);
-        W.ray[2 * (size_t)(i) + 1] = make_float4(ray.d.x, ray.d.y, ray.d.z, ray.t_max);
-        if (write_state) {
-            W.beta[i] = make_float4(1.0f, 1.0f, 1.0f, __uint_as_float(PS_ALIVE));
-            W.rad[i] = make_float4(0.0f, 0.0f, 0.0f, 0.0f);
-            W.rng01[i] = make_ulonglong2(rng.s0, rng.s1); W.rng23[i] = make_ulonglong2(rng.s2, rng.s3);
+        if (!W.cam_rebuild) {
+            Rng rng; V2 p_film, p_lens;
+            const DRay ray = wf_camera_ray(P.C, P.seed, P.tiles, W, i, &rng, &p_film, &p_lens);
+            W.ray[2 * (size_t)(i)] = make_float4(ray.o.x, ray.o.y, ray.o.z, 0.0f);
+            W.ray[2 * (size_t)(i) + 1] = make_float4(ray.d.x, ray.d.y, ray.d.z, ray.t_max);
+            if (write_state) {
+                W.beta[i] = make_float4(1.0f, 1.0f, 1.0f, __uint_as_float(PS_ALIVE));
+                W.rad[i] = make_float4(0.0f, 0.0f, 0.0f, 0.0f);
+                W.rng01[i] = make_ulonglong2(rng.s0, rng.s1); W.rng23[i] = make_ulonglong2(rng.s2, rng.s3);
+            }
         }
         uint32_t local = (uint32_t)(py - tile.y0) * (uint32_t)(tile.x1 - tile.x0) + (uint32_t)(px - tile.x0);
         if (W.gen_blocks && tile.x1 - tile.x0 == 16 && tile.y1 - tile.y0 == 16) {
@@ -332,9 +330,10 @@
 #ifndef FTN_SHADE_WAVES_OTHER
 #define FTN_SHADE_WAVES_OTHER 3
 #endif
-template <bool TEX, int MT, bool ENV>
-__global__ void __launch_bounds__(256, (MT == -1 ? FTN_SHADE_MIN_WAVES : (MT == -2 ? FTN_SHADE_WAVES_NOBSDF : (MT == 0 ? FTN_SHADE_WAVES_MATTE : FTN_SHADE_WAVES_OTHER)))) k_wf_shade(RenderParams P, WfBuffers W, int in_q, uint32_t class_mask, uint32_t first ) {
+template <bool TEX, int MT, bool ENV, bool CAM = false>
+__global__ void __launch_bounds__(256, (MT == -1 ? FTN_SHADE_MIN_WAVES : (MT == -2 ? FTN_SHADE_WAVES_NOBSDF : (MT == 0 ? FTN_SHADE_WAVES_MATTE : FTN_SHADE_WAVES_OTHER)))) k_wf_shade(RenderParams P, WfBuffers W, int in_q, uint32_t class_mask, uint32_t first_pass ) {
     const DScene& S = P.S;
+    const uint32_t first = CAM ? 1u : first_pass;
     uint32_t cbase[WF_NCLASS + 1], ccnt[WF_NCLASS];
     cbase[0] = 0;
 #pragma unroll
@@ -348,13 +347,14 @@
     for (uint32_t round = 0; round < rounds; round++) {
         const uint32_t qi = round * stride + blockIdx.x * 256u + threadIdx.x;
         bool have = false;
-        uint32_t sorted_idx = 0;
+        uint32_t sorted_idx = 0, path_class = 0;
         if (qi < count) {
             uint32_t c = 0, cb = 0, cc = ccnt[0];
 #pragma unroll
             for (int k = 1; k < WF_NCLASS; k++) if (qi >= cbase[k]) { c = (uint32_t)k; cb = cbase[k]; cc = ccnt[k]; }
             have = qi - cb < cc;
             sorted_idx = c * W.seg_cap + (qi - cb);
+            path_class = c;
         }
         bool push_active = false, push_closest = false, push_mis = false, push_shadow = false, push_mis_any = false;
         uint32_t p = 0, active_entry = 0;
@@ -406,7 +406,12 @@
                 DHit h; h.t = FTN_INF; h.b0 = 0.0f; h.b1 = 0.0f; h.b2 = 0.0f; h.prim = -1;
                 bool need_ray = true;
                 if (MT == -2 && !first) { h.prim = W.hit_prim[p]; need_ray = h.prim >= 0 || (ps & PS_BOUNCE_MASK) == 0u || (ps & PS_SPECULAR) != 0u; }
-                if (need_ray) {
+                Rng cam_rng; V2 cam_film, cam_lens;
+                if (CAM) {
+                    ray0 = wf_camera_ray(P.C, P.seed, P.tiles, W, p, &cam_rng, &cam_film, &cam_lens);
+                    ray0.time = 0.0f;
+                    if (!(MT == -2 && path_class == 1u && P.max_depth > 0)) h = load_hit(W, p);
+                } else if (need_ray) {
                     const float4 ro = W.ray[2 * (size_t)(p)], rdv = W.ray[2 * (size_t)(p) + 1];
                     ray0.o = V3(ro.x, ro.y, ro.z); ray0.d = V3(rdv.x, rdv.y, rdv.z); ray0.t_max = rdv.w;
                     h = load_hit(W, p);
@@ -428,7 +433,8 @@
                 if (!hit || bounces >= P.max_depth) alive = false;
                 else {
                     Rng rng;
-                    if (first) {
+                    if (CAM) rng = cam_rng;
+                    else if (first) {
                         const uint32_t slot = p / W.samples, sidx = p % W.samples;
                         const DTile tile = P.tiles[slot >> 8];
                         rng.seed(indexed_key(P.seed, tile.x0 + (int)(slot & 15u), tile.y0 + (int)((slot >> 4) & 15u), W.first_sample + sidx));
@@ -453,14 +459,11 @@
                             if (W.serial) {
                                 const float4 d0 = W.dfd[p], d1 = W.dfd[(size_t)W.n_paths + p], d2 = W.dfd[2 * (size_t)W.n_paths + p];
                                 rd.has = true; rd.rxo = V3(d0.x, d0.y, d0.z); rd.ryo = V3(d1.x, d1.y, d1.z); rd.ryd = V3(d2.x, d2.y, d2.z); rd.rxd = V3(d0.w, d1.w, d2.w);
-                            } else {
-                                const uint32_t slot = p / W.samples, sidx = p % W.samples;
-                                const DTile tile = P.tiles[slot >> 8];
-                                const int px = tile.x0 + (int)(slot & 15u), py = tile.y0 + (int)((slot >> 4) & 15u);
-                                Rng crng; crng.seed(indexed_key(P.seed, px, py, W.first_sample + sidx));
-                                const V2 j = crng.next2(); const V2 p_film((float)px + j.x, (float)py + j.y); const V2 p_lens = crng.next2(); const float time_u = crng.next();
-                                const DRay cam = camera_ray(P.C, p_film, p_lens, time_u);
-                                rd = camera_ray_diff(P.C, p_film, p_lens, cam, 1.0f / sqrtf((float)P.spp));
+                            } else if (CAM) rd = camera_ray_diff(P.C, cam_film, cam_lens, ray0, 1.0f / sqrtf((float)P.spp));
+                            else {
+                                Rng crng; V2 p_film, p_lens;
+                                const DRay cray = wf_camera_ray(P.C, P.seed, P.tiles, W, p, &crng, &p_film, &p_lens);
+                                rd = camera_ray_diff(P.C, p_film, p_lens, cray, 1.0f / sqrtf((float)P.spp));
                             }
                             DSIX ex; DSI s2; make_interaction(S, h, ray0, &s2, &ex);
                             const DTexDiffs td = compute_tex_diffs(si.hit.p, si.hit.n, ex.dpdu, ex.dpdv, rd);
@@ -567,8 +570,8 @@
     if (err) atomicCAS(&P.stats->error, 0, err);
 }
 
-template <bool TEX, int MT, bool ENV> static unsigned shade_wgs_per_cu() {
-    static const unsigned nb = [] { int v = 0; return (hipOccupancyMaxActiveBlocksPerMultiprocessor(&v, k_wf_shade<TEX, MT, ENV>, 256, 0) == hipSuccess && v >= 1) ? (unsigned)(v > 8 ? 8 : v) : 3u; }();
+template <bool TEX, int MT, bool ENV, bool CAM> static unsigned shade_wgs_per_cu() {
+    static const unsigned nb = [] { int v = 0; return (hipOccupancyMaxActiveBlocksPerMultiprocessor(&v, k_wf_shade<TEX, MT, ENV, CAM>, 256, 0) == hipSuccess && v >= 1) ? (unsigned)(v > 8 ? 8 : v) : 3u; }();
     return nb;
 }
 
@@ -678,12 +681,8 @@
                     DSIX ex; DTexDiffs td; float bsdf_eta = 1.0f; DRayDiff rd; rd.has = false;
                     if (TEX && mp) {
                         if (depth == 0u) {
-                            const uint32_t slot = p / W.samples, sidx = p % W.samples;
-                            const DTile tile = P.tiles[slot >> 8];
-                            const int px = tile.x0 + (int)(slot & 15u), py = tile.y0 + (int)((slot >> 4) & 15u);
-                            Rng crng; crng.seed(indexed_key(P.seed, px, py, W.first_sample + sidx));
-                            const V2 j = crng.next2(); const V2 p_film((float)px + j.x, (float)py + j.y); const V2 p_lens = crng.next2(); const float time_u = crng.next();
-                            const DRay cam = camera_ray(P.C, p_film, p_lens, time_u);
+                            Rng crng; V2 p_film, p_lens;
+                            const DRay cam = wf_camera_ray(P.C, P.seed, P.tiles, W, p, &crng, &p_film, &p_lens);
                             rd = camera_ray_diff(P.C, p_film, p_lens, cam, 1.0f / sqrtf((float)P.spp));
                         } else {
                             const float4 d0 = W.dfd[p], d1 = W.dfd[(size_t)W.n_paths + p], d2 = W.dfd[2 * (size_t)W.n_paths + p];
@@ -1091,8 +1090,11 @@
     return FTN_OK;
 }
 
+static uint32_t closest_burst(bool camera_rays) { return camera_rays ? knob("FTN_T4_BURST0", 3) : knob("FTN_T4_BURST", 2); }
+
 static void launch_trace(WavefrontState* st, bool any, int count, bool spheres, unsigned grid, size_t lds, hipStream_t stream, const RenderParams& P, const WfBuffers& W,
-                         const uint32_t* queue, const uint32_t* count_ptr, uint32_t* head, uint32_t max_rays, bool camera_rays = false) {
+                         const uint32_t* queue, const uint32_t* count_ptr, uint32_t* head, uint32_t max_rays, bool camera_rays = false,
+                         const CamKey* cam = nullptr ) {
     if (st->t4_on && count != 1) {
         const Trace4Plan& T = st->t4;
         const bool oct = any && st->t8_on, q64 = !any && st->q64_on;
@@ -1106,7 +1108,8 @@
                       queue, count_ptr, head, P.stats,
                       any ? knob("FTN_T4_ANY_REFILL", 32) : (camera_rays ? knob("FTN_T4_REFILL0", 64) : knob("FTN_T4_REFILL", 32)),
                       any ? knob("FTN_T4_ANY_LEAF_BATCH", 16) : (camera_rays ? knob("FTN_T4_LEAF_BATCH0", 2) : knob("FTN_T4_LEAF_BATCH", 16)), chunk4,
-                      any ? knob("FTN_T4_ANY_BURST", 4) : (camera_rays ? knob("FTN_T4_BURST0", 3) : knob("FTN_T4_BURST", 2)), knob("FTN_T4_ANY_POLICY", 1), any ? T.spill_any : (q64 ? T.spill_q64 : T.spill_closest));
+                      any ? knob("FTN_T4_ANY_BURST", 4) : closest_burst(camera_rays), knob("FTN_T4_ANY_POLICY", 1), any ? T.spill_any : (q64 ? T.spill_q64 : T.spill_closest),
+                      any ? nullptr : cam);
         const unsigned ge = std::min<unsigned>(grid, (unsigned)st->n_cu);
         uint32_t* ecount = &W.counters[CTR(any ? 33 : 32)]; uint32_t* ehead = &W.counters[CTR(any ? 48 : 40)];
         DevStats* none = nullptr;
@@ -1265,7 +1268,7 @@
     WfBuffers W = st->W;
     W.serial = 1; W.ser_cursor = (uint2*)st->ser_mem[0]; W.ser_pfilm = (float2*)st->ser_mem[1]; W.ser_retired = (unsigned char*)st->ser_mem[2]; W.dfd = (float4*)st->ser_mem[3];
     W.n_slots = 0; W.samples = 1; W.n_paths = n_tiles; W.first_sample = 0; W.seg_cap = (uint32_t)st->cap_paths; W.valid_per_sample = 0;
-    W.gen_blocks = 0; W.rng_replay = 0; W.br = nullptr; W.pd = nullptr; W.pd_md = 0; W.pd_occ = 0;
+    W.gen_blocks = 0; W.rng_replay = 0; W.cam_rebuild = 0; W.br = nullptr; W.pd = nullptr; W.pd_md = 0; W.pd_occ = 0;
     const int count_mode = count ? (count_production ? 2 : 1) : 0;
     W.mis_any = ((!count || count_production) && knob("FTN_MIS_ANY", 1)) ? 1u : 0u;
     const bool spheres = P.S.n_spheres != 0;
@@ -1393,6 +1396,8 @@
     W.pd_md = (W.pd && knob("FTN_WF_PD", 3) >= 2) ? 1u : 0u;
     W.pd_occ = (W.pd && knob("FTN_WF_PD", 3) >= 3) ? 1u : 0u;
     W.gen_blocks = knob("FTN_GEN_BLOCKS", 1);
+    const bool cam_ok = !dl_mode && st->t4_on && count_mode != 1 && knob("FTN_WF_CAMRAYS", 0) == 0;
+    CamKey cam_key; cam_key.C = P.C; cam_key.seed = P.seed; cam_key.tiles = P.tiles;
     const size_t lds = (size_t)P.stack_entries * 256 * sizeof(uint32_t);
     const unsigned blocks_per_cu = (unsigned)std::max<size_t>(1, std::min<size_t>(8, (size_t)(160 * 1024) / std::max<size_t>(lds, 1)));
     const unsigned trace_grid_max = (unsigned)st->n_cu * blocks_per_cu;
@@ -1425,6 +1430,8 @@
     for (uint32_t s0 = 0; s0 < total_samples; s0 += S) {
         const uint32_t Sp = std::min(S, total_samples - s0);
         W.n_slots = n_slots; W.samples = Sp; W.n_paths = Sp * n_slots; W.first_sample = P.first_sample + s0; W.seg_cap = (uint32_t)st->cap_paths;
+        const bool lockstep = W.samples >= knob("FTN_T4_LOCKSTEP_MIN_SPP", 1);
+        W.cam_rebuild = (cam_ok && trace4_has_camera_variant(st->q64_on ? T4K_CLOSEST_Q64 : T4K_CLOSEST, count_mode == 2, spheres, closest_burst(lockstep))) ? 1u : 0u;
         hipLaunchKernelGGL(k_wf_reset, dim3(1), dim3(64), 0, stream, W, 0, 0, P.stats);
         hipLaunchKernelGGL(k_wf_generate, dim3((W.n_paths + 255) / 256), dim3(256), 0, stream, P, W, dl_mode ? 1 : 0);
         int in_q = 0;
@@ -1449,7 +1456,7 @@
             }
             { const int e = span_begin(stream);
               launch_trace(st, false, count_mode, spheres, tg, lds, stream, P, W, q_cl, &W.counters[CTR(2)], &W.counters[CTR(16)], 2 * W.n_paths,
-                           it == 0 && W.samples >= knob("FTN_T4_LOCKSTEP_MIN_SPP", 1) );
+                           it == 0 && lockstep, it == 0 && W.cam_rebuild ? &cam_key : nullptr);
               span_end(e, 0, stream); }
             if (gated) WF_TRY(hipStreamWriteValue32(stream, st->drain_sig, W.drain_seq, 0));
             trace_launches++;
@@ -1477,17 +1484,21 @@
                 const dim3 sgrid(std::min<unsigned>(shade_grid_max, (W.n_paths + 255) / 256));
                 const bool tex = P.S.n_textures != 0;
                 const uint32_t first = it == 0 ? 1u : 0u;
+                const bool cam = first && W.cam_rebuild;
                 if (dl_mode) {
                     if (whitted) { if (tex) hipLaunchKernelGGL((k_wf_shade_dl<true, true>), sgrid, dim3(256), 0, stream, P, W, in_q); else hipLaunchKernelGGL((k_wf_shade_dl<true, false>), sgrid, dim3(256), 0, stream, P, W, in_q); }
                     else { if (tex) hipLaunchKernelGGL((k_wf_shade_dl<false, true>), sgrid, dim3(256), 0, stream, P, W, in_q); else hipLaunchKernelGGL((k_wf_shade_dl<false, false>), sgrid, dim3(256), 0, stream, P, W, in_q); }
                 } else if (!knob("FTN_SHADE_SPECIALISE", 1)) {
-                    if (tex) hipLaunchKernelGGL((k_wf_shade<true, -1, false>), sgrid, dim3(256), 0, stream, P, W, in_q, 0xffu, first);
-                    else hipLaunchKernelGGL((k_wf_shade<false, -1, false>), sgrid, dim3(256), 0, stream, P, W, in_q, 0xffu, first);
+                    if (tex) { if (cam) hipLaunchKernelGGL((k_wf_shade<true, -1, false, true>), sgrid, dim3(256), 0, stream, P, W, in_q, 0xffu, first);
+                               else hipLaunchKernelGGL((k_wf_shade<true, -1, false>), sgrid, dim3(256), 0, stream, P, W, in_q, 0xffu, first); }
+                    else { if (cam) hipLaunchKernelGGL((k_wf_shade<false, -1, false, true>), sgrid, dim3(256), 0, stream, P, W, in_q, 0xffu, first);
+                           else hipLaunchKernelGGL((k_wf_shade<false, -1, false>), sgrid, dim3(256), 0, stream, P, W, in_q, 0xffu, first); }
                 } else {
                     const bool env = P.S.env_only && knob("FTN_SHADE_ENV", 1);
                     const unsigned grid_k = knob("FTN_SHADE_GRID", 0), grid_k_nb = knob("FTN_SHADE_GRID_NOBSDF", 0);
-#define FTN_SH2(T, M, E, mask) do { const unsigned per_cu = (M) == -2 ? (grid_k_nb ? grid_k_nb : 2u * shade_wgs_per_cu<T, M, E>()) : (grid_k ? grid_k : shade_wgs_per_cu<T, M, E>()); \
-                                    hipLaunchKernelGGL((k_wf_shade<T, M, E>), dim3(std::min<unsigned>((unsigned)st->n_cu * per_cu, (W.n_paths + 255) / 256)), dim3(256), 0, stream, P, W, in_q, mask, first); } while (0)
+#define FTN_SH3(T, M, E, C, mask) do { const unsigned per_cu = (M) == -2 ? (grid_k_nb ? grid_k_nb : 2u * shade_wgs_per_cu<T, M, E, C>()) : (grid_k ? grid_k : shade_wgs_per_cu<T, M, E, C>()); \
+                                       hipLaunchKernelGGL((k_wf_shade<T, M, E, C>), dim3(std::min<unsigned>((unsigned)st->n_cu * per_cu, (W.n_paths + 255) / 256)), dim3(256), 0, stream, P, W, in_q, mask, first); } while (0)
+#define FTN_SH2(T, M, E, mask) do { if (cam) FTN_SH3(T, M, E, true, mask); else FTN_SH3(T, M, E, false, mask); } while (0)
 #define FTN_SH(M, mask) do { if (tex) { if (env) FTN_SH2(true, M, true, mask); else FTN_SH2(true, M, false, mask); } \
                              else { if (env) FTN_SH2(false, M, true, mask); else FTN_SH2(false, M, false, mask); } } while (0)
                     FTN_SH(-2, 0x83u);
@@ -1496,6 +1507,7 @@
                     if (P.S.material_types & 4u) FTN_SH(2, 1u << 4);
                     if (P.S.material_types & 8u) FTN_SH(3, 1u << 5);
                     if (P.S.material_types & 16u) FTN_SH(4, 1u << 6);
+#undef FTN_SH3
 #undef FTN_SH2
 #undef FTN_SH
                 }
diff --git a/fountain_amd/csrc/ftn_wf_common.h b/fountain_amd/csrc/ftn_wf_common.h
--- a/fountain_amd/csrc/ftn_wf_common.h
+++ b/fountain_amd/csrc/ftn_wf_common.h
@@ -42,7 +42,22 @@
     uint32_t rng_replay;
     uint32_t gen_blocks;
     uint32_t mis_any;
+    uint32_t cam_rebuild;
 };
+
+struct CamKey { DCamera C; unsigned long long seed; const DTile* tiles; };
+
+__device__ inline DRay wf_camera_ray(const DCamera& C, unsigned long long seed, const DTile* tiles, const WfBuffers& W, uint32_t p, Rng* rng, V2* p_film, V2* p_lens) {
+    const uint32_t slot = p / W.samples, sidx = p % W.samples;
+    const DTile tile = tiles[slot >> 8];
+    const int px = tile.x0 + (int)(slot & 15u), py = tile.y0 + (int)((slot >> 4) & 15u);
+    rng->seed(indexed_key(seed, px, py, W.first_sample + sidx));
+    const V2 j = rng->next2();
+    *p_film = V2((float)px + j.x, (float)py + j.y);
+    *p_lens = rng->next2();
+    const float time_u = rng->next();
+    return camera_ray(C, *p_film, *p_lens, time_u);
+}
 
 #define WF_Q_FIN 0x80000000u
 #define WF_Q_DEPTH 0x40000000u
@@ -169,7 +184,9 @@
 #endif
 Trace4Plan trace4_plan(const DScene& S, int n_cu, uint32_t knob_entries_closest, uint32_t knob_entries_any, uint32_t knob_wg_closest, uint32_t knob_wg_any, uint32_t knob_wg_oct, uint32_t knob_entries_oct);
 void launch_trace4(int kind, bool count, bool spheres, unsigned grid, size_t lds, uint32_t lds_entries, void* spill, hipStream_t stream, const DScene& S, const WfBuffers& W,
-                   const uint32_t* queue, const uint32_t* count_ptr, uint32_t* head, DevStats* stats, uint32_t refill, uint32_t leaf_batch, uint32_t chunk, uint32_t burst, uint32_t any_policy, uint32_t spill_levels);
+                   const uint32_t* queue, const uint32_t* count_ptr, uint32_t* head, DevStats* stats, uint32_t refill, uint32_t leaf_batch, uint32_t chunk, uint32_t burst, uint32_t any_policy, uint32_t spill_levels,
+                   const CamKey* cam = nullptr );
+bool trace4_has_camera_variant(int kind, bool count, bool spheres, uint32_t burst);
 
 }
 #endif
```

Measured after the change: 3233 (median of 2 runs). Within noise of the previous version (+0.1%).
